# mandanasmi/lane-slam

Hardware: AMD Instinct MI355X
Metric: frames/sec (640x480) detect->descript->project->sanity->associate (higher is better)
Workload: dtype u8/f64 (FP4 e2m1 MFMA with exact f32 accumulation for association)

## Files before the change

lane_slam_amd/csrc/common.h:

```cpp
#pragma once
#include <hip/hip_runtime.h>
#include <stdint.h>
#include <stddef.h>
#include "../../include/lanefront.h"
#include "detmath.h"

namespace lf {

constexpr int kMaxKsize = 9;
constexpr int kMaxGaussTaps = 15;
constexpr float kNotDef = -1024.0f;
#ifndef LF_LABEL_ITEMS
#define LF_LABEL_ITEMS 8192
#endif
constexpr int kLabelItems = LF_LABEL_ITEMS;
#ifndef LF_LABEL_LDS
#define LF_LABEL_LDS 6144
#endif
constexpr int kLabelLds = LF_LABEL_LDS;
constexpr int kCompCap = 1024;

enum Stage {
    ST_PRE = 0, ST_CANNY, ST_HYST, ST_LSD_GRAD, ST_LSD_ORDER, ST_LSD_GROW, ST_SEGMENTS,
    ST_LBD_GRAD, ST_LBD, ST_ASSOC_PACK, ST_ASSOC, ST_MISC, ST_JPEG, ST_LSD_LABEL, ST_HOUGH, ST_DENSE, ST_COUNT
};
static_assert(ST_COUNT == LF_N_STAGES, "stage table out of sync with lanefront.h");

struct PreParams {
    int in_rows, in_cols, img_rows, img_cols, top_cutoff, Hc, W;
    int resize;
    int identity_ai;
    double ifx, ify;
    float ai_scale[3], ai_shift[3];
    int lo[4][3], hi[4][3];
    int ksize, r;
    int j1[kMaxKsize], j2[kMaxKsize];
};

struct CannyParams {
    int Hc, W, Ww;
    int low, high;
};

struct LsdParams {
    int Hc, W;
    int Hs, Ws;
    int Ww;
    int scaled;
    int ntaps, half;
    double k[kMaxGaussTaps];
    double rho;
    double prec, p;
    double log_nt, log_eps, density_th, scale;
    int min_reg_size, n_bins, refine;
    int cap_lines;
    int label_items;
    int label_items_max;
    int label_lds;
    int rec_cap;
    float* r_sd = nullptr;
    float* c_sd = nullptr;
};

struct SegParams {
    int Hc, W, img_rows, img_cols, top_cutoff, cap_lines;
    double rx, ry, cut;
    double cw, ch;
    double H[9], K[9], D[5], RR[9];
    double lanewidth, linewidth_white, linewidth_yellow, d_min, d_max, phi_min, phi_max;
    int rectified_input;
};

struct ResizeTables {
    const int* xofs;
    const float* xa;
    const int* y0;
    const int* y1;
    const float* yb;
    int xmax;
};

}

#ifdef __HIPCC__
__device__ __forceinline__ void lf_xcd_tile(int& bx, int& by, int& bz)
{
    const unsigned nx = gridDim.x, ny = gridDim.y, total = nx * ny * gridDim.z;
    unsigned b = blockIdx.x + nx * (blockIdx.y + ny * blockIdx.z);
    const unsigned group = 8u * nx;
    if (b < total / group * group) {
        const unsigned g = b / group, r = b - g * group;
        b = g * group + (r & 7u) * nx + (r >> 3);
    }
    bx = (int)(b % nx);
    const unsigned q = b / nx;
    by = (int)(q % ny);
    bz = (int)(q / ny);
}
#endif

extern "C" void lf_set_error(lf_handle* h, int code, const char* fmt, ...);

namespace lf {
void launch_pre_gray(const PreParams& p, const uint8_t* frames, int n_frames, uint8_t* gray, hipStream_t s);
void launch_pre(const PreParams& p, const uint8_t* frames, int n_frames, uint32_t* bgr, uint8_t* gray,
                uint32_t* maskbits, const int* sdiv, const int* hdiv, hipStream_t s, uint32_t* bwbits = nullptr);
void launch_canny(const CannyParams& p, const uint32_t* bgr, int n_frames, uint32_t* strong, uint32_t* weak,
                  hipStream_t s);
int launch_hysteresis(const CannyParams& p, int n_frames, uint32_t* strong, const uint32_t* weak, hipStream_t s);
void launch_bgrx_to_bgr(int n_pix, const uint32_t* bgrx, uint8_t* bgr, hipStream_t s);
void launch_edges_u8(const CannyParams& p, int n_frames, const uint32_t* bits, uint8_t* edges, hipStream_t s);
void launch_lsd_grad(const LsdParams& p, const ResizeTables& rt, int n_frames, const uint32_t* edge_bits,
                     const uint32_t* mask_bits, uint32_t* r_addr, float* r_deg, double* r_mod, double* r_cs, double* r_sn,
                     int* n_rec, unsigned long long* maxgrad, int max_nsx, int max_nsy, uint32_t* list, int* list_count,
                     uint32_t* l_addr, double* l_mod, int* n_low, int* rec_need, bool counters_zeroed, hipStream_t s);
void launch_lsd_grad_gray(const LsdParams& p, const ResizeTables& rt, int n_frames, const uint8_t* gray, uint32_t* r_addr, float* r_deg,
                          double* r_mod, double* r_cs, double* r_sn, int* n_rec, unsigned long long* maxgrad, int max_nsx, int max_nsy,
                          uint32_t* list, int* list_count, uint32_t* l_addr, double* l_mod, int* n_low, hipStream_t s);
bool lsd_seed32_supported(const LsdParams& p);
void launch_lsd_seed32(const LsdParams& p, int n_frames, int* n_rec, int* norder, int* rec_need, const unsigned long long* maxgrad, const uint32_t* c_xy,
                       const double* c_mod, const uint32_t* l_addr, double* l_mod, const int* n_low,
                       unsigned long long* sort_a, unsigned long long* sort_b, uint32_t* order_a, uint32_t* order_b, int big, hipStream_t s);
size_t std_sort_debug_words(int n);
void launch_std_sort_debug(const uint32_t* E, uint32_t* work, int n, int* count, hipStream_t s);
void launch_lsd_order(const LsdParams& p, int n_frames, const uint32_t* r_addr, const float* r_deg, const double* r_mod,
                      const double* r_cs, const double* r_sn, int* n_rec, const unsigned long long* maxgrad,
                      unsigned long long* sort_a, unsigned long long* sort_b, uint32_t* order_a, uint32_t* order_b,
                      int* norder, uint32_t* c_xy, float* c_deg, double* c_mod, double* c_cs, double* c_sn,
                      int* row_start, hipStream_t s);
void launch_lsd_dense_debug(const LsdParams& p, int n_frames, const int* norder, const uint32_t* c_xy, const float* c_deg,
                            const double* c_mod, float* ang, double* mod, hipStream_t s);
void launch_lsd_rank(int n_prob, const int* norder, int* perm, hipStream_t s);
void launch_lsd_label(const LsdParams& p, int n_frames, const int* norder, const uint32_t* c_xy, const int* row_start,
                      uint16_t* c_label, uint16_t* comp_list, int* comp_count, int* comp_key, uint32_t* scratch, hipStream_t s);
size_t lsd_grow_reg_stride(const LsdParams& p);
void launch_lsd_grow(const LsdParams& p, int n_frames, const uint32_t* order, const int* norder, const uint32_t* c_xy,
                     const float* c_deg, const double* c_mod, const double* c_cs, const double* c_sn,
                     const int* row_start, const uint16_t* c_label, const uint16_t* comp_list, const int* comp_count, int comp_cap,
                     uint32_t* reg, uint32_t* gused, float* tmp_lines, int* tmp_tags, float* lines, int* counts, const int* perm,
                     int lds_kb, bool mixed, int bitmap, hipStream_t s);
int lsd_grow_def_lds(const LsdParams& p, int lds_kb);
constexpr int kGrowLdsKb[3] = { 13, 28, 40 };
void launch_seg_offsets(int n_frames, int cap_lines, const int* counts, int* seg_offset, int* frame_offset,
                        int* overflow, const int* norder, int cap_small, int cap_medium, hipStream_t s);
void launch_dense(int Hc, int W, int Ww, int cap_lines, float thr, int n_problems, const uint32_t* strong, const uint32_t* maskbits,
                  const uint32_t* bwbits, float* slot_lines, float* rec, int* counts, hipStream_t s);
enum SegMode { SEG_FLOAT = 0, SEG_HOUGH = 1, SEG_DENSE = 2 };
void launch_segments(const SegParams& p, int n_frames, const float* slot_lines, const int* counts,
                     const int* seg_offset, const uint32_t* side, int Ww, lf_segments out, int* seg_frame,
                     double* normals64, float* centers, hipStream_t s, SegMode mode = SEG_FLOAT);
void launch_lbd_grad(int Hc, int W, int n_frames, const uint8_t* gray, uint32_t* dxy, hipStream_t s);
struct LbdPlanes { const uint32_t* base[LF_MAX_OCTAVES]; int W[LF_MAX_OCTAVES], H[LF_MAX_OCTAVES]; };
void launch_lbd_keylines(const LbdPlanes& planes, int n_cap, int n_frames, const int* n_lines, const float* in_octave4, const float* angle, const int* npx,
                         const int* octave, const int* frame, const float* gauss_g, const float* gauss_l, float* desc, uint8_t* code,
                         hipStream_t s, int wband = 7);
void launch_lbd_split_debug(size_t n, const uint32_t* dxy, int16_t* dx, int16_t* dy, hipStream_t s);
void launch_lbd(int Hc, int W, int n_seg_cap, const int* n_seg, const float* lines, const int* seg_frame,
                const uint32_t* dxy, const float* gauss_g, const float* gauss_l,
                float* desc, uint8_t* code, hipStream_t s, int wband = 7);
int lbd_max_width_of_band();
size_t assoc_rows_padded_m(int nm);
__host__ __device__ inline size_t assoc_map_offset_fp4(size_t row, int byte)
{
    return (row >> 6) * 8192 + (size_t)(byte >> 4) * 1024 + (row & 63) * 16 + (size_t)(byte & 15);
}
__host__ __device__ inline uint32_t assoc_fp4_expand(uint32_t byte)
{
    uint32_t t = (byte | (byte << 12)) & 0x000f000fu;
    t = (t | (t << 6)) & 0x03030303u;
    t = (t | (t << 3)) & 0x11111111u;
    return (t << 3) | 0x22222222u;
}
#ifdef __HIPCC__
__device__ __forceinline__ void assoc_map_write_row(int8_t* mx, int8_t* mcx, size_t pos, int b, uint32_t byte, const uint8_t* colour_byte)
{
    *reinterpret_cast<uint32_t*>(mx + assoc_map_offset_fp4(pos, 4 * b)) = assoc_fp4_expand(byte);
    if (b < 8) {
        const int colour = *colour_byte;
        uint32_t w = 0;
        if (b == 0 && colour < 3)
            for (int g = 0; g < 3; ++g) if (g != colour) w |= 0xFu << (4 * g);
        *reinterpret_cast<uint32_t*>(mcx + pos * 32 + 4 * b) = w;
    }
}
__device__ __forceinline__ void assoc_map_zero_row(int8_t* mx, int8_t* mcx, size_t pos, int b)
{
    *reinterpret_cast<uint32_t*>(mx + assoc_map_offset_fp4(pos, 4 * b)) = 0u;
    if (b < 8) *reinterpret_cast<uint32_t*>(mcx + pos * 32 + 4 * b) = 0u;
}
#endif
template <typename T>
struct DevArray {
    T* p = nullptr;
    size_t bytes = 0;
    DevArray() = default;
    DevArray(DevArray&& o) noexcept : p(o.p), bytes(o.bytes) { o.p = nullptr; o.bytes = 0; }
    DevArray& operator=(DevArray&& o) noexcept
    {
        if (this != &o) { reset(); p = o.p; bytes = o.bytes; o.p = nullptr; o.bytes = 0; }
        return *this;
    }
    ~DevArray() { reset(); }
    hipError_t alloc(size_t n_bytes)
    {
        reset();
        const hipError_t e = hipMalloc((void**)&p, n_bytes);
        if (e != hipSuccess) p = nullptr; else bytes = n_bytes;
        return e;
    }
    void reset() { if (p) (void)hipFree(p); p = nullptr; bytes = 0; }
    operator T*() const { return p; }
};
using DevBuf = DevArray<void>;

template <typename T>
struct HostArray {
    T* p = nullptr;
    size_t bytes = 0;
    HostArray() = default;
    HostArray(HostArray&& o) noexcept : p(o.p), bytes(o.bytes) { o.p = nullptr; o.bytes = 0; }
    HostArray& operator=(HostArray&& o) noexcept
    {
        if (this != &o) { reset(); p = o.p; bytes = o.bytes; o.p = nullptr; o.bytes = 0; }
        return *this;
    }
    ~HostArray() { reset(); }
    hipError_t alloc(size_t n_bytes)
    {
        reset();
        const hipError_t e = hipHostMalloc((void**)&p, n_bytes, hipHostMallocDefault);
        if (e != hipSuccess) p = nullptr; else bytes = n_bytes;
        return e;
    }
    void reset() { if (p) (void)hipHostFree(p); p = nullptr; bytes = 0; }
    operator T*() const { return p; }
};

struct AssocScratch {
    DevArray<unsigned int> part; DevArray<int> done; size_t cap_part = 0, cap_blocks = 0;
    int qblocks = 0, splits = 0, m_chunk = 0;
    DevArray<int> tie_list; size_t cap_list = 0;
    unsigned long long* tie_res = nullptr;
};
void launch_assoc_pack_map(const uint8_t* codes, int n, int n_pad, int8_t* x, hipStream_t s);
hipError_t launch_assoc_core(const uint8_t* q, const uint8_t* qcolor, int nq, const int8_t* mx, const int8_t* mcx, int nm,
                             const int* nm_dev, int gating, int max_distance, AssocScratch& w, int32_t* idx, float* dist, hipStream_t s);
hipError_t launch_assoc_ties(const uint8_t* q, const uint8_t* qcolor, int nq, const int8_t* mx, const uint8_t* mcode, const uint8_t* mcolor,
                             int nm, const int* nm_dev, int gating, AssocScratch& w, unsigned long long* res, int32_t* idx, const float* dist, hipStream_t s);
hipError_t launch_assoc(const uint8_t* q, int nq, const uint8_t* m, int nm, int8_t* mx, AssocScratch& w, int32_t* idx, float* dist, hipStream_t s);
void launch_assoc_nomatch(int nq, int32_t* idx, float* dist, hipStream_t s);
void launch_kmeans(const uint8_t* bgr, int n, int k, const double* init, int max_iter, double tol_rel, uint8_t* lab, double* out,
                   long long* counts, int* status, hipStream_t s);
void launch_draw(const void* src, bool src_bgrx, uint8_t* out, int n_frames, int Hc, int W, const int32_t* frame_offset, const float* lines,
                 const uint8_t* color, int capacity, int* bad, hipStream_t s);
void launch_ai_transform(const uint8_t* strips, long long frame_stride, int n_frames, int S, int cols, uint8_t* lab, double* fo,
                         long long* fc, int* fs, lf_ai_transform* out, hipStream_t s);
struct MapDevice {
    int capacity, policy, kept_only, merge_distance, when_full;
    uint8_t* code; uint8_t* color; double* ground; int* hits; int* last_seen; int* winner;
    int8_t* mx; int8_t* mcx;
    int* state;
    unsigned long long* totals;
};
void launch_fill_i32(int* p, size_t n, int v, hipStream_t s);
void launch_map_pack_block(int n, int n_frames, const int* frame_offset, const uint8_t* code, const uint8_t* color,
                           const uint8_t* keep, const double* ground, const int32_t* idx, const float* dist,
                           const double* pose4, int step, uint8_t* block, hipStream_t s);
void launch_map_overflow_block(int n, int n_frames, int step, uint8_t* block, hipStream_t s);
void launch_map_seed_block(int n, const uint8_t* code, const uint8_t* color, const double* ground, uint8_t* block, hipStream_t s);
void launch_map_update(const MapDevice& md, const uint8_t* blocks, int n_blocks, int block_rows, int force_append, int* act,
                       hipStream_t s);
void launch_select_queries(const uint8_t* q, const uint8_t* mask, int nq, uint8_t* out, int32_t* qidx, int* n_out, hipStream_t s);
void launch_knn(const uint8_t* q, int nq, const uint8_t* m, int nm, int k, int max_distance, int mih, int32_t* idx, float* dist, hipStream_t s);
void launch_radius(const uint8_t* q, int nq, const uint8_t* m, int nm, int max_distance, int32_t* hist, int32_t* count, int32_t* offsets,
                   int* total, int cap, int mih, int32_t* idx, float* dist, hipStream_t s);
size_t assoc_float_scratch_bytes(int nq, int nm);
hipError_t launch_assoc_float(const float* q, int nq, const float* m, int nm, float* qn, float* mn,
                              void* scratch, int32_t* idx, float* dist, hipStream_t s);
namespace jpeg { struct FrameHeader; }
struct JpegGeom { int rows, cols, Wp, Hp; int first_row = 0; };
void launch_jpeg_decode(const JpegGeom& g, int n_frames, int max_blocks, const jpeg::FrameHeader* hdrs,
                        const uint32_t* entries, const uint32_t* block_end, uint8_t* planes, uint8_t* frames,
                        hipStream_t s);

void launch_jpeg_color(const JpegGeom& g, int n_frames, const void* hdrs, size_t hdr_stride, const uint8_t* planes, uint8_t* frames, hipStream_t s);
namespace jpeg { struct DevFrame; }
void launch_jh_decode(const JpegGeom& g, int n_frames, int max_blocks, size_t max_scan_len, jpeg::DevFrame* frames, const uint8_t* bytes, uint8_t* clean,
                      uint32_t* seg_begin, void* info, uint32_t* sub, int16_t* coef, int* status, uint8_t* planes, hipStream_t s);
size_t jh_info_bytes();

void launch_msg_layout(int n_frames, int stage, const int* frame_offset, const uint8_t* keep, int* counts,
                       long long* byte_offset, hipStream_t s);
void launch_msg_write(int n_frames, int stage, const int* frame_offset, const uint8_t* color, const float* pixels_normalized,
                      const float* normals, const double* ground, const uint8_t* keep, const int* counts,
                      const long long* byte_offset, uint8_t* out, hipStream_t s);
void launch_msg_read(int n_frames, int capacity, const uint8_t* body, const long long* byte_offset, int* frame_offset,
                     int* bad, uint8_t* color, float* pixels_normalized, float* normals, double* ground, hipStream_t s);

}
```

lane_slam_amd/csrc/k_lbd.hip:

```cpp
#include "common.h"

namespace lf {

#ifndef LF_LBD_TILE_H
#define LF_LBD_TILE_H 64
#endif
constexpr int LT_W = 64, LT_H = LF_LBD_TILE_H;
static_assert(LT_H % 16 == 0, "the Sobel phase gives every lane LT_H / 16 rows of its column group");

__device__ __forceinline__ int refl101(int p, int n)
{
    if (n == 1) return 0;
    while (p < 0 || p >= n) { p = p < 0 ? -p : 2 * (n - 1) - p; }
    return p;
}

__global__ __launch_bounds__(256) void k_lbd_grad(int Hc, int W, const uint8_t* __restrict__ gray_in,
                                                  uint32_t* __restrict__ dxyo)
{
    constexpr int GW = 72, GH = LT_H + 6;
    constexpr int RW = 68, RG = RW / 4;
    constexpr int BW_ = 72, BH = LT_H + 2;
    __shared__ __attribute__((aligned(16))) uint8_t gray[GH * GW];
    __shared__ __attribute__((aligned(16))) uint32_t rowp[(GH / 2) * RW];
    __shared__ __attribute__((aligned(16))) uint8_t blur[BH * BW_];
    int tbx, tby, f;
    lf_xcd_tile(tbx, tby, f);
    const int x0 = tbx * LT_W, y0 = tby * LT_H;
    const int tid = threadIdx.y * 64 + threadIdx.x;
    const uint8_t* img = gray_in + (size_t)f * Hc * W;
    const bool interior = x0 >= 4 && x0 + 72 <= W;
    auto reflect_row = [&](int ty) {
        int gy = y0 + ty - 3;
        gy = gy < 0 ? -gy : (gy >= Hc ? 2 * (Hc - 1) - gy : gy);
        if (gy < 0 || gy >= Hc) gy = refl101(y0 + ty - 3, Hc);
        return (uint32_t)gy * (uint32_t)W;
    };
    if (interior) {
        const uint8_t* base = img + (x0 - 4);
        for (int idx = tid; idx < GH * (GW / 4); idx += 256) {
            const int ty = idx / (GW / 4), g = idx - ty * (GW / 4);
            const uint32_t* q = reinterpret_cast<const uint32_t*>(base + (reflect_row(ty) + 4u * (uint32_t)g));
            *reinterpret_cast<uint32_t*>(gray + ty * GW + 4 * g) = (q[0] >> 8) | (q[1] << 24);
        }
    } else {
        for (int idx = tid; idx < GH * (GW / 4); idx += 256) {
            const int ty = idx / (GW / 4), g = idx - ty * (GW / 4);
            const uint32_t row = reflect_row(ty);
            const int xa = x0 + 4 * g - 4;
            uint32_t packed = 0;
            if (xa >= 0 && xa + 7 < W) {
                const uint32_t* q = reinterpret_cast<const uint32_t*>(img + (row + (uint32_t)xa));
                packed = (q[0] >> 8) | (q[1] << 24);
            } else {
#pragma unroll
                for (int k = 0; k < 4; ++k) packed |= (uint32_t)img[row + (uint32_t)refl101(x0 + 4 * g + k - 3, W)] << (8 * k);
            }
            *reinterpret_cast<uint32_t*>(gray + ty * GW + 4 * g) = packed;
        }
    }
    __syncthreads();
    static_assert(GH % 2 == 0 && BH % 2 == 0, "rows are filtered in pairs");
    typedef unsigned short us2 __attribute__((ext_vector_type(2)));
    for (int idx = tid; idx < (GH / 2) * RG; idx += 256) {
        const int m = idx / RG, g = idx - m * RG;
        uint32_t o02[2], o13[2];
#pragma unroll
        for (int r = 0; r < 2; ++r) {
            const uint32_t* src = reinterpret_cast<const uint32_t*>(gray + (2 * m + r) * GW + 4 * g);
            const uint32_t lo = src[0], hi = src[1];
            const us2 E = __builtin_bit_cast(us2, lo & 0x00ff00ffu), O = __builtin_bit_cast(us2, (lo >> 8) & 0x00ff00ffu);
            const us2 E2 = __builtin_bit_cast(us2, hi & 0x00ff00ffu), O2 = __builtin_bit_cast(us2, (hi >> 8) & 0x00ff00ffu);
            const us2 P24 = { E.y, E2.x }, P35 = { O.y, O2.x };
            const us2 c14 = { 14, 14 }, c63 = { 63, 63 }, c103 = { 103, 103 };
            o02[r] = __builtin_bit_cast(uint32_t, c14 * E + c63 * O + c103 * P24 + c63 * P35 + c14 * E2);
            o13[r] = __builtin_bit_cast(uint32_t, c14 * O + c63 * P24 + c103 * P35 + c63 * E2 + c14 * O2);
        }
        const uint4 q = make_uint4(__builtin_amdgcn_perm(o02[1], o02[0], 0x05040100u), __builtin_amdgcn_perm(o13[1], o13[0], 0x05040100u),
                                   __builtin_amdgcn_perm(o02[1], o02[0], 0x07060302u), __builtin_amdgcn_perm(o13[1], o13[0], 0x07060302u));
        *reinterpret_cast<uint4*>(rowp + m * RW + 4 * g) = q;
    }
    __syncthreads();
    {
        constexpr int VPAIRS = 3, VSEG = (BH / 2 + VPAIRS - 1) / VPAIRS;
        static_assert(VSEG * RG <= 256, "one lane per (column group, segment)");
        const int g = tid % RG, seg = tid / RG;
        if (seg < VSEG) {
            const int m0 = seg * VPAIRS;
            uint4 P[3];
            auto fetch = [&](int m) { return *reinterpret_cast<const uint4*>(rowp + (m < GH / 2 ? m : GH / 2 - 1) * RW + 4 * g); };
            P[0] = fetch(m0); P[1] = fetch(m0 + 1);
#pragma unroll
            for (int i = 0; i < VPAIRS; ++i) {
                const int m = m0 + i;
                P[(i + 2) % 3] = fetch(m + 2);
                if (2 * m < BH) {
                    const uint4 A = P[i % 3], B = P[(i + 1) % 3], C = P[(i + 2) % 3];
                    const uint32_t a[4] = { A.x, A.y, A.z, A.w }, bb[4] = { B.x, B.y, B.z, B.w }, cc[4] = { C.x, C.y, C.z, C.w };
                    uint32_t even = 0, odd = 0;
#pragma unroll
                    for (int k = 0; k < 4; ++k) {
                        uint32_t e = __builtin_amdgcn_udot2(__builtin_bit_cast(us2, a[k]), us2{ 14, 63 }, 1u << 15, false);
                        e = __builtin_amdgcn_udot2(__builtin_bit_cast(us2, bb[k]), us2{ 103, 63 }, e, false);
                        e = __builtin_amdgcn_udot2(__builtin_bit_cast(us2, cc[k]), us2{ 14, 0 }, e, false);
                        uint32_t o = __builtin_amdgcn_udot2(__builtin_bit_cast(us2, a[k]), us2{ 0, 14 }, 1u << 15, false);
                        o = __builtin_amdgcn_udot2(__builtin_bit_cast(us2, bb[k]), us2{ 63, 103 }, o, false);
                        o = __builtin_amdgcn_udot2(__builtin_bit_cast(us2, cc[k]), us2{ 63, 14 }, o, false);
                        e >>= 16; o >>= 16;
                        even |= (e > 255u ? 255u : e) << (8 * k);
                        odd |= (o > 255u ? 255u : o) << (8 * k);
                    }
                    *reinterpret_cast<uint32_t*>(blur + (2 * m) * BW_ + 4 * g) = even;
                    *reinterpret_cast<uint32_t*>(blur + (2 * m + 1) * BW_ + 4 * g) = odd;
                }
            }
        }
    }
    __syncthreads();
    {
        constexpr int SROWS = LT_H / 16;
        const int g = tid & 15, seg = tid >> 4;
        const int lx = 4 * g, gx = x0 + lx, ry0 = seg * SROWS;
        typedef short s2 __attribute__((ext_vector_type(2)));
        s2 P[3][4];
        auto unpack = [&](int row, s2 (&d)[4]) {
            const uint32_t* src = reinterpret_cast<const uint32_t*>(blur + row * BW_ + lx);
            const uint32_t lo = src[0], hi = src[1];
            const s2 E = __builtin_bit_cast(s2, lo & 0x00ff00ffu), O = __builtin_bit_cast(s2, (lo >> 8) & 0x00ff00ffu);
            const s2 E2 = __builtin_bit_cast(s2, hi & 0x00ff00ffu), O2 = __builtin_bit_cast(s2, (hi >> 8) & 0x00ff00ffu);
            d[0] = E; d[1] = O; d[2] = s2{ E.y, E2.x }; d[3] = s2{ O.y, O2.x };
        };
        unpack(ry0, P[0]);
        unpack(ry0 + 1, P[1]);
        auto a_plus_2b = [](s2 a, s2 b) {
            s2 d;
            const uint32_t two = 0x00020002u;
            asm("v_pk_mad_i16 %0, %1, %2, %3" : "=v"(d) : "v"(b), "v"(two), "v"(a));
            return d;
        };
        uint32_t* orow = dxyo + ((size_t)f * Hc + (size_t)(y0 + ry0)) * W + gx;
#pragma unroll
        for (int i = 0; i < SROWS; ++i) {
            const int ry = ry0 + i, gy = y0 + ry;
            unpack(ry + 2, P[(i + 2) % 3]);
            if (gx < W && gy < Hc) {
                s2 S[4], D[4];
#pragma unroll
                for (int c = 0; c < 4; ++c) { S[c] = a_plus_2b(P[i % 3][c], P[(i + 1) % 3][c]) + P[(i + 2) % 3][c]; D[c] = P[(i + 2) % 3][c] - P[i % 3][c]; }
                const s2 vx02 = S[2] - S[0], vx13 = S[3] - S[1];
                const s2 vy02 = a_plus_2b(D[0], D[1]) + D[2], vy13 = a_plus_2b(D[1], D[2]) + D[3];
                uint32_t* op = orow + (size_t)i * W;
                const uint32_t x02 = __builtin_bit_cast(uint32_t, vx02), x13 = __builtin_bit_cast(uint32_t, vx13);
                const uint32_t y02 = __builtin_bit_cast(uint32_t, vy02), y13 = __builtin_bit_cast(uint32_t, vy13);
                const uint32_t w[4] = { __builtin_amdgcn_perm(y02, x02, 0x05040100u), __builtin_amdgcn_perm(y13, x13, 0x05040100u),
                                        __builtin_amdgcn_perm(y02, x02, 0x07060302u), __builtin_amdgcn_perm(y13, x13, 0x07060302u) };
                if (gx + 3 < W && (W & 3) == 0) {
                    *reinterpret_cast<uint4*>(op) = make_uint4(w[0], w[1], w[2], w[3]);
                } else {
                    for (int k = 0; k < 4 && gx + k < W; ++k) op[k] = w[k];
                }
            }
        }
    }
}

void launch_lbd_grad(int Hc, int W, int n_frames, const uint8_t* gray, uint32_t* dxy, hipStream_t s)
{
    dim3 grid((W + LT_W - 1) / LT_W, (Hc + LT_H - 1) / LT_H, n_frames);
    hipLaunchKernelGGL(k_lbd_grad, grid, dim3(64, 4), 0, s, Hc, W, gray, dxy);
}

__constant__ int c_comb[32][2] = {
    {0,1},{0,2},{0,3},{0,4},{0,5},{0,6},{1,2},{1,3},{1,4},{1,5},{1,6},{2,3},{2,4},{2,5},{2,6},{2,7},
    {2,8},{3,4},{3,5},{3,6},{3,7},{3,8},{4,5},{4,6},{4,7},{4,8},{5,6},{5,7},{5,8},{6,7},{6,8},{7,8} };

constexpr int NBANDS = 9, WBAND = 7, LSP_H = 63;
constexpr int LBD_STEPS = 8;

constexpr int LBD_MAXW = 21;
template <bool KL, bool ANYW = false>
__global__ __launch_bounds__(256) void k_lbd(int Hc_, int W_, const int* __restrict__ n_seg_ptr,
                                             const float* __restrict__ lines, const int* __restrict__ seg_frame,
                                             const uint32_t* __restrict__ dxyi,
                                             const float* __restrict__ gauss_g , const float* __restrict__ gauss_l ,
                                             float* __restrict__ desc, uint8_t* __restrict__ code,
                                             LbdPlanes planes, const float* __restrict__ kl_angle, const int* __restrict__ kl_npx,
                                             const int* __restrict__ kl_octave, int n_cap, int n_frames, int wband_arg = WBAND)
{
    const int WBAND = ANYW ? wband_arg : lf::WBAND;
    const int LSP_H = ANYW ? NBANDS * wband_arg : lf::LSP_H;
    __shared__ float rows[4][ANYW ? NBANDS * LBD_MAXW : lf::LSP_H][4];
    __shared__ float dsc[4][72];
    const int wave = threadIdx.x >> 6, lane = threadIdx.x & 63;
    const int n_seg = min(*n_seg_ptr, n_cap);
  for (int seg = blockIdx.x * 4 + wave; seg < n_seg; seg += gridDim.x * 4) {
    __builtin_amdgcn_wave_barrier();
    __builtin_amdgcn_fence(__ATOMIC_ACQ_REL, "wavefront");
    const int f = seg_frame[seg];
    int Hc = Hc_, W = W_;
    const uint32_t* pdxy;
    float e0 = lines[4 * (size_t)seg], e1 = lines[4 * (size_t)seg + 1], e2 = lines[4 * (size_t)seg + 2], e3 = lines[4 * (size_t)seg + 3];
    int lengthOfLSP;
    float direction;
    if (KL) {
        const int oc = kl_octave[seg];
        if (oc < 0 || oc >= LF_MAX_OCTAVES || planes.base[oc] == nullptr || f < 0 || f >= n_frames) {
            if (desc) for (int i = lane; i < 72; i += 64) desc[(size_t)seg * 72 + i] = 0.f;
            if (code && lane < 32) code[(size_t)seg * 32 + lane] = 0;
            continue;
        }
        Hc = planes.H[oc]; W = planes.W[oc];
        pdxy = planes.base[oc] + (size_t)f * Hc * W;
        lengthOfLSP = (int)(short)kl_npx[seg];
        direction = kl_angle[seg];
    } else {
    pdxy = dxyi + (size_t)f * Hc * W;
    if (e0 < 0) e0 = 0;
    if (e0 >= W) e0 = (float)W - 1.0f;
    if (e2 < 0) e2 = 0;
    if (e2 >= W) e2 = (float)W - 1.0f;
    if (e1 < 0) e1 = 0;
    if (e1 >= Hc) e1 = (float)Hc - 1.0f;
    if (e3 < 0) e3 = 0;
    if (e3 >= Hc) e3 = (float)Hc - 1.0f;
    const int ix0 = dm::round_half_even((double)e0), iy0 = dm::round_half_even((double)e1);
    const int ix1 = dm::round_half_even((double)e2), iy1 = dm::round_half_even((double)e3);
    lengthOfLSP = max(abs(ix1 - ix0), abs(iy1 - iy0)) + 1;
    const float ddy = e3 - e1, ddx = e2 - e0;
    direction = (float)dm::datan2((double)ddy, (double)ddx);
    }
    const int halfWidth = (lengthOfLSP - 1) / 2;
    const int halfHeight = (LSP_H - 1) / 2;
    const int imageWidth = W - 1, imageHeight = Hc - 1;
    const float midX = (float)(0.5 * (e0 + e2));
    const float midY = (float)(0.5 * (e1 + e3));
    double sn_, cs_;
    dm::dsincos((double)direction, sn_, cs_);
    const float dL0 = (float)cs_, dL1 = (float)sn_;
    const float dO0 = -dL1, dO1 = dL0;
    float sCorX0 = -dL0 * halfWidth + dL1 * halfHeight + midX;
    float sCorY0 = -dL1 * halfWidth - dL0 * halfHeight + midY;
    int row_done = 0;
    for (int row = lane; row < LSP_H; row += 64) {
        for (; row_done < row; ++row_done) { sCorX0 -= dL1; sCorY0 += dL0; }
        float sCorX = sCorX0, sCorY = sCorY0;
        float pgdL = 0, ngdL = 0, pgdO = 0, ngdO = 0;
        for (int w0 = 0; w0 < lengthOfLSP; w0 += LBD_STEPS) {
            uint32_t dxyv[LBD_STEPS];
#pragma unroll
            for (int u = 0; u < LBD_STEPS; ++u) {
                int tx = (int)dm::round_half_away_f(sCorX);
                int xCor = tx < 0 ? 0 : (tx > imageWidth ? imageWidth : tx);
                int ty = (int)dm::round_half_away_f(sCorY);
                int yCor = ty < 0 ? 0 : (ty > imageHeight ? imageHeight : ty);
                dxyv[u] = pdxy[yCor * W + xCor];
                sCorX += dL0;
                sCorY += dL1;
            }
#pragma unroll
            for (int u = 0; u < LBD_STEPS; ++u) {
                if (w0 + u >= lengthOfLSP) break;
                const float gx_ = (float)(int)(int16_t)(dxyv[u] & 0xffffu), gy_ = (float)((int)dxyv[u] >> 16);
                float gDL = gx_ * dL0 + gy_ * dL1;
                float gDO = gx_ * dO0 + gy_ * dO1;
                if (gDL > 0) pgdL += gDL; else ngdL -= gDL;
                if (gDO > 0) pgdO += gDO; else ngdO -= gDO;
            }
        }
        const float cg = gauss_g[row];
        rows[wave][row][0] = cg * pgdL;
        rows[wave][row][1] = cg * ngdL;
        rows[wave][row][2] = cg * pgdO;
        rows[wave][row][3] = cg * ngdO;
        if (!ANYW) break;
    }
    __builtin_amdgcn_wave_barrier();
    __builtin_amdgcn_fence(__ATOMIC_ACQ_REL, "wavefront");
    float* D = dsc[wave];
    for (int e = lane; e < 72; e += 64) {
        const int b = e >> 3, q = e & 7;
        const bool sq = q >= 4;
        const int src = q & 3;
        const int h0 = (b - 1) * WBAND;
        const float* rp = &rows[wave][0][src] + 4 * h0;
        float acc = 0;
#pragma unroll
        for (int i = 0; i < (ANYW ? 3 * LBD_MAXW : 3 * lf::WBAND); ++i) {
            if (ANYW && i >= 3 * WBAND) break;
            const int hID = h0 + i;
            if (hID >= 0 && hID < LSP_H) {
                const float coef = gauss_l[i];
                const float v = rp[4 * i];
                if (!sq) acc += coef * v;
                else acc += coef * coef * (v * v);
            }
        }
        D[e] = acc;
    }
    __builtin_amdgcn_wave_barrier();
    __builtin_amdgcn_fence(__ATOMIC_ACQ_REL, "wavefront");
    float mean[4] = {0, 0, 0, 0}, sd[4] = {0, 0, 0, 0};
    if (lane < NBANDS) {
        const float invN = (lane == 0 || lane == NBANDS - 1) ? (float)(1.0 / (WBAND * 2.0)) : (float)(1.0 / (WBAND * 3.0));
#pragma unroll
        for (int q = 0; q < 4; ++q) {
            float temp = D[lane * 8 + q] * invN;
            mean[q] = temp;
            sd[q] = (float)dm::dsqrt((double)(D[lane * 8 + 4 + q] * invN - temp * temp));
        }
    }
    __builtin_amdgcn_wave_barrier();
    __builtin_amdgcn_fence(__ATOMIC_ACQ_REL, "wavefront");
    if (lane < NBANDS) {
#pragma unroll
        for (int q = 0; q < 4; ++q) { D[lane * 8 + q] = mean[q]; D[lane * 8 + 4 + q] = sd[q]; }
    }
    __builtin_amdgcn_wave_barrier();
    __builtin_amdgcn_fence(__ATOMIC_ACQ_REL, "wavefront");
    float tempM = 0, tempS = 0;
    for (int b = 0; b < NBANDS; ++b) {
        const float* v = D + 8 * b;
        tempM += v[0] * v[0]; tempM += v[1] * v[1]; tempM += v[2] * v[2]; tempM += v[3] * v[3];
        tempS += v[4] * v[4]; tempS += v[5] * v[5]; tempS += v[6] * v[6]; tempS += v[7] * v[7];
    }
    tempM = dm::fdiv(1.f, dm::fsqrt(tempM));
    tempS = dm::fdiv(1.f, dm::fsqrt(tempS));
    __builtin_amdgcn_wave_barrier();
    for (int e = lane; e < 72; e += 64) {
        float v = D[e] * (((e & 7) < 4) ? tempM : tempS);
        if ((double)v > 0.4) v = (float)0.4;
        D[e] = v;
    }
    __builtin_amdgcn_wave_barrier();
    __builtin_amdgcn_fence(__ATOMIC_ACQ_REL, "wavefront");
    float temp = 0;
    for (int i = 0; i < 72; ++i) temp += D[i] * D[i];
    temp = dm::fdiv(1.f, dm::fsqrt(temp));
    __builtin_amdgcn_wave_barrier();
    for (int e = lane; e < 72; e += 64) {
        float v = D[e] * temp;
        D[e] = v;
        if (desc) desc[(size_t)seg * 72 + e] = v;
    }
    __builtin_amdgcn_wave_barrier();
    __builtin_amdgcn_fence(__ATOMIC_ACQ_REL, "wavefront");
    if (code && lane < 32) {
        const float* f1 = D + 8 * c_comb[lane][0];
        const float* f2 = D + 8 * c_comb[lane][1];
        unsigned r = 0;
#pragma unroll
        for (int i = 0; i < 8; ++i) if (f1[i] > f2[i]) r += 1u << i;
        code[(size_t)seg * 32 + lane] = (uint8_t)r;
    }
  }
}

void launch_lbd(int Hc, int W, int n_seg_cap, const int* n_seg, const float* lines, const int* seg_frame,
                const uint32_t* dxy, const float* gauss_g, const float* gauss_l,
                float* desc, uint8_t* code, hipStream_t s, int wband)
{
    if (n_seg_cap <= 0) return;
    int blocks = (n_seg_cap + 3) / 4;
    if (blocks > 4096) blocks = 4096;
    LbdPlanes none;
    for (int i = 0; i < LF_MAX_OCTAVES; ++i) { none.base[i] = nullptr; none.W[i] = 0; none.H[i] = 0; }
    if (wband == WBAND)
        hipLaunchKernelGGL((k_lbd<false, false>), dim3(blocks), dim3(256), 0, s, Hc, W, n_seg, lines, seg_frame, dxy,
                           gauss_g, gauss_l, desc, code, none, nullptr, nullptr, nullptr, n_seg_cap, 0, WBAND);
    else
        hipLaunchKernelGGL((k_lbd<false, true>), dim3(blocks), dim3(256), 0, s, Hc, W, n_seg, lines, seg_frame, dxy,
                           gauss_g, gauss_l, desc, code, none, nullptr, nullptr, nullptr, n_seg_cap, 0, wband);
}
int lbd_max_width_of_band() { return LBD_MAXW; }

void launch_lbd_keylines(const LbdPlanes& planes, int n_cap, int n_frames, const int* n_lines, const float* in_octave4, const float* angle, const int* npx,
                         const int* octave, const int* frame, const float* gauss_g, const float* gauss_l, float* desc, uint8_t* code,
                         hipStream_t s, int wband)
{
    if (n_cap <= 0) return;
    int blocks = (n_cap + 3) / 4;
    if (blocks > 4096) blocks = 4096;
    if (wband == WBAND)
        hipLaunchKernelGGL((k_lbd<true, false>), dim3(blocks), dim3(256), 0, s, 0, 0, n_lines, in_octave4, frame, nullptr, gauss_g, gauss_l, desc, code,
                           planes, angle, npx, octave, n_cap, n_frames, WBAND);
    else
        hipLaunchKernelGGL((k_lbd<true, true>), dim3(blocks), dim3(256), 0, s, 0, 0, n_lines, in_octave4, frame, nullptr, gauss_g, gauss_l, desc, code,
                           planes, angle, npx, octave, n_cap, n_frames, wband);
}

__global__ void k_lbd_split_debug(size_t n, const uint32_t* __restrict__ dxy, int16_t* __restrict__ dx, int16_t* __restrict__ dy)
{
    const size_t i = blockIdx.x * (size_t)blockDim.x + threadIdx.x;
    if (i >= n) return;
    const uint32_t v = dxy[i];
    dx[i] = (int16_t)(v & 0xffffu);
    dy[i] = (int16_t)(v >> 16);
}

void launch_lbd_split_debug(size_t n, const uint32_t* dxy, int16_t* dx, int16_t* dy, hipStream_t s)
{
    hipLaunchKernelGGL(k_lbd_split_debug, dim3((unsigned)((n + 255) / 256)), dim3(256), 0, s, n, dxy, dx, dy);
}

}
```

lane_slam_amd/csrc/k_segments.hip:

```cpp
#include "common.h"
#include "lane_vote.h"

namespace lf {

__global__ void k_seg_offsets(int n_frames, int cap_lines, const int* __restrict__ counts, int* __restrict__ seg_offset,
                              int* __restrict__ frame_offset, int* __restrict__ overflow, const int* __restrict__ norder, int cap_small, int cap_medium)
{
    __shared__ int carry;
    __shared__ int wsum[16];
    const int n = n_frames * 3;
    const int t = threadIdx.x, lane = t & 63, wave = t >> 6;
    if (t == 0) carry = 0;
    __syncthreads();
    int ovf = 0;
    for (int base = 0; base < n; base += blockDim.x) {
        int i = base + t;
        int v = 0;
        if (i < n) {
            v = counts[i]; if (v > cap_lines) { v = cap_lines; ovf = 1; }
            if (norder) { const int nd = norder[i]; if (nd > cap_small) atomicAdd(overflow + 1, 1); if (nd > cap_medium) atomicAdd(overflow + 2, 1); atomicMax(overflow + 3, nd); }
        }
        int inc = v;
#pragma unroll
        for (int d = 1; d < 64; d <<= 1) { int o = __shfl_up(inc, d); if (lane >= d) inc += o; }
        if (lane == 63) wsum[wave] = inc;
        __syncthreads();
        int off = carry;
        for (int w = 0; w < wave; ++w) off += wsum[w];
        if (i < n) {
            int ex = off + inc - v;
            seg_offset[i] = ex;
            if (i % 3 == 0) frame_offset[i / 3] = ex;
        }
        __syncthreads();
        if (t == blockDim.x - 1) carry = off + inc;
        __syncthreads();
    }
    if (t == 0) { seg_offset[n] = carry; frame_offset[n_frames] = carry; overflow[7] = carry; }
    if (ovf) atomicOr(overflow, 1);
}

void launch_seg_offsets(int n_frames, int cap_lines, const int* counts, int* seg_offset, int* frame_offset,
                        int* overflow, const int* norder, int cap_small, int cap_medium, hipStream_t s)
{
    hipLaunchKernelGGL(k_seg_offsets, dim3(1), dim3(256), 0, s, n_frames, cap_lines, counts, seg_offset,
                       frame_offset, overflow, norder, cap_small, cap_medium);
}

__device__ __forceinline__ int check_bounds(int v, int bound) { return v < 0 ? 0 : (v >= bound ? bound - 1 : v); }

__device__ void ground_point(const SegParams& p, double vx, double vy, double& gx, double& gy)
{
    double u = p.cw * vx, v = p.ch * vy;
    if (u < 0) u = 0;
    if (u > p.cw - 1) u = p.cw - 1;
    if (v < 0) v = 0;
    if (v > p.ch - 1) v = 0;
    double ur = u, vr = v;
    if (!p.rectified_input) {
    const double fx = p.K[0], fy = p.K[4], cx = p.K[2], cy = p.K[5];
    const double ifx = 1. / fx, ify = 1. / fy;
    const double* k = p.D;
    double x = (u - cx) * ifx, y = (v - cy) * ify;
    const double x0 = x, y0 = y;
    for (int j = 0; j < 5; ++j) {
        double r2 = x * x + y * y;
        double icdist = 1 / (1 + ((k[4] * r2 + k[1]) * r2 + k[0]) * r2);
        double deltaX = 2 * k[2] * x * y + k[3] * (r2 + 2 * x * x);
        double deltaY = k[2] * (r2 + 2 * y * y) + 2 * k[3] * x * y;
        x = (x0 - deltaX) * icdist;
        y = (y0 - deltaY) * icdist;
    }
    const double* RR = p.RR;
    double xx = RR[0] * x + RR[1] * y + RR[2];
    double yy = RR[3] * x + RR[4] * y + RR[5];
    double ww = 1. / (RR[6] * x + RR[7] * y + RR[8]);
    ur = xx * ww; vr = yy * ww;
    }
    const double* H = p.H;
    double g0 = H[0] * ur + H[1] * vr + H[2] * 1.0;
    double g1 = H[3] * ur + H[4] * vr + H[5] * 1.0;
    double g2 = H[6] * ur + H[7] * vr + H[8] * 1.0;
    gx = g0 / g2;
    gy = g1 / g2;
}

template <int kMode>
__global__ void k_segments(SegParams p, int n_frames, const float* __restrict__ slot_lines,
                           const int* __restrict__ counts, const int* __restrict__ seg_offset,
                           const uint32_t* __restrict__ maskbits, int Ww, lf_segments out, int* __restrict__ seg_frame,
                           double* __restrict__ normals64, float* __restrict__ centers)
{
    const int slot = blockIdx.x * blockDim.x + threadIdx.x;
    const int pc = slot / p.cap_lines, i = slot - pc * p.cap_lines;
    if (pc >= n_frames * 3) return;
    int cnt = counts[pc];
    if (cnt > p.cap_lines) cnt = p.cap_lines;
    if (i >= cnt) return;
    const int idx = seg_offset[pc] + i;
    if (idx >= out.capacity) return;
    const int f = pc / 3, col = pc - 3 * f;
    const float* L = slot_lines + ((size_t)pc * p.cap_lines + i) * 4;
    float x1 = L[0], y1 = L[1], x2 = L[2], y2 = L[3];
    if constexpr (kMode == SEG_DENSE) {
        const float4 r = reinterpret_cast<const float4*>(maskbits)[(size_t)pc * p.cap_lines + i];
        if (out.lines) { float* o = out.lines + 4 * (size_t)idx; o[0] = x1; o[1] = y1; o[2] = x2; o[3] = y2; }
        if (out.normals) { out.normals[2 * (size_t)idx] = r.x; out.normals[2 * (size_t)idx + 1] = r.y; }
        if (out.color) out.color[idx] = (uint8_t)col;
        if (normals64) { normals64[2 * (size_t)idx] = (double)r.x; normals64[2 * (size_t)idx + 1] = (double)r.y; }
        if (centers) { centers[2 * (size_t)idx] = r.z; centers[2 * (size_t)idx + 1] = r.w; }
    } else if constexpr (kMode == SEG_HOUGH) {
        int ix1 = (int)x1, iy1 = (int)y1, ix2 = (int)x2, iy2 = (int)y2;
        const int ex = ix1 - ix2, ey = iy1 - iy2;
        const double len = dm::dsqrt((double)(ex * ex + ey * ey));
        const double dx = (double)(iy2 - iy1) / len;
        const double dy = (double)(ix1 - ix2) / len;
        const int cx = (ix1 + ix2) >> 1, cy = (iy1 + iy2) >> 1;
        int x3 = (int)((double)cx - 3. * dx), y3 = (int)((double)cy - 3. * dy);
        int x4 = (int)((double)cx + 3. * dx), y4 = (int)((double)cy + 3. * dy);
        x3 = check_bounds(x3, p.W); y3 = check_bounds(y3, p.Hc);
        x4 = check_bounds(x4, p.W); y4 = check_bounds(y4, p.Hc);
        const uint32_t* bw = maskbits + (size_t)pc * p.Hc * Ww;
        const bool on3 = (bw[(size_t)y3 * Ww + (x3 >> 5)] >> (x3 & 31)) & 1u;
        const bool on4 = (bw[(size_t)y4 * Ww + (x4 >> 5)] >> (x4 & 31)) & 1u;
        const int sign = (on3 && !on4) ? 1 : -1;
        const double nx = dx * sign, ny = dy * sign;
        const double flag = (double)(ix2 - ix1) * ny - (double)(iy2 - iy1) * nx;
        if (flag > 0) { int tx = ix1, ty = iy1; ix1 = ix2; iy1 = iy2; ix2 = tx; iy2 = ty; }
        x1 = (float)ix1; y1 = (float)iy1; x2 = (float)ix2; y2 = (float)iy2;
        if (out.lines) { float* o = out.lines + 4 * (size_t)idx; o[0] = x1; o[1] = y1; o[2] = x2; o[3] = y2; }
        if (out.normals) { out.normals[2 * (size_t)idx] = (float)nx; out.normals[2 * (size_t)idx + 1] = (float)ny; }
        if (out.color) out.color[idx] = (uint8_t)col;
        if (normals64) { normals64[2 * (size_t)idx] = nx; normals64[2 * (size_t)idx + 1] = ny; }
        if (centers) { centers[2 * (size_t)idx] = (float)cx; centers[2 * (size_t)idx + 1] = (float)cy; }
    } else {
    const float ex = x1 - x2, ey = y1 - y2;
    const float len = dm::fsqrt(ex * ex + ey * ey);
    const float dx = dm::fdiv(y2 - y1, len);
    const float dy = dm::fdiv(x1 - x2, len);
    const float cx = (x1 + x2) / 2, cy = (y1 + y2) / 2;
    int x3 = (int)(cx - 3.f * dx), y3 = (int)(cy - 3.f * dy);
    int x4 = (int)(cx + 3.f * dx), y4 = (int)(cy + 3.f * dy);
    x3 = check_bounds(x3, p.W); y3 = check_bounds(y3, p.Hc);
    x4 = check_bounds(x4, p.W); y4 = check_bounds(y4, p.Hc);
    const uint32_t* bw = maskbits + (size_t)pc * p.Hc * Ww;
    const bool on3 = (bw[(size_t)y3 * Ww + (x3 >> 5)] >> (x3 & 31)) & 1u;
    const bool on4 = (bw[(size_t)y4 * Ww + (x4 >> 5)] >> (x4 & 31)) & 1u;
    const int sign = (on3 && !on4) ? 1 : -1;
    const double nx = (double)dx * sign, ny = (double)dy * sign;
    const double flag = (double)(x2 - x1) * ny - (double)(y2 - y1) * nx;
    if (flag > 0) { float tx = x1, ty = y1; x1 = x2; y1 = y2; x2 = tx; y2 = ty; }
    if (out.lines) { float* o = out.lines + 4 * (size_t)idx; o[0] = x1; o[1] = y1; o[2] = x2; o[3] = y2; }
    if (out.normals) { out.normals[2 * (size_t)idx] = (float)nx; out.normals[2 * (size_t)idx + 1] = (float)ny; }
    if (out.color) out.color[idx] = (uint8_t)col;
    if (normals64) { normals64[2 * (size_t)idx] = nx; normals64[2 * (size_t)idx + 1] = ny; }
    if (centers) { centers[2 * (size_t)idx] = cx; centers[2 * (size_t)idx + 1] = cy; }
    }
    if (seg_frame) seg_frame[idx] = f;
    const float pn0 = (float)(((double)x1 + 0.0) * p.rx);
    const float pn1 = (float)(((double)y1 + p.cut) * p.ry);
    const float pn2 = (float)(((double)x2 + 0.0) * p.rx);
    const float pn3 = (float)(((double)y2 + p.cut) * p.ry);
    if (out.pixels_normalized) {
        float* o = out.pixels_normalized + 4 * (size_t)idx;
        o[0] = pn0; o[1] = pn1; o[2] = pn2; o[3] = pn3;
    }
    double p1x, p1y, p2x, p2y;
    ground_point(p, (double)pn0, (double)pn1, p1x, p1y);
    ground_point(p, (double)pn2, (double)pn3, p2x, p2y);
    if (out.ground) { double* o = out.ground + 4 * (size_t)idx; o[0] = p1x; o[1] = p1y; o[2] = p2x; o[3] = p2y; }
    if (out.keep) {
        double d_i, phi_i;
        const int state = lane_vote(col, p1x, p1y, p2x, p2y, p.lanewidth, p.linewidth_white, p.linewidth_yellow, d_i, phi_i);
        int k = 1;
        if (p1x < 0 || p2x < 0) k = 0;
        else if (col != LF_WHITE && col != LF_YELLOW) k = 0;
        else if (state == 0) k = 0;
        else if (d_i > p.d_max || d_i < p.d_min || phi_i < p.phi_min || phi_i > p.phi_max) k = 0;
        out.keep[idx] = (uint8_t)k;
    }
}

void launch_segments(const SegParams& p, int n_frames, const float* slot_lines, const int* counts,
                     const int* seg_offset, const uint32_t* side, int Ww, lf_segments out, int* seg_frame,
                     double* normals64, float* centers, hipStream_t s, SegMode mode)
{
    const int total = n_frames * 3 * p.cap_lines;
    if (mode == SEG_DENSE)
        hipLaunchKernelGGL(k_segments<SEG_DENSE>, dim3((total + 255) / 256), dim3(256), 0, s, p, n_frames, slot_lines, counts,
                           seg_offset, side, Ww, out, seg_frame, normals64, centers);
    else if (mode == SEG_HOUGH)
        hipLaunchKernelGGL(k_segments<SEG_HOUGH>, dim3((total + 255) / 256), dim3(256), 0, s, p, n_frames, slot_lines, counts,
                           seg_offset, side, Ww, out, seg_frame, normals64, centers);
    else
        hipLaunchKernelGGL(k_segments<SEG_FLOAT>, dim3((total + 255) / 256), dim3(256), 0, s, p, n_frames, slot_lines, counts,
                           seg_offset, side, Ww, out, seg_frame, normals64, centers);
}

}
```

lane_slam_amd/csrc/lanefront_api.hip:

```cpp
#include <stdarg.h>
#include <stdio.h>
#include <string.h>
#include <math.h>
#include <vector>
#include <new>
#include <atomic>
#include <chrono>
#include <cstdlib>
#include <functional>
#include "lanefront_handle.h"

using namespace lf;

static const char* kStageNames[LF_N_STAGES] = {
    "pre(resize+correct+hsv+masks+dilate)", "canny_nms", "canny_hysteresis", "lsd_blur_resample_grad",
    "lsd_order", "lsd_grow", "segments(normal+project+sanity)", "lbd_gray_blur_sobel", "lbd_descriptor",
    "assoc_pack", "assoc_mfma", "misc", "jpeg(idct+upsample+color)", "lsd_label(components+launch order)",
    "hough(probabilistic lines)", "dense(sobel-vote lines)" };




extern "C" void lf_set_error(lf_handle* h, int code, const char* fmt, ...)
{
    va_list ap;
    va_start(ap, fmt);
    vset_error(h, code, fmt, ap);
    va_end(ap);
}

static char g_create_err[512] = "no error";



static int cv_round_host(double v) { return dm::round_half_even(v); }


static int build_params(lf_handle* h)
{
    const lf_config& c = h->cfg;
    h->Hc = c.img_rows - c.top_cutoff;
    h->W = c.img_cols;
    if (h->Hc <= 0 || h->W <= 0 || c.in_rows <= 0 || c.in_cols <= 0 || c.top_cutoff < 0) {
        lf_set_error(h, LF_ERR_BAD_ARG, "bad geometry: in %dx%d img %dx%d cutoff %d", c.in_rows, c.in_cols, c.img_rows,
                     c.img_cols, c.top_cutoff);
        return LF_ERR_BAD_ARG;
    }
    if (h->W % 32 != 0) { lf_set_error(h, LF_ERR_UNSUPPORTED, "img_cols must be a multiple of 32 (got %d)", h->W); return LF_ERR_UNSUPPORTED; }
    h->P = (size_t)h->Hc * h->W;
    h->Ww = (h->W + 31) / 32;
    PreParams& p = h->pre;
    memset(&p, 0, sizeof(p));
    p.in_rows = c.in_rows; p.in_cols = c.in_cols; p.img_rows = c.img_rows; p.img_cols = c.img_cols;
    p.top_cutoff = c.top_cutoff; p.Hc = h->Hc; p.W = h->W;
    p.resize = (c.img_rows != c.in_rows) || (c.img_cols != c.in_cols);
    const double fx = (double)c.img_cols / (double)c.in_cols, fy = (double)c.img_rows / (double)c.in_rows;
    p.ifx = 1.0 / fx; p.ify = 1.0 / fy;
    p.identity_ai = 1;
    for (int i = 0; i < 3; ++i) { p.ai_scale[i] = c.ai_scale[i]; p.ai_shift[i] = c.ai_shift[i]; if (c.ai_scale[i] != 1.f || c.ai_shift[i] != 0.f) p.identity_ai = 0; }
    for (int k = 0; k < 4; ++k) for (int ch = 0; ch < 3; ++ch) { p.lo[k][ch] = c.hsv_lo[k][ch]; p.hi[k][ch] = c.hsv_hi[k][ch]; }
    p.ksize = c.dilation_kernel_size;
    if (p.ksize < 1 || p.ksize > kMaxKsize) { lf_set_error(h, LF_ERR_UNSUPPORTED, "dilation_kernel_size %d not in [1,%d]", p.ksize, kMaxKsize); return LF_ERR_UNSUPPORTED; }
    p.r = p.ksize / 2;
    {
        int r = p.ksize / 2, cc = p.ksize / 2;
        double inv_r2 = r ? 1.0 / ((double)r * r) : 0.0;
        for (int i = 0; i < p.ksize; ++i) {
            int dy = i - r;
            p.j1[i] = 0; p.j2[i] = 0;
            if (abs(dy) <= r) {
                int dx = cv_round_host(cc * sqrt((r * r - dy * dy) * inv_r2));
                p.j1[i] = cc - dx > 0 ? cc - dx : 0;
                p.j2[i] = cc + dx + 1 < p.ksize ? cc + dx + 1 : p.ksize;
            }
        }
        if (p.ksize % 2 == 0) { lf_set_error(h, LF_ERR_UNSUPPORTED, "even dilation kernels are not supported"); return LF_ERR_UNSUPPORTED; }
    }
    h->canny.Hc = h->Hc; h->canny.W = h->W; h->canny.Ww = h->Ww;
    double lo = c.canny_lo, hi = c.canny_hi;
    if (lo > hi) { double t = lo; lo = hi; hi = t; }
    h->canny.low = dm::ifloor(lo); h->canny.high = dm::ifloor(hi);
    if ((size_t)h->Hc * h->Ww > 8 * 1024 && (8192 / h->Ww < 1 || (int)((60 * 1024 / 4) / (2 * (size_t)h->Ww)) - 1 < 1)) { lf_set_error(h, LF_ERR_UNSUPPORTED, "img_cols %d: one row of the edge bit planes exceeds the hysteresis strip budget", h->W); return LF_ERR_UNSUPPORTED; }
    SegParams& S = h->seg;
    memset(&S, 0, sizeof(S));
    S.Hc = h->Hc; S.W = h->W; S.img_rows = c.img_rows; S.img_cols = c.img_cols; S.top_cutoff = c.top_cutoff;
    S.cap_lines = h->cap_lines;
    S.rx = 1.0 / (double)c.img_cols; S.ry = 1.0 / (double)c.img_rows; S.cut = (double)c.top_cutoff;
    memcpy(S.H, c.H, sizeof(S.H));
    seg_camera(h);
    S.lanewidth = c.lanewidth; S.linewidth_white = c.linewidth_white; S.linewidth_yellow = c.linewidth_yellow;
    S.d_min = c.d_min; S.d_max = c.d_max; S.phi_min = c.phi_min; S.phi_max = c.phi_max;
    return LF_OK;
}

static int lbd_weights(lf_handle* h, int w)
{
    std::vector<float> gg(9 * (size_t)w), gl(3 * (size_t)w);
    double u = (w * 3 - 1) / 2;
    double sigma = (w * 2 + 1) / 2;
    double inv = -1 / (2 * sigma * sigma);
    for (int i = 0; i < 3 * w; ++i) { double d = i - u; gl[i] = (float)dm::dexp(d * d * inv); }
    u = (9 * w - 1) / 2;
    sigma = u;
    inv = -1 / (2 * sigma * sigma);
    for (int i = 0; i < 9 * w; ++i) { double d = i - u; gg[i] = (float)dm::dexp(d * d * inv); }
    LF_HIP_CHECK(h, hipMemcpy(h->d_gauss_g, gg.data(), gg.size() * sizeof(float), hipMemcpyHostToDevice));
    LF_HIP_CHECK(h, hipMemcpy(h->d_gauss_l, gl.data(), gl.size() * sizeof(float), hipMemcpyHostToDevice));
    return LF_OK;
}

static int upload_tables(lf_handle* h)
{
    std::vector<int> sdiv(256), hdiv(256);
    sdiv[0] = hdiv[0] = 0;
    for (int i = 1; i < 256; ++i) {
        sdiv[i] = cv_round_host((255 << 12) / (1.0 * i));
        hdiv[i] = cv_round_host((180 << 12) / (6.0 * i));
    }
    if (dalloc(h, &h->d_sdiv, 256) || dalloc(h, &h->d_hdiv, 256)) return LF_ERR_HIP;
    LF_HIP_CHECK(h, hipMemcpy(h->d_sdiv, sdiv.data(), 256 * sizeof(int), hipMemcpyHostToDevice));
    LF_HIP_CHECK(h, hipMemcpy(h->d_hdiv, hdiv.data(), 256 * sizeof(int), hipMemcpyHostToDevice));
    const int mw = lbd_max_width_of_band();
    if (dalloc(h, &h->d_gauss_g, 9 * (size_t)mw) || dalloc(h, &h->d_gauss_l, 3 * (size_t)mw)) return LF_ERR_HIP;
    return lbd_weights(h, h->desc_params.width_of_band);
}

extern "C" void lf_descriptor_default_params(lf_descriptor_params* p)
{
    if (!p) return;
    p->num_of_octave = 1; p->width_of_band = 7; p->reduction_ratio = 2; p->ksize = 5;
}

extern "C" int lf_get_descriptor_params(lf_handle* h, lf_descriptor_params* p)
{
    if (!h) return LF_ERR_NOT_INITIALISED;
    if (!p) { lf_set_error(h, LF_ERR_BAD_ARG, "lf_get_descriptor_params: null argument"); return LF_ERR_BAD_ARG; }
    *p = h->desc_params;
    return LF_OK;
}

extern "C" int lf_set_descriptor_params(lf_handle* h, const lf_descriptor_params* p)
{
    if (!h) return LF_ERR_NOT_INITIALISED;
    if (!p) { lf_set_error(h, LF_ERR_BAD_ARG, "lf_set_descriptor_params: null argument"); return LF_ERR_BAD_ARG; }
    if (h->pending) { lf_set_error(h, LF_ERR_BAD_ARG, "a batch is in flight on this handle: call lf_wait first"); return LF_ERR_BAD_ARG; }
    if (p->width_of_band < 1 || p->width_of_band > lbd_max_width_of_band()) {
        lf_set_error(h, LF_ERR_UNSUPPORTED, "widthOfBand %d outside 1..%d", p->width_of_band, lbd_max_width_of_band());
        return LF_ERR_UNSUPPORTED;
    }
    if (p->ksize < 1 || p->ksize > 31 || !(p->ksize & 1)) { lf_set_error(h, LF_ERR_BAD_ARG, "ksize %d: an odd size in 1..31 (cv::GaussianBlur asserts the oddness)", p->ksize); return LF_ERR_BAD_ARG; }
    if (p->num_of_octave < 1 || p->num_of_octave > LF_MAX_OCTAVES || p->reduction_ratio < 1) {
        lf_set_error(h, LF_ERR_BAD_ARG, "lf_set_descriptor_params: numOfOctave_ outside 1..%d or reductionRatio < 1", LF_MAX_OCTAVES);
        return LF_ERR_BAD_ARG;
    }
    LF_HIP_CHECK(h, hipSetDevice(h->device));
    LF_HIP_CHECK(h, hipStreamSynchronize(h->stream));
    if (p->width_of_band != h->desc_params.width_of_band) { const int rc = lbd_weights(h, p->width_of_band); if (rc != LF_OK) return rc; }
    h->desc_params = *p;
    return LF_OK;
}

static int init_lsd(lf_handle* h)
{
    const lf_config& c = h->cfg;
    lf_lsd_options o;
    o.refine = c.lsd_refine; o.n_bins = c.lsd_n_bins; o.scale = c.lsd_scale; o.sigma_scale = c.lsd_sigma_scale; o.quant = c.lsd_quant;
    o.ang_th = c.lsd_ang_th; o.log_eps = c.lsd_log_eps; o.density_th = c.lsd_density_th; o.min_length = 0.0;
    const int rc = h->lsd.init(h, h->Hc, h->W, o, c.lsd_seed_order, h->max_frames, h->cap_lines);
    if (rc != LF_OK) return rc;
    const size_t Ps = h->lsd.Ps;
    size_t cap = Ps;
    if (h->max_frames > 16) cap = (Ps / 8 + 4095) / 4096 * 4096;
    const char* e = getenv("LF_LSD_RECORDS");
    if (e && *e) { if (!strcmp(e, "full")) cap = Ps; else if (atol(e) > 0) cap = (size_t)atol(e); }
    else if (cap < 8192) cap = 8192;
    if (cap < 1024) cap = 1024;
    if (cap > Ps) cap = Ps;
    return h->lsd.alloc_lists(h, (int)cap);
}

static int alloc_buffers(lf_handle* h)
{
    const size_t B = (size_t)h->max_frames, P = h->P;
    const size_t in_px = (size_t)h->cfg.in_rows * h->cfg.in_cols;
    const size_t nprob = B * 3;
    const size_t cap = nprob * (size_t)h->cap_lines;
    h->frames_bytes = B * in_px * 3 > P * 3 ? B * in_px * 3 : P * 3;
    if (dalloc(h, &h->d_frames, h->frames_bytes) || dalloc(h, &h->d_bgr, B * P) || dalloc(h, &h->d_gray, B * P) || 
        dalloc(h, &h->d_edges_u8, B * P) || dalloc(h, &h->d_strong, B * h->Hc * h->Ww) || dalloc(h, &h->d_weak, B * h->Hc * h->Ww) || dalloc(h, &h->d_maskbits, nprob * h->Hc * h->Ww) ||
        dalloc(h, &h->d_counts, nprob) || dalloc(h, &h->d_seg_offset, nprob + 1) || dalloc(h, &h->d_frame_offset, B + 1) ||
        dalloc(h, &h->d_slot_lines, cap * 4) || dalloc(h, &h->d_seg_frame, cap) ||
        dalloc(h, &h->d_dxy, B * P) || dalloc(h, &h->d_normals64, cap * 2) ||
        dalloc(h, &h->d_centers, cap * 2))
        return LF_ERR_HIP;
    h->out_capacity = (int)cap;
    lf_segments& o = h->d_out;
    memset(&o, 0, sizeof(o));
    o.capacity = (int)cap;
    if (dalloc(h, &h->out_lines, cap * 4) || dalloc(h, &h->out_normals, cap * 2) || dalloc(h, &h->out_color, cap) ||
        dalloc(h, &h->out_pixels_normalized, cap * 4) || dalloc(h, &h->out_ground, cap * 4) || dalloc(h, &h->out_keep, cap) ||
        dalloc(h, &h->out_desc, cap * 72) || dalloc(h, &h->out_code, cap * 32))
        return LF_ERR_HIP;
    o.lines = h->out_lines; o.normals = h->out_normals; o.color = h->out_color; o.pixels_normalized = h->out_pixels_normalized;
    o.ground = h->out_ground; o.keep = h->out_keep; o.desc = h->out_desc; o.code = h->out_code;
    o.frame_offset = h->d_frame_offset;
    LF_HIP_CHECK(h, h->h_pinned.alloc(16 * sizeof(int)));
    return LF_OK;
}

extern "C" int lf_abi_version(void) { return LF_ABI_VERSION; }

extern "C" int lf_get_stream(lf_handle* h, void** hip_stream)
{
    if (!h) return LF_ERR_NOT_INITIALISED;
    if (!hip_stream) { lf_set_error(h, LF_ERR_BAD_ARG, "lf_get_stream: null argument"); return LF_ERR_BAD_ARG; }
    *hip_stream = static_cast<void*>(h->stream);
    return LF_OK;
}

extern "C" const char* lf_last_error(const lf_handle* h) { return h ? h->err : g_create_err; }

extern "C" const char* lf_stage_name(int stage) { return (stage >= 0 && stage < LF_N_STAGES) ? kStageNames[stage] : "?"; }

extern "C" void lf_destroy(lf_handle* h)
{
    if (!h) return;
    (void)hipSetDevice(h->device);
    if (h->stream) (void)hipStreamSynchronize(h->stream);
    if (h->stream) (void)hipStreamDestroy(h->stream);
    delete h;
}

extern "C" int lf_create(const lf_config* cfg, int device_id, int max_frames, int max_lines_per_color, lf_handle** out)
{
    if (!cfg || !out || max_frames < 1 || max_lines_per_color < 1) {
        snprintf(g_create_err, sizeof(g_create_err), "lf_create: bad argument");
        return LF_ERR_BAD_ARG;
    }
    *out = nullptr;
    if (const int rc = check_device(device_id, "lf_create", g_create_err, sizeof(g_create_err))) return rc;
    lf_handle* h = new (std::nothrow) lf_handle();
    if (!h) return LF_ERR_HIP;
    h->cfg = *cfg; h->device = device_id; h->max_frames = max_frames; h->cap_lines = max_lines_per_color;
    if (const char* ev = getenv("LF_KL_LDS_LINES")) { const int v = atoi(ev); h->env_kl_lds_lines = v < 1 ? 1 : (v > 4096 ? 4096 : v); }
    int rc = LF_OK;
    do {
        if (hipSetDevice(device_id) != hipSuccess) { lf_set_error(h, LF_ERR_HIP, "hipSetDevice(%d) failed", device_id); rc = LF_ERR_HIP; break; }
        if ((rc = build_params(h)) != LF_OK) break;
        if ((rc = init_lsd(h)) != LF_OK) break;
        if (hipStreamCreateWithFlags(&h->stream, hipStreamNonBlocking) != hipSuccess) { lf_set_error(h, LF_ERR_HIP, "hipStreamCreate failed"); rc = LF_ERR_HIP; break; }
        if ((rc = upload_tables(h)) != LF_OK) break;
        if ((rc = alloc_buffers(h)) != LF_OK) break;
    } while (0);
    if (rc != LF_OK) {
        snprintf(g_create_err, sizeof(g_create_err), "%s", h->err);
        lf_destroy(h);
        return rc;
    }
    *out = h;
    return LF_OK;
}

extern "C" int lf_synchronize(lf_handle* h)
{
    if (!h) return LF_ERR_NOT_INITIALISED;
    LF_HIP_CHECK(h, hipSetDevice(h->device));
    LF_HIP_CHECK(h, hipStreamSynchronize(h->stream));
    return LF_OK;
}

static const char* detector_name(int detector)
{
    return detector == LF_DETECTOR_HOUGH ? "HoughLinesP" : (detector == LF_DETECTOR_DENSE ? "LineDetector2Dense" : "LSD");
}

int lf::run_detect(lf_handle* h, const uint8_t* d_frames, int n, bool from_working_image)
{
    hipStream_t s = h->stream;
    if (h->lsd.lists_lost) { lf_set_error(h, LF_ERR_HIP, "the handle lost its LSD lists to an out-of-memory growth (lf_wait / lf_set_image reported it)"); return LF_ERR_HIP; }
    h->overflow_zeroed = false;
    h->draw_frames = 0;
    PreParams pp = h->pre;
    if (from_working_image) {
        pp.in_rows = h->Hc; pp.in_cols = h->W; pp.img_rows = h->Hc; pp.img_cols = h->W; pp.top_cutoff = 0;
        pp.resize = 0;
        for (int i = 0; i < 3; ++i) { pp.ai_scale[i] = 1.f; pp.ai_shift[i] = 0.f; }
        pp.identity_ai = 1;
    }
    const bool dense = h->detector == LF_DETECTOR_DENSE;
    if (dense) {
        int rc = dense_prepare(h);
        if (rc != LF_OK) return rc;
    }
    { StageClock::Scope t(h, h->clock, ST_PRE); launch_pre(pp, d_frames, n, h->d_bgr, h->d_gray, h->d_maskbits, h->d_sdiv, h->d_hdiv, s, dense ? h->d_bwbits.p : nullptr); }
    { StageClock::Scope t(h, h->clock, ST_CANNY); launch_canny(h->canny, h->d_bgr, n, h->d_strong, h->d_weak, s); }
    {
        StageClock::Scope t(h, h->clock, ST_HYST);
        if (launch_hysteresis(h->canny, n, h->d_strong, h->d_weak, s) != 0) {
            lf_set_error(h, LF_ERR_UNSUPPORTED, "canny hysteresis: a %dx%d working image does not fit the LDS-resident strips", h->Hc, h->W);
            return LF_ERR_UNSUPPORTED;
        }
    }
    if (h->detector == LF_DETECTOR_HOUGH) {
        int rc = hough_prepare(h);
        if (rc != LF_OK) return rc;
        StageClock::Scope t(h, h->clock, ST_HOUGH);
        LF_HIP_CHECK(h, hipMemsetAsync(h->lsd.d_zero, 0, h->lsd.zero_bytes, s));
        HoughParams hp = h->hough_p;
        hp.threshold = h->hough_params.threshold; hp.line_length = h->hough_params.min_line_length; hp.line_gap = h->hough_params.max_line_gap;
        launch_hough(hp, n * 3, h->hough_slots < n * 3 ? h->hough_slots : n * 3, h->d_strong, h->d_maskbits, h->d_hough_tab, h->d_hough_acc,
                     h->d_hough_nz, h->d_slot_lines, h->d_counts, s);
        LF_HIP_CHECK(h, hipGetLastError());
        h->slot_mode = SEG_HOUGH;
        h->last_frames = n;
        h->overflow_zeroed = true;
        return LF_OK;
    }
    if (dense) {
        StageClock::Scope t(h, h->clock, ST_DENSE);
        LF_HIP_CHECK(h, hipMemsetAsync(h->lsd.d_zero, 0, h->lsd.zero_bytes, s));
        launch_dense(h->Hc, h->W, h->Ww, h->cap_lines, (float)h->dense_params.sobel_threshold, n * 3, h->d_strong, h->d_maskbits,
                     h->d_bwbits, h->d_slot_lines, h->d_dense_rec, h->d_counts, s);
        LF_HIP_CHECK(h, hipGetLastError());
        h->slot_mode = SEG_DENSE;
        h->last_frames = n;
        h->overflow_zeroed = true;
        return LF_OK;
    }
    h->slot_mode = SEG_FLOAT;
    {
        StageClock::Scope t(h, h->clock, ST_LSD_GRAD);
        LF_HIP_CHECK(h, hipMemsetAsync(h->lsd.d_zero, 0, h->lsd.zero_bytes, s));
        h->lsd.grad(n, h->d_strong, h->d_maskbits, true, s);
    }
    { StageClock::Scope t(h, h->clock, ST_LSD_ORDER); h->lsd.order(n, 0, s); }
    {
        StageClock::Scope t(h, h->clock, ST_LSD_LABEL);
        h->lsd.label(n, true, s);
    }
    static const char* diag_skip = getenv("LF_DIAG_SKIP");
    if (diag_skip && strstr(diag_skip, "grow")) LF_HIP_CHECK(h, hipMemsetAsync(h->d_counts, 0, (size_t)n * 3 * sizeof(int), s));
    else {
        StageClock::Scope t(h, h->clock, ST_LSD_GROW);
        const LsdState& L = h->lsd;
        h->lsd.grow(n, h->d_slot_lines, h->d_counts, kGrowLdsKb[L.env_lds_level >= 0 ? L.env_lds_level : L.grow_lds_level],
                    L.env_mixed >= 0 ? L.env_mixed != 0 : L.grow_mixed, true, s);
    }
    LF_HIP_CHECK(h, hipGetLastError());
    h->last_frames = n;
    h->overflow_zeroed = true;
    return LF_OK;
}


int lf::run_segments(lf_handle* h, int n, lf_segments dev_out, bool describe)
{
    hipStream_t s = h->stream;
    {
        StageClock::Scope t(h, h->clock, ST_SEGMENTS);
        if (!h->overflow_zeroed) LF_HIP_CHECK(h, hipMemsetAsync(h->lsd.d_overflow, 0, 4 * sizeof(int), s));
        h->overflow_zeroed = false;
        launch_seg_offsets(n, h->cap_lines, h->d_counts, h->d_seg_offset, dev_out.frame_offset ? dev_out.frame_offset : h->d_frame_offset,
                           h->lsd.d_overflow, h->slot_mode != SEG_FLOAT ? nullptr : h->lsd.d_norder, lsd_grow_def_lds(h->lsd.params, kGrowLdsKb[0]),
                           lsd_grow_def_lds(h->lsd.params, kGrowLdsKb[1]), s);
        launch_segments(h->seg, n, h->d_slot_lines, h->d_counts, h->d_seg_offset,
                        h->slot_mode == SEG_DENSE ? reinterpret_cast<const uint32_t*>(h->d_dense_rec.p) : h->d_maskbits.p, h->Ww, dev_out,
                        h->d_seg_frame, h->d_normals64, h->d_centers, s, h->slot_mode);
    }
    if (describe) {
        { StageClock::Scope t(h, h->clock, ST_LBD_GRAD); launch_lbd_grad(h->Hc, h->W, n, h->d_gray, h->d_dxy, s); }
        {
            StageClock::Scope t(h, h->clock, ST_LBD);
            int cap = dev_out.capacity < n * 3 * h->cap_lines ? dev_out.capacity : n * 3 * h->cap_lines;
            launch_lbd(h->Hc, h->W, cap, h->d_seg_offset + n * 3, dev_out.lines, h->d_seg_frame, h->d_dxy,
                       h->d_gauss_g, h->d_gauss_l, dev_out.desc, dev_out.code, s, h->desc_params.width_of_band);
        }
    }
    LF_HIP_CHECK(h, hipGetLastError());
    return LF_OK;
}

extern "C" int lf_process_batch_async(lf_handle* h, const uint8_t* frames, int n_frames, int frames_on_device,
                                      lf_segments* out_dev, int describe)
{
    if (!h) return LF_ERR_NOT_INITIALISED;
    if (!frames || !out_dev || n_frames < 1) { lf_set_error(h, LF_ERR_BAD_ARG, "lf_process_batch: null argument or n_frames < 1"); return LF_ERR_BAD_ARG; }
    if (n_frames > h->max_frames) { lf_set_error(h, LF_ERR_CAPACITY, "n_frames %d exceeds max_frames %d", n_frames, h->max_frames); return LF_ERR_CAPACITY; }
    if (describe && (!out_dev->lines)) { lf_set_error(h, LF_ERR_BAD_ARG, "describe needs out->lines"); return LF_ERR_BAD_ARG; }
    if (h->pending) { lf_set_error(h, LF_ERR_BAD_ARG, "a batch is already in flight on this handle: call lf_wait first"); return LF_ERR_BAD_ARG; }
    LF_HIP_CHECK(h, hipSetDevice(h->device));
    hipStream_t s = h->stream;
    const size_t frame_bytes = (size_t)h->cfg.in_rows * h->cfg.in_cols * 3;
    const uint8_t* d_in = frames;
    if (!frames_on_device) {
        int r0 = h->cfg.top_cutoff;
        if (h->pre.resize) r0 = dm::ifloor(h->cfg.top_cutoff * h->pre.ify) - 1;
        r0 = r0 < 0 ? 0 : (r0 > h->cfg.in_rows - 1 ? h->cfg.in_rows - 1 : r0);
        const size_t skip = (size_t)r0 * h->cfg.in_cols * 3;
        LF_HIP_CHECK(h, hipMemcpy2DAsync(h->d_frames + skip, frame_bytes, frames + skip, frame_bytes, frame_bytes - skip, (size_t)n_frames,
                                         hipMemcpyHostToDevice, s));
        d_in = h->d_frames;
    }
    h->plugin_ready = false;
    int rc = h->detector == LF_DETECTOR_EDLINES ? run_detect_edlines(h, d_in, n_frames) : run_detect(h, d_in, n_frames, false);
    if (rc != LF_OK) return rc;
    rc = run_segments(h, n_frames, *out_dev, describe != 0);
    if (rc != LF_OK) return rc;
    LF_HIP_CHECK(h, hipMemcpyAsync(&h->h_pinned[1], h->lsd.d_overflow, 8 * sizeof(int), hipMemcpyDeviceToHost, s));
    h->pending = true;
    h->pending_keylines = false;
    h->pending_problems = n_frames * 3;
    h->pending_capacity = out_dev->capacity;
    h->pend_in = d_in; h->pend_n = n_frames; h->pend_out = *out_dev; h->pend_describe = describe != 0;
    return LF_OK;
}

extern "C" int lf_wait(lf_handle* h, int* n_segments)
{
    if (!h) return LF_ERR_NOT_INITIALISED;
    LF_HIP_CHECK(h, hipSetDevice(h->device));
    LF_HIP_CHECK(h, hipStreamSynchronize(h->stream));
    if (!h->pending) { if (n_segments) *n_segments = 0; return LF_OK; }
    h->pending = false;
    if (h->pending_keylines) {
        h->pending_keylines = false;
        int total_kl = 0, overflow = 0;
        keylines_pending_result(h, &total_kl, &overflow);
        if (n_segments) *n_segments = total_kl;
        if (overflow) { lf_set_error(h, LF_ERR_CAPACITY, "%d KeyLines exceed the output capacity %d", total_kl, h->pending_capacity); return LF_ERR_CAPACITY; }
        return LF_OK;
    }
    for (int attempt = 0; h->detector == LF_DETECTOR_LSD && h->h_pinned[6] > h->lsd.params.rec_cap; ++attempt) {
        if (attempt == 4) { lf_set_error(h, LF_ERR_CAPACITY, "the LSD lists keep overflowing (%d entries needed)", h->h_pinned[6]); return LF_ERR_CAPACITY; }
        int rc = h->lsd.grow_lists(h, h->h_pinned[6]);
        if (rc == LF_OK) rc = run_detect(h, h->pend_in, h->pend_n, false);
        if (rc == LF_OK) rc = run_segments(h, h->pend_n, h->pend_out, h->pend_describe);
        if (rc != LF_OK) return rc;
        LF_HIP_CHECK(h, hipMemcpyAsync(&h->h_pinned[1], h->lsd.d_overflow, 8 * sizeof(int), hipMemcpyDeviceToHost, h->stream));
        LF_HIP_CHECK(h, hipStreamSynchronize(h->stream));
    }
    h->detector_failures = h->detector == LF_DETECTOR_EDLINES ? h->h_pinned[5] : 0;
    h->draw_frames = 0;
    const int total = h->h_pinned[8];
    if (n_segments) *n_segments = total;
    if (h->pending_problems > 0) h->lsd.adapt_slice(h->h_pinned[2], h->h_pinned[3], h->pending_problems);
    if (h->h_pinned[1]) { lf_set_error(h, LF_ERR_CAPACITY, "%s %s run produced more than max_lines_per_color=%d lines", h->detector == LF_DETECTOR_DENSE ? "a" : "an", detector_name(h->detector), h->cap_lines); return LF_ERR_CAPACITY; }
    if (total > h->pending_capacity) { lf_set_error(h, LF_ERR_CAPACITY, "%d segments exceed the output capacity %d", total, h->pending_capacity); return LF_ERR_CAPACITY; }
    h->draw_frames = h->pend_n;
    return LF_OK;
}

extern "C" int lf_process_batch(lf_handle* h, const uint8_t* frames, int n_frames, int frames_on_device,
                                lf_segments* out, int out_on_device, int describe, int* n_segments)
{
    if (!h) return LF_ERR_NOT_INITIALISED;
    if (!out) { lf_set_error(h, LF_ERR_BAD_ARG, "lf_process_batch: null out"); return LF_ERR_BAD_ARG; }
    lf_segments dev = out_on_device ? *out : h->d_out;
    if (!out_on_device) {
        dev.capacity = out->capacity < h->out_capacity ? out->capacity : h->out_capacity;
        if (!out->normals) dev.normals = nullptr;
        if (!out->color) dev.color = nullptr;
        if (!out->pixels_normalized) dev.pixels_normalized = nullptr;
        if (!out->ground) dev.ground = nullptr;
        if (!out->keep) dev.keep = nullptr;
        if (!out->desc) dev.desc = nullptr;
        if (!out->code) dev.code = nullptr;
        dev.frame_offset = h->d_frame_offset;
        if (describe && !out->lines) { lf_set_error(h, LF_ERR_BAD_ARG, "describe needs out->lines"); return LF_ERR_BAD_ARG; }
    }
    int rc = lf_process_batch_async(h, frames, n_frames, frames_on_device, &dev, describe);
    if (rc != LF_OK) return rc;
    int total = 0;
    rc = lf_wait(h, &total);
    if (n_segments) *n_segments = total;
    if (rc != LF_OK) return rc;
    hipStream_t s = h->stream;
    if (!out_on_device) {
        const size_t n = (size_t)total;
        if (out->frame_offset) LF_HIP_CHECK(h, hipMemcpyAsync(out->frame_offset, h->d_frame_offset, (n_frames + 1) * sizeof(int), hipMemcpyDeviceToHost, s));
        if (out->lines) LF_HIP_CHECK(h, hipMemcpyAsync(out->lines, dev.lines, n * 4 * sizeof(float), hipMemcpyDeviceToHost, s));
        if (out->normals) LF_HIP_CHECK(h, hipMemcpyAsync(out->normals, dev.normals, n * 2 * sizeof(float), hipMemcpyDeviceToHost, s));
        if (out->color) LF_HIP_CHECK(h, hipMemcpyAsync(out->color, dev.color, n, hipMemcpyDeviceToHost, s));
        if (out->pixels_normalized) LF_HIP_CHECK(h, hipMemcpyAsync(out->pixels_normalized, dev.pixels_normalized, n * 4 * sizeof(float), hipMemcpyDeviceToHost, s));
        if (out->ground) LF_HIP_CHECK(h, hipMemcpyAsync(out->ground, dev.ground, n * 4 * sizeof(double), hipMemcpyDeviceToHost, s));
        if (out->keep) LF_HIP_CHECK(h, hipMemcpyAsync(out->keep, dev.keep, n, hipMemcpyDeviceToHost, s));
        if (describe && out->desc) LF_HIP_CHECK(h, hipMemcpyAsync(out->desc, dev.desc, n * 72 * sizeof(float), hipMemcpyDeviceToHost, s));
        if (describe && out->code) LF_HIP_CHECK(h, hipMemcpyAsync(out->code, dev.code, n * 32, hipMemcpyDeviceToHost, s));
        LF_HIP_CHECK(h, hipStreamSynchronize(s));
    }
    return LF_OK;
}

constexpr int kPlugEager = 1024;

int lf::plugin_stage_image(lf_handle* h, const uint8_t* bgr, int rows, int cols, int row_stride_bytes)
{
    const size_t need = (size_t)rows * cols * 3;
    if (h->plug_in.bytes < need) LF_HIP_CHECK(h, h->plug_in.alloc(need));
    LF_HIP_CHECK(h, hipStreamSynchronize(h->stream));
    for (int y = 0; y < rows; ++y) memcpy(h->plug_in + (size_t)y * cols * 3, bgr + (size_t)y * row_stride_bytes, (size_t)cols * 3);
    LF_HIP_CHECK(h, hipMemcpyAsync(h->d_frames, h->plug_in, need, hipMemcpyHostToDevice, h->stream));
    return LF_OK;
}

int lf::plugin_fetch_results(lf_handle* h)
{
    hipStream_t s = h->stream;
    const int eager = kPlugEager < 3 * h->cap_lines ? kPlugEager : 3 * h->cap_lines;
    const size_t need = (size_t)eager * 40 + 3 * h->P;
    if (h->plug_host.bytes < need) LF_HIP_CHECK(h, h->plug_host.alloc(need));
    h->plug_eager = eager;
    uint8_t* p = h->plug_host;
    LF_HIP_CHECK(h, hipMemcpyAsync(p, h->d_out.lines, (size_t)eager * 16, hipMemcpyDeviceToHost, s));
    LF_HIP_CHECK(h, hipMemcpyAsync(p + (size_t)eager * 16, h->d_normals64, (size_t)eager * 16, hipMemcpyDeviceToHost, s));
    LF_HIP_CHECK(h, hipMemcpyAsync(p + (size_t)eager * 32, h->d_centers, (size_t)eager * 8, hipMemcpyDeviceToHost, s));
    LF_HIP_CHECK(h, hipMemcpyAsync(p + (size_t)eager * 40, h->dbg_masks.p, 3 * h->P, hipMemcpyDeviceToHost, s));
    return LF_OK;
}

extern "C" int lf_set_image(lf_handle* h, const uint8_t* bgr, int rows, int cols, int row_stride_bytes)
{
    if (!h) return LF_ERR_NOT_INITIALISED;
    if (!bgr) { lf_set_error(h, LF_ERR_BAD_ARG, "lf_set_image: null image"); return LF_ERR_BAD_ARG; }
    if (rows != h->Hc || cols != h->W) { lf_set_error(h, LF_ERR_BAD_ARG, "lf_set_image: image is %dx%d, handle expects %dx%d", rows, cols, h->Hc, h->W); return LF_ERR_BAD_ARG; }
    if (row_stride_bytes < cols * 3) { lf_set_error(h, LF_ERR_BAD_ARG, "lf_set_image: row stride %d < %d", row_stride_bytes, cols * 3); return LF_ERR_BAD_ARG; }
    LF_HIP_CHECK(h, hipSetDevice(h->device));
    hipStream_t s = h->stream;
    h->plugin_ready = false;
    int rc = plugin_stage_image(h, bgr, rows, cols, row_stride_bytes);
    if (rc != LF_OK) return rc;
    for (int attempt = 0;; ++attempt) {
    rc = run_detect(h, h->d_frames, 1, true);
    if (rc != LF_OK) return rc;
    lf_segments dev = h->d_out;
    dev.desc = nullptr; dev.code = nullptr;
    rc = run_segments(h, 1, dev, false);
    if (rc != LF_OK) return rc;
    if ((rc = scratch(h, h->dbg_masks, 3 * h->P)) != LF_OK) return rc;
    launch_edges_u8(h->canny, 3, h->detector == LF_DETECTOR_DENSE ? h->d_bwbits.p : h->d_maskbits.p, (uint8_t*)h->dbg_masks.p, s);
    h->h_counts.resize(3); h->h_seg_offset.resize(4);
    if ((rc = plugin_fetch_results(h)) != LF_OK) return rc;
    LF_HIP_CHECK(h, hipMemcpyAsync(h->h_counts.data(), h->d_counts, 3 * sizeof(int), hipMemcpyDeviceToHost, s));
    LF_HIP_CHECK(h, hipMemcpyAsync(h->h_seg_offset.data(), h->d_seg_offset, 4 * sizeof(int), hipMemcpyDeviceToHost, s));
    LF_HIP_CHECK(h, hipMemcpyAsync(&h->h_pinned[6], h->lsd.d_overflow + 5, sizeof(int), hipMemcpyDeviceToHost, s));
    LF_HIP_CHECK(h, hipStreamSynchronize(s));
    if (h->h_pinned[6] <= h->lsd.params.rec_cap) break;
    if (attempt == 4) { lf_set_error(h, LF_ERR_CAPACITY, "the LSD lists keep overflowing (%d entries needed)", h->h_pinned[6]); return LF_ERR_CAPACITY; }
    if ((rc = h->lsd.grow_lists(h, h->h_pinned[6])) != LF_OK) return rc;
    }
    h->plugin_ready = true;
    return LF_OK;
}

extern "C" int lf_detect_lines(lf_handle* h, int color, float* lines4, double* normals2, float* centers2,
                               uint8_t* area_or_null, int cap, int* n_out)
{
    if (!h) return LF_ERR_NOT_INITIALISED;
    if (color < 0 || color > 2) { lf_set_error(h, LF_ERR_BAD_ARG, "Error: Undefined color strings..."); return LF_ERR_BAD_ARG; }
    if (!h->plugin_ready) { lf_set_error(h, LF_ERR_NOT_INITIALISED, "lf_detect_lines before lf_set_image"); return LF_ERR_NOT_INITIALISED; }
    if (!n_out) { lf_set_error(h, LF_ERR_BAD_ARG, "lf_detect_lines: n_out is null"); return LF_ERR_BAD_ARG; }
    LF_HIP_CHECK(h, hipSetDevice(h->device));
    hipStream_t s = h->stream;
    int n = h->h_counts[color];
    if (n > h->cap_lines) { lf_set_error(h, LF_ERR_CAPACITY, "%s found %d lines, max_lines_per_color is %d", detector_name(h->detector), n, h->cap_lines); return LF_ERR_CAPACITY; }
    if (n > cap) { lf_set_error(h, LF_ERR_CAPACITY, "%d lines exceed caller capacity %d", n, cap); return LF_ERR_CAPACITY; }
    const size_t off = (size_t)h->h_seg_offset[color];
    if (h->plug_host && off + (size_t)n <= (size_t)h->plug_eager) {
        const uint8_t* p = h->plug_host;
        const size_t e = (size_t)h->plug_eager;
        if (n > 0) {
            if (lines4) memcpy(lines4, p + off * 16, (size_t)n * 16);
            if (normals2) memcpy(normals2, p + e * 16 + off * 16, (size_t)n * 16);
            if (centers2) memcpy(centers2, p + e * 32 + off * 8, (size_t)n * 8);
        }
        if (area_or_null) memcpy(area_or_null, p + e * 40 + (size_t)color * h->P, h->P);
        *n_out = n;
        return LF_OK;
    }
    if (n > 0) {
        if (lines4) LF_HIP_CHECK(h, hipMemcpyAsync(lines4, h->d_out.lines + off * 4, (size_t)n * 4 * sizeof(float), hipMemcpyDeviceToHost, s));
        if (normals2) LF_HIP_CHECK(h, hipMemcpyAsync(normals2, h->d_normals64 + off * 2, (size_t)n * 2 * sizeof(double), hipMemcpyDeviceToHost, s));
        if (centers2) LF_HIP_CHECK(h, hipMemcpyAsync(centers2, h->d_centers + off * 2, (size_t)n * 2 * sizeof(float), hipMemcpyDeviceToHost, s));
    }
    if (area_or_null) LF_HIP_CHECK(h, hipMemcpyAsync(area_or_null, static_cast<uint8_t*>(h->dbg_masks.p) + (size_t)color * h->P, h->P, hipMemcpyDeviceToHost, s));
    LF_HIP_CHECK(h, hipStreamSynchronize(s));
    *n_out = n;
    return LF_OK;
}

extern "C" int lf_associate(lf_handle* h, const uint8_t* query32, int nq, const uint8_t* map32, int nm,
                            int32_t* idx, float* dist, int on_device)
{
    if (!h) return LF_ERR_NOT_INITIALISED;
    if (nq < 0 || nm < 0 || (nq > 0 && (!query32 || !idx || !dist)) || (nm > 0 && !map32)) { lf_set_error(h, LF_ERR_BAD_ARG, "lf_associate: bad argument"); return LF_ERR_BAD_ARG; }
    if (nm > (1 << 21)) { lf_set_error(h, LF_ERR_UNSUPPORTED, "map larger than 2^21 entries"); return LF_ERR_UNSUPPORTED; }
    if (nq == 0) return LF_OK;
    LF_HIP_CHECK(h, hipSetDevice(h->device));
    hipStream_t s = h->stream;
    if (nm == 0) {
        std::vector<int32_t> hi(nq, -1); std::vector<float> hd(nq, -1.f);
        if (on_device) {
            LF_HIP_CHECK(h, hipMemcpyAsync(idx, hi.data(), nq * sizeof(int32_t), hipMemcpyHostToDevice, s));
            LF_HIP_CHECK(h, hipMemcpyAsync(dist, hd.data(), nq * sizeof(float), hipMemcpyHostToDevice, s));
            LF_HIP_CHECK(h, hipStreamSynchronize(s));
        } else { memcpy(idx, hi.data(), nq * sizeof(int32_t)); memcpy(dist, hd.data(), nq * sizeof(float)); }
        return LF_OK;
    }
    const size_t nm_pad = assoc_rows_padded_m(nm);
    int rc;
    if ((rc = scratch(h, h->a_mx, nm_pad * 256)) != LF_OK) return rc;
    const bool ties = h->tie_rule == LF_TIE_MIHASHER;
    if (ties && (rc = scratch(h, h->a_best, (size_t)nq * 8)) != LF_OK) return rc;
    const uint8_t *dq = query32, *dmp = map32;
    int32_t* didx = idx; float* ddist = dist;
    if (!on_device) {
        if ((rc = scratch(h, h->a_q, (size_t)nq * 32)) || (rc = scratch(h, h->a_m, (size_t)nm * 32)) ||
            (rc = scratch(h, h->a_idx, (size_t)nq * 4)) || (rc = scratch(h, h->a_dist, (size_t)nq * 4))) return rc;
        LF_HIP_CHECK(h, hipMemcpyAsync(h->a_q.p, query32, (size_t)nq * 32, hipMemcpyHostToDevice, s));
        LF_HIP_CHECK(h, hipMemcpyAsync(h->a_m.p, map32, (size_t)nm * 32, hipMemcpyHostToDevice, s));
        dq = (const uint8_t*)h->a_q.p; dmp = (const uint8_t*)h->a_m.p; didx = (int32_t*)h->a_idx.p; ddist = (float*)h->a_dist.p;
    }
    {
        StageClock::Scope t(h, h->clock, ST_ASSOC);
        h->a_ws.tie_res = ties ? static_cast<unsigned long long*>(h->a_best.p) : nullptr;
        LF_HIP_CHECK(h, launch_assoc(dq, nq, dmp, nm, (int8_t*)h->a_mx.p, h->a_ws, didx, ddist, s));
        if (ties)
            LF_HIP_CHECK(h, launch_assoc_ties(dq, nullptr, nq, (const int8_t*)h->a_mx.p, dmp, nullptr, nm, nullptr, 0, h->a_ws,
                                              static_cast<unsigned long long*>(h->a_best.p), didx, ddist, s));
    }
    LF_HIP_CHECK(h, hipGetLastError());
    if (!on_device) {
        LF_HIP_CHECK(h, hipMemcpyAsync(idx, didx, (size_t)nq * 4, hipMemcpyDeviceToHost, s));
        LF_HIP_CHECK(h, hipMemcpyAsync(dist, ddist, (size_t)nq * 4, hipMemcpyDeviceToHost, s));
        LF_HIP_CHECK(h, hipStreamSynchronize(s));
    }
    return LF_OK;
}

extern "C" int lf_set_tie_rule(lf_handle* h, int tie_rule)
{
    if (!h) return LF_ERR_NOT_INITIALISED;
    if (tie_rule != LF_TIE_LOWEST && tie_rule != LF_TIE_MIHASHER) { lf_set_error(h, LF_ERR_BAD_ARG, "lf_set_tie_rule: unknown rule %d", tie_rule); return LF_ERR_BAD_ARG; }
    h->tie_rule = tie_rule;
    return LF_OK;
}

extern "C" int lf_associate_float(lf_handle* h, const float* query72, int nq, const float* map72, int nm,
                                  int32_t* idx, float* dist, int on_device)
{
    if (!h) return LF_ERR_NOT_INITIALISED;
    if (nq <= 0 || nm <= 0 || !query72 || !map72 || !idx || !dist) { lf_set_error(h, LF_ERR_BAD_ARG, "lf_associate_float: bad argument"); return LF_ERR_BAD_ARG; }
    LF_HIP_CHECK(h, hipSetDevice(h->device));
    hipStream_t s = h->stream;
    int rc;
    if ((rc = scratch(h, h->a_best, assoc_float_scratch_bytes(nq, nm))) || (rc = scratch(h, h->a_qn, (size_t)nq * 4)) || (rc = scratch(h, h->a_mn, (size_t)nm * 4))) return rc;
    const float *dq = query72, *dmp = map72;
    int32_t* didx = idx; float* ddist = dist;
    if (!on_device) {
        if ((rc = scratch(h, h->a_q, (size_t)nq * 288)) || (rc = scratch(h, h->a_m, (size_t)nm * 288)) ||
            (rc = scratch(h, h->a_idx, (size_t)nq * 4)) || (rc = scratch(h, h->a_dist, (size_t)nq * 4))) return rc;
        LF_HIP_CHECK(h, hipMemcpyAsync(h->a_q.p, query72, (size_t)nq * 288, hipMemcpyHostToDevice, s));
        LF_HIP_CHECK(h, hipMemcpyAsync(h->a_m.p, map72, (size_t)nm * 288, hipMemcpyHostToDevice, s));
        dq = (const float*)h->a_q.p; dmp = (const float*)h->a_m.p; didx = (int32_t*)h->a_idx.p; ddist = (float*)h->a_dist.p;
    }
    {
        StageClock::Scope t(h, h->clock, ST_ASSOC);
        LF_HIP_CHECK(h, launch_assoc_float(dq, nq, dmp, nm, (float*)h->a_qn.p, (float*)h->a_mn.p, h->a_best.p, didx, ddist, s));
    }
    LF_HIP_CHECK(h, hipGetLastError());
    if (!on_device) {
        LF_HIP_CHECK(h, hipMemcpyAsync(idx, didx, (size_t)nq * 4, hipMemcpyDeviceToHost, s));
        LF_HIP_CHECK(h, hipMemcpyAsync(dist, ddist, (size_t)nq * 4, hipMemcpyDeviceToHost, s));
        LF_HIP_CHECK(h, hipStreamSynchronize(s));
    }
    return LF_OK;
}

extern "C" int lf_select_queries(lf_handle* h, const uint8_t* query32, int nq, const uint8_t* mask, uint8_t* selected32, int32_t* query_idx,
                                 int* n_selected, int on_device)
{
    if (!h) return LF_ERR_NOT_INITIALISED;
    if (nq < 0 || !n_selected || (nq > 0 && (!query32 || !mask || !selected32 || !query_idx))) { lf_set_error(h, LF_ERR_BAD_ARG, "lf_select_queries: bad argument"); return LF_ERR_BAD_ARG; }
    *n_selected = 0;
    if (nq == 0) return LF_OK;
    LF_HIP_CHECK(h, hipSetDevice(h->device));
    hipStream_t s = h->stream;
    int rc;
    if ((rc = scratch(h, h->kn_total, 4 * sizeof(int))) != LF_OK) return rc;
    const uint8_t *dq = query32, *dmask = mask;
    uint8_t* dsel = selected32; int32_t* dqi = query_idx;
    if (!on_device) {
        if ((rc = scratch(h, h->a_q, (size_t)nq * 32)) || (rc = scratch(h, h->a_m, (size_t)nq * 33)) || (rc = scratch(h, h->a_idx, (size_t)nq * 4))) return rc;
        LF_HIP_CHECK(h, hipMemcpyAsync(h->a_q.p, query32, (size_t)nq * 32, hipMemcpyHostToDevice, s));
        uint8_t* m8 = static_cast<uint8_t*>(h->a_m.p) + (size_t)nq * 32;
        LF_HIP_CHECK(h, hipMemcpyAsync(m8, mask, (size_t)nq, hipMemcpyHostToDevice, s));
        dq = static_cast<const uint8_t*>(h->a_q.p); dmask = m8; dsel = static_cast<uint8_t*>(h->a_m.p); dqi = static_cast<int32_t*>(h->a_idx.p);
    }
    launch_select_queries(dq, dmask, nq, dsel, dqi, static_cast<int*>(h->kn_total.p), s);
    LF_HIP_CHECK(h, hipGetLastError());
    int n = 0;
    LF_HIP_CHECK(h, hipMemcpyAsync(&n, h->kn_total.p, sizeof(int), hipMemcpyDeviceToHost, s));
    LF_HIP_CHECK(h, hipStreamSynchronize(s));
    *n_selected = n;
    if (!on_device && n > 0) {
        LF_HIP_CHECK(h, hipMemcpyAsync(selected32, dsel, (size_t)n * 32, hipMemcpyDeviceToHost, s));
        LF_HIP_CHECK(h, hipMemcpyAsync(query_idx, dqi, (size_t)n * 4, hipMemcpyDeviceToHost, s));
        LF_HIP_CHECK(h, hipStreamSynchronize(s));
    }
    return LF_OK;
}

extern "C" int lf_knn_match(lf_handle* h, const uint8_t* query32, int nq, const uint8_t* map32, int nm, int k, int32_t* idx, float* dist,
                            int on_device)
{
    if (!h) return LF_ERR_NOT_INITIALISED;
    if (nq < 0 || nm < 0 || k < 1 || k > 16 || (nq > 0 && (!query32 || !idx || !dist)) || (nm > 0 && !map32)) {
        lf_set_error(h, LF_ERR_BAD_ARG, "lf_knn_match: bad argument (k must be 1..16)");
        return LF_ERR_BAD_ARG;
    }
    if (nm > (1 << 24)) { lf_set_error(h, LF_ERR_UNSUPPORTED, "lf_knn_match: map larger than 2^24 entries"); return LF_ERR_UNSUPPORTED; }
    if (nq == 0) return LF_OK;
    LF_HIP_CHECK(h, hipSetDevice(h->device));
    hipStream_t s = h->stream;
    int rc;
    const uint8_t *dq = query32, *dm_ = map32;
    int32_t* didx = idx; float* ddist = dist;
    const size_t out = (size_t)nq * k;
    if (!on_device) {
        if ((rc = scratch(h, h->a_q, (size_t)nq * 32)) || (rc = scratch(h, h->a_m, (size_t)(nm > 0 ? nm : 1) * 32)) ||
            (rc = scratch(h, h->a_idx, out * 4)) || (rc = scratch(h, h->a_dist, out * 4))) return rc;
        LF_HIP_CHECK(h, hipMemcpyAsync(h->a_q.p, query32, (size_t)nq * 32, hipMemcpyHostToDevice, s));
        if (nm > 0) LF_HIP_CHECK(h, hipMemcpyAsync(h->a_m.p, map32, (size_t)nm * 32, hipMemcpyHostToDevice, s));
        dq = (const uint8_t*)h->a_q.p; dm_ = (const uint8_t*)h->a_m.p; didx = (int32_t*)h->a_idx.p; ddist = (float*)h->a_dist.p;
    }
    { StageClock::Scope t(h, h->clock, ST_ASSOC); launch_knn(dq, nq, dm_, nm, k, 128, h->tie_rule == LF_TIE_MIHASHER, didx, ddist, s); }
    LF_HIP_CHECK(h, hipGetLastError());
    if (!on_device) {
        LF_HIP_CHECK(h, hipMemcpyAsync(idx, didx, out * 4, hipMemcpyDeviceToHost, s));
        LF_HIP_CHECK(h, hipMemcpyAsync(dist, ddist, out * 4, hipMemcpyDeviceToHost, s));
        LF_HIP_CHECK(h, hipStreamSynchronize(s));
    }
    return LF_OK;
}

extern "C" int lf_radius_match(lf_handle* h, const uint8_t* query32, int nq, const uint8_t* map32, int nm, float max_distance,
                               int32_t* offsets, int32_t* idx, float* dist, int cap, int* total_out, int on_device)
{
    if (!h) return LF_ERR_NOT_INITIALISED;
    if (nq < 0 || nm < 0 || cap < 0 || !offsets || (cap > 0 && (!idx || !dist)) || (nq > 0 && !query32) || (nm > 0 && !map32) || !(max_distance >= 0)) {
        lf_set_error(h, LF_ERR_BAD_ARG, "lf_radius_match: bad argument");
        return LF_ERR_BAD_ARG;
    }
    if (nm > (1 << 24)) { lf_set_error(h, LF_ERR_UNSUPPORTED, "lf_radius_match: map larger than 2^24 entries"); return LF_ERR_UNSUPPORTED; }
    int md = max_distance >= 128.f ? 128 : (int)max_distance;
    LF_HIP_CHECK(h, hipSetDevice(h->device));
    hipStream_t s = h->stream;
    if (nq == 0) { if (on_device) LF_HIP_CHECK(h, hipMemsetAsync(offsets, 0, sizeof(int32_t), s)); else offsets[0] = 0; if (total_out) *total_out = 0; return LF_OK; }
    int rc;
    if ((rc = scratch(h, h->kn_hist, (size_t)nq * 129 * 4)) || (rc = scratch(h, h->kn_count, (size_t)nq * 4)) || (rc = scratch(h, h->kn_off, (size_t)(nq + 1) * 4)) ||
        (rc = scratch(h, h->kn_total, 16))) return rc;
    const uint8_t *dq = query32, *dm_ = map32;
    int32_t *doff = offsets, *didx = idx; float* ddist = dist;
    if (!on_device) {
        if ((rc = scratch(h, h->a_q, (size_t)nq * 32)) || (rc = scratch(h, h->a_m, (size_t)(nm > 0 ? nm : 1) * 32)) ||
            (rc = scratch(h, h->a_idx, (size_t)(cap > 0 ? cap : 1) * 4)) || (rc = scratch(h, h->a_dist, (size_t)(cap > 0 ? cap : 1) * 4))) return rc;
        LF_HIP_CHECK(h, hipMemcpyAsync(h->a_q.p, query32, (size_t)nq * 32, hipMemcpyHostToDevice, s));
        if (nm > 0) LF_HIP_CHECK(h, hipMemcpyAsync(h->a_m.p, map32, (size_t)nm * 32, hipMemcpyHostToDevice, s));
        dq = (const uint8_t*)h->a_q.p; dm_ = (const uint8_t*)h->a_m.p; doff = (int32_t*)h->kn_off.p; didx = (int32_t*)h->a_idx.p; ddist = (float*)h->a_dist.p;
    }
    {
        StageClock::Scope t(h, h->clock, ST_ASSOC);
        launch_radius(dq, nq, dm_, nm, md, (int32_t*)h->kn_hist.p, (int32_t*)h->kn_count.p, doff, (int*)h->kn_total.p, cap, h->tie_rule == LF_TIE_MIHASHER, didx, ddist, s);
    }
    LF_HIP_CHECK(h, hipGetLastError());
    int total = 0;
    LF_HIP_CHECK(h, hipMemcpyAsync(&total, h->kn_total.p, sizeof(int), hipMemcpyDeviceToHost, s));
    if (!on_device) LF_HIP_CHECK(h, hipMemcpyAsync(offsets, doff, (size_t)(nq + 1) * 4, hipMemcpyDeviceToHost, s));
    LF_HIP_CHECK(h, hipStreamSynchronize(s));
    if (total_out) *total_out = total;
    if (total > cap) { lf_set_error(h, LF_ERR_CAPACITY, "lf_radius_match: %d matches exceed the capacity %d (offsets are complete: size the arrays from them)", total, cap); return LF_ERR_CAPACITY; }
    if (!on_device && total > 0) {
        LF_HIP_CHECK(h, hipMemcpyAsync(idx, didx, (size_t)total * 4, hipMemcpyDeviceToHost, s));
        LF_HIP_CHECK(h, hipMemcpyAsync(dist, ddist, (size_t)total * 4, hipMemcpyDeviceToHost, s));
        LF_HIP_CHECK(h, hipStreamSynchronize(s));
    }
    return LF_OK;
}

extern "C" int lf_kmeans(lf_handle* h, const uint8_t* bgr_points, int n, int on_device, int k, const double* init_centers, int max_iter,
                         double tol, double* centers_out, long long* counts_out, double* inertia_out, int* n_iter_out)
{
    if (!h) return LF_ERR_NOT_INITIALISED;
    if (!bgr_points || !init_centers || !centers_out || !counts_out || n < 1 || k < 1 || k > 16 || max_iter < 1) {
        lf_set_error(h, LF_ERR_BAD_ARG, "lf_kmeans: null argument, n < 1, max_iter < 1 or k outside 1..16");
        return LF_ERR_BAD_ARG;
    }
    if (n > (1 << 24)) {
        lf_set_error(h, LF_ERR_UNSUPPORTED, "lf_kmeans: more than 2^24 points (%d) are not supported", n);
        return LF_ERR_UNSUPPORTED;
    }
    LF_HIP_CHECK(h, hipSetDevice(h->device));
    hipStream_t s = h->stream;
    int rc;
    if ((rc = scratch(h, h->km_lab, (size_t)n)) || (rc = scratch(h, h->km_f64, 128 * sizeof(double))) || (rc = scratch(h, h->km_cnt, 32 * sizeof(long long)))) return rc;
    const uint8_t* dp = bgr_points;
    if (!on_device) {
        if ((rc = scratch(h, h->km_pts, (size_t)n * 3)) != LF_OK) return rc;
        LF_HIP_CHECK(h, hipMemcpyAsync(h->km_pts.p, bgr_points, (size_t)n * 3, hipMemcpyHostToDevice, s));
        dp = static_cast<const uint8_t*>(h->km_pts.p);
    }
    double* f64 = static_cast<double*>(h->km_f64.p);
    long long* cnt = static_cast<long long*>(h->km_cnt.p);
    int* status = reinterpret_cast<int*>(cnt + 16);
    LF_HIP_CHECK(h, hipMemcpyAsync(f64, init_centers, (size_t)k * 3 * sizeof(double), hipMemcpyHostToDevice, s));
    launch_kmeans(dp, n, k, f64, max_iter, tol, static_cast<uint8_t*>(h->km_lab.p), f64 + 64, cnt, status, s);
    LF_HIP_CHECK(h, hipGetLastError());
    double res[49];
    long long hc[17];
    LF_HIP_CHECK(h, hipMemcpyAsync(res, f64 + 64, (size_t)(3 * k + 1) * sizeof(double), hipMemcpyDeviceToHost, s));
    LF_HIP_CHECK(h, hipMemcpyAsync(hc, cnt, 17 * sizeof(long long), hipMemcpyDeviceToHost, s));
    LF_HIP_CHECK(h, hipStreamSynchronize(s));
    const int iters = *reinterpret_cast<int*>(&hc[16]);
    if (iters < 0) { lf_set_error(h, LF_ERR_BAD_ARG, "lf_kmeans: a cluster stayed empty (fewer distinct samples than clusters)"); return LF_ERR_BAD_ARG; }
    for (int j = 0; j < 3 * k; ++j) centers_out[j] = res[j];
    for (int j = 0; j < k; ++j) counts_out[j] = hc[j];
    if (inertia_out) *inertia_out = res[3 * k];
    if (n_iter_out) *n_iter_out = iters;
    return LF_OK;
}

extern "C" int lf_lsd_list_capacity(const lf_handle* h, int* entries, int* grown)
{
    if (!h) return LF_ERR_NOT_INITIALISED;
    if (entries) *entries = h->lsd.params.rec_cap;
    if (grown) *grown = h->lsd.lists_grown;
    return LF_OK;
}

extern "C" int lf_lsd_scratch_stride(const lf_handle* h)
{
    if (!h) return LF_ERR_NOT_INITIALISED;
    return (int)lsd_grow_reg_stride(h->lsd.params);
}

extern "C" int lf_suggested_depth(const lf_handle* h)
{
    if (!h) return LF_ERR_NOT_INITIALISED;
    return h->lsd.grow_lds_level == 0 && !h->lsd.grow_mixed ? 8 : 18;
}

extern "C" int lf_debug_std_sort(lf_handle* h, const int32_t* keys, int n, int32_t* order)
{
    if (!h) return LF_ERR_NOT_INITIALISED;
    if (!keys || !order || n < 1 || n >= (1 << 20)) { lf_set_error(h, LF_ERR_BAD_ARG, "lf_debug_std_sort: bad argument (1 <= n < 2^20)"); return LF_ERR_BAD_ARG; }
    LF_HIP_CHECK(h, hipSetDevice(h->device));
    hipStream_t s = h->stream;
    std::vector<uint32_t> e((size_t)n);
    for (int i = 0; i < n; ++i) {
        if (keys[i] < 0 || keys[i] > 1023) { lf_set_error(h, LF_ERR_BAD_ARG, "lf_debug_std_sort: keys must be in [0, 1023]"); return LF_ERR_BAD_ARG; }
        e[i] = ((uint32_t)keys[i] << 20) | (uint32_t)(i + 1);
    }
    int rc;
    const size_t words = std_sort_debug_words(n);
    if ((rc = scratch(h, h->a_q, (size_t)n * 4)) || (rc = scratch(h, h->a_m, words * 4)) || (rc = scratch(h, h->a_best, 64))) return rc;
    LF_HIP_CHECK(h, hipMemcpyAsync(h->a_q.p, e.data(), (size_t)n * 4, hipMemcpyHostToDevice, s));
    launch_std_sort_debug(static_cast<const uint32_t*>(h->a_q.p), static_cast<uint32_t*>(h->a_m.p), n, static_cast<int*>(h->a_best.p), s);
    LF_HIP_CHECK(h, hipGetLastError());
    int cnt = 0;
    LF_HIP_CHECK(h, hipMemcpyAsync(&cnt, h->a_best.p, sizeof(int), hipMemcpyDeviceToHost, s));
    LF_HIP_CHECK(h, hipStreamSynchronize(s));
    const size_t cap = words / 12;
    if (cnt > 0) LF_HIP_CHECK(h, hipMemcpy(e.data(), static_cast<uint32_t*>(h->a_m.p) + 4 * cap, (size_t)cnt * 4, hipMemcpyDeviceToHost));
    for (int i = 0; i < cnt; ++i) order[i] = (int32_t)(e[i] & 0xfffffu);
    {
        int k = cnt;
        for (int i = 0; i < n; ++i) if (keys[i] == 0) order[k++] = i;
    }
    return LF_OK;
}

extern "C" int lf_debug_lsd_binary(lf_handle* h, const uint8_t* img, int rows, int cols, float* lines4, int cap, int* n_out)
{
    if (!h) return LF_ERR_NOT_INITIALISED;
    if (!img || !lines4 || !n_out || rows != h->Hc || cols != h->W) { lf_set_error(h, LF_ERR_BAD_ARG, "lf_debug_lsd_binary: bad argument (image must be %dx%d)", h->Hc, h->W); return LF_ERR_BAD_ARG; }
    LF_HIP_CHECK(h, hipSetDevice(h->device));
    hipStream_t s = h->stream;
    if ((size_t)h->lsd.params.rec_cap < h->lsd.Ps) {
        LF_HIP_CHECK(h, hipStreamSynchronize(s));
        const int rc = h->lsd.grow_lists(h, (int)h->lsd.Ps);
        if (rc != LF_OK) return rc;
    }
    const size_t nw = (size_t)h->Hc * h->Ww;
    std::vector<uint32_t> bits(nw, 0u), ones(nw * 3, 0xffffffffu);
    for (int y = 0; y < rows; ++y)
        for (int x = 0; x < cols; ++x)
            if (img[(size_t)y * cols + x]) bits[(size_t)y * h->Ww + (x >> 5)] |= 1u << (x & 31);
    LF_HIP_CHECK(h, hipMemcpyAsync(h->d_strong, bits.data(), nw * 4, hipMemcpyHostToDevice, s));
    LF_HIP_CHECK(h, hipMemcpyAsync(h->d_maskbits, ones.data(), nw * 12, hipMemcpyHostToDevice, s));
    LF_HIP_CHECK(h, hipMemsetAsync(h->lsd.d_maxgrad, 0, 3 * sizeof(unsigned long long), s));
    h->lsd.grad(1, h->d_strong, h->d_maskbits, false, s);
    h->lsd.order(1, 0, s);
    h->lsd.label(1, false, s);
    h->lsd.grow(1, h->d_slot_lines, h->d_counts, kGrowLdsKb[h->lsd.grow_lds_level], true, false, s);
    LF_HIP_CHECK(h, hipGetLastError());
    int n = 0;
    LF_HIP_CHECK(h, hipMemcpyAsync(&n, h->d_counts, sizeof(int), hipMemcpyDeviceToHost, s));
    LF_HIP_CHECK(h, hipStreamSynchronize(s));
    h->last_frames = 1;
    h->plugin_ready = false;
    *n_out = n;
    if (n > h->cap_lines) { lf_set_error(h, LF_ERR_CAPACITY, "LSD found %d lines, max_lines_per_color is %d", n, h->cap_lines); return LF_ERR_CAPACITY; }
    if (n > cap) { lf_set_error(h, LF_ERR_CAPACITY, "%d lines exceed caller capacity %d", n, cap); return LF_ERR_CAPACITY; }
    if (n > 0) LF_HIP_CHECK(h, hipMemcpy(lines4, h->d_slot_lines, (size_t)n * 4 * sizeof(float), hipMemcpyDeviceToHost));
    return LF_OK;
}

extern "C" int lf_lsd_size(const lf_handle* h, int* rows, int* cols)
{
    if (!h || !rows || !cols) return LF_ERR_BAD_ARG;
    *rows = h->lsd.params.Hs; *cols = h->lsd.params.Ws;
    return LF_OK;
}

extern "C" int lf_debug_fetch(lf_handle* h, int buffer_id, void* dst, size_t bytes)
{
    if (!h) return LF_ERR_NOT_INITIALISED;
    if (!dst) { lf_set_error(h, LF_ERR_BAD_ARG, "lf_debug_fetch: null dst"); return LF_ERR_BAD_ARG; }
    LF_HIP_CHECK(h, hipSetDevice(h->device));
    hipStream_t s = h->stream;
    const size_t n = (size_t)h->last_frames;
    const void* src = nullptr;
    size_t avail = 0;
    switch (buffer_id) {
    case LF_BUF_BGR: {
        int rc = scratch(h, h->dbg_bgr, n * h->P * 3);
        if (rc != LF_OK) return rc;
        launch_bgrx_to_bgr((int)(n * h->P), h->d_bgr, (uint8_t*)h->dbg_bgr.p, s);
        src = h->dbg_bgr.p; avail = n * h->P * 3; break;
    }
    case LF_BUF_MASKS: {
        int rc = scratch(h, h->dbg_masks, n * 3 * h->P);
        if (rc != LF_OK) return rc;
        launch_edges_u8(h->canny, (int)(n * 3), h->d_maskbits, (uint8_t*)h->dbg_masks.p, s);
        src = h->dbg_masks.p; avail = n * 3 * h->P; break;
    }
    case LF_BUF_EDGES:
        launch_edges_u8(h->canny, (int)n, h->d_strong, h->d_edges_u8, s);
        src = h->d_edges_u8; avail = n * h->P; break;
    case LF_BUF_LSD_ANGLE:
    case LF_BUF_LSD_MODGRAD: {
        const LsdState& L = h->lsd;
        int rc = scratch(h, h->dbg_ang, n * 3 * L.Ps * sizeof(float));
        if (rc == LF_OK) rc = scratch(h, h->dbg_mod, n * 3 * L.Ps * sizeof(double));
        if (rc != LF_OK) return rc;
        launch_lsd_dense_debug(L.params, (int)n, L.d_norder, L.d_cxy, L.d_cdeg, L.d_cmod, (float*)h->dbg_ang.p, (double*)h->dbg_mod.p, s);
        if (buffer_id == LF_BUF_LSD_ANGLE) { src = h->dbg_ang.p; avail = n * 3 * L.Ps * sizeof(float); }
        else { src = h->dbg_mod.p; avail = n * 3 * L.Ps * sizeof(double); }
        break;
    }
    case LF_BUF_LSD_ORDER: {
        const size_t row = h->lsd.Ps * sizeof(uint32_t), have = (size_t)h->lsd.params.rec_cap * sizeof(uint32_t);
        if (bytes > n * 3 * row) { lf_set_error(h, LF_ERR_CAPACITY, "buffer %d holds %zu bytes, %zu requested", buffer_id, n * 3 * row, bytes); return LF_ERR_CAPACITY; }
        LF_HIP_CHECK(h, hipMemcpy2DAsync(dst, row, h->lsd.d_order_a, have, have, bytes / row, hipMemcpyDeviceToHost, s));
        LF_HIP_CHECK(h, hipStreamSynchronize(s));
        return LF_OK;
    }
    case LF_BUF_LSD_NORDER: src = h->lsd.d_norder; avail = n * 3 * sizeof(int); break;
    case LF_BUF_LBD_DX:
    case LF_BUF_LBD_DY: {
        int rc = scratch(h, h->dbg_dx, n * h->P * sizeof(int16_t));
        if (rc == LF_OK) rc = scratch(h, h->dbg_dy, n * h->P * sizeof(int16_t));
        if (rc != LF_OK) return rc;
        launch_lbd_split_debug(n * h->P, h->d_dxy, (int16_t*)h->dbg_dx.p, (int16_t*)h->dbg_dy.p, s);
        src = buffer_id == LF_BUF_LBD_DX ? h->dbg_dx.p : h->dbg_dy.p;
        avail = n * h->P * sizeof(int16_t);
        break;
    }
    case LF_BUF_LSD_COUNTS: src = h->d_counts; avail = n * 3 * sizeof(int); break;
    case LF_BUF_LSD_NLOW:
        if (!h->lsd.d_nlow) { memset(dst, 0, bytes < n * 3 * sizeof(int) ? bytes : n * 3 * sizeof(int)); return LF_OK; }
        src = h->lsd.d_nlow; avail = n * 3 * sizeof(int); break;
    case LF_BUF_LSD_SCRATCH: src = h->lsd.d_reg; avail = n * 3 * lsd_grow_reg_stride(h->lsd.params) * sizeof(uint32_t); break;
    default: lf_set_error(h, LF_ERR_BAD_ARG, "unknown buffer id %d", buffer_id); return LF_ERR_BAD_ARG;
    }
    if (bytes > avail) { lf_set_error(h, LF_ERR_CAPACITY, "buffer %d holds %zu bytes, %zu requested", buffer_id, avail, bytes); return LF_ERR_CAPACITY; }
    LF_HIP_CHECK(h, hipMemcpyAsync(dst, src, bytes, hipMemcpyDeviceToHost, s));
    LF_HIP_CHECK(h, hipStreamSynchronize(s));
    return LF_OK;
}

extern "C" int lf_set_profiling(lf_handle* h, int enabled)
{
    if (!h) return LF_ERR_NOT_INITIALISED;
    h->profiling = enabled != 0;
    if (h->profiling) {
        (void)hipSetDevice(h->device);
        h->clock.prefill(1024);
    }
    return LF_OK;
}

extern "C" int lf_reset_timing(lf_handle* h)
{
    if (!h) return LF_ERR_NOT_INITIALISED;
    h->clock.take(nullptr, nullptr, 0);
    return LF_OK;
}

extern "C" int lf_get_timing(lf_handle* h, double* ms_per_stage, int32_t* launches_per_stage, int n)
{
    if (!h) return LF_ERR_NOT_INITIALISED;
    h->clock.resolve();
    for (int i = 0; i < n && i < LF_N_STAGES; ++i) {
        if (ms_per_stage) ms_per_stage[i] = h->clock.ms[i];
        if (launches_per_stage) launches_per_stage[i] = h->clock.launches[i];
    }
    return LF_OK;
}

extern "C" int lf_jpeg_info(const uint8_t* jpeg, size_t jpeg_size, int* rows, int* cols, int* components, int* hmax, int* vmax)
{
    if (!jpeg) return LF_ERR_BAD_ARG;
    return lf::jpeg::peek(jpeg, jpeg_size, rows, cols, components, hmax, vmax);
}

extern "C" int lf_frames_buffer(lf_handle* h, uint8_t** device_ptr, size_t* bytes)
{
    if (!h) return LF_ERR_NOT_INITIALISED;
    if (device_ptr) *device_ptr = h->d_frames;
    if (bytes) *bytes = h->frames_bytes;
    return LF_OK;
}

extern "C" int lf_jpeg_decode_batch(lf_handle* h, const uint8_t* const* jpeg, const size_t* jpeg_size, int n_frames,
                                    int rows, int cols, uint8_t* frames, int frames_on_device, int n_threads,
                                    int* frame_status)
{
    if (!h) return LF_ERR_NOT_INITIALISED;
    if (!jpeg || !jpeg_size || !frames || n_frames < 1 || rows < 1 || cols < 1 || rows > 65535 || cols > 65535) {
        lf_set_error(h, LF_ERR_BAD_ARG, "lf_jpeg_decode_batch: null argument, n_frames < 1 or bad size %dx%d", rows, cols);
        return LF_ERR_BAD_ARG;
    }
    if (n_frames > 65535) { lf_set_error(h, LF_ERR_CAPACITY, "lf_jpeg_decode_batch: at most 65535 frames per call"); return LF_ERR_CAPACITY; }
    if (frames_on_device && frames == h->d_frames &&
        (size_t)n_frames * rows * cols * 3 > h->frames_bytes) {
        lf_set_error(h, LF_ERR_CAPACITY, "lf_jpeg_decode_batch: %d frames of %dx%d do not fit the handle's frame buffer (%d of %dx%d)",
                     n_frames, rows, cols, h->max_frames, h->cfg.in_rows, h->cfg.in_cols);
        return LF_ERR_CAPACITY;
    }
    LF_HIP_CHECK(h, hipSetDevice(h->device));
    if (!h->jpeg) {
        h->jpeg.reset(new (std::nothrow) JpegState());
        if (!h->jpeg) { lf_set_error(h, LF_ERR_HIP, "out of host memory"); return LF_ERR_HIP; }
        LF_HIP_CHECK(h, hipEventCreateWithFlags(&h->jpeg->staged, hipEventDisableTiming));
    }
    JpegState& J = *h->jpeg;
    hipStream_t s = h->stream;
    static const bool trace = getenv("LF_JPEG_TRACE") != nullptr;
    auto now = [] { return std::chrono::steady_clock::now(); };
    auto ms_since = [](std::chrono::steady_clock::time_point a) { return std::chrono::duration<double, std::milli>(std::chrono::steady_clock::now() - a).count(); };
    const auto t_begin = now();
    double t_decode = 0, t_wait = 0, t_pack = 0;
    if ((int)J.frames.size() < n_frames) J.frames.resize((size_t)n_frames);

    int nt = n_threads > 0 ? n_threads : (n_frames < 64 ? n_frames : 64);
    if (nt > n_frames) nt = n_frames;
    {
        std::atomic<int> next(0);
        J.pool.run(nt, [&](int) {
            for (;;) {
                const int i = next.fetch_add(1);
                if (i >= n_frames) break;
                lf::jpeg::FrameCoefs& fc = J.frames[(size_t)i];
                if (!jpeg[i]) { fc.status = LF_ERR_BAD_ARG; fc.hdr.valid = 0; fc.hdr.nblocks = 0; fc.n_entries = 0; continue; }
                (void)lf::jpeg::decode_coefficients(jpeg[i], jpeg_size[i], fc, rows, cols);
                if (fc.status != LF_OK) { fc.hdr.valid = 0; fc.hdr.nblocks = 0; fc.n_entries = 0; }
            }
        });
    }
    t_decode = ms_since(t_begin);
    size_t total_entries = 0, total_blocks = 0;
    int max_blocks = 0, n_failed = 0, first_error = LF_OK;
    for (int i = 0; i < n_frames; ++i) {
        lf::jpeg::FrameCoefs& fc = J.frames[(size_t)i];
        if (frame_status) frame_status[i] = fc.status;
        if (fc.status != LF_OK) { ++n_failed; if (first_error == LF_OK) first_error = fc.status; }
        fc.hdr.entry_base = (uint32_t)total_entries;
        fc.hdr.block_base = (uint32_t)total_blocks;
        total_entries += fc.n_entries;
        total_blocks += (size_t)fc.hdr.nblocks;
        if (fc.hdr.nblocks > max_blocks) max_blocks = fc.hdr.nblocks;
    }
    if (total_entries >= (1ull << 32) || total_blocks >= (1ull << 32)) { lf_set_error(h, LF_ERR_CAPACITY, "batch too large"); return LF_ERR_CAPACITY; }
    const size_t hdr_bytes = (size_t)n_frames * sizeof(lf::jpeg::FrameHeader);
    const size_t blk_bytes = (total_blocks + 1) * sizeof(uint32_t);
    const size_t ent_bytes = (total_entries + 1) * sizeof(uint32_t);
    const size_t off_blk = (hdr_bytes + 255) & ~(size_t)255, off_ent = (off_blk + blk_bytes + 255) & ~(size_t)255;
    const size_t stage_bytes = off_ent + ent_bytes;
    const auto t_w = now();
    if (J.staged_pending) { LF_HIP_CHECK(h, hipEventSynchronize(J.staged)); J.staged_pending = false; }
    t_wait = ms_since(t_w);
    if (J.h_stage.bytes < stage_bytes) LF_HIP_CHECK(h, J.h_stage.alloc(stage_bytes + stage_bytes / 4 + 4096));
    const auto t_p = now();
    {
        uint8_t* st = static_cast<uint8_t*>(J.h_stage.p);
        std::atomic<int> next(0);
        J.pool.run(nt, [&](int) {
            for (;;) {
                const int i = next.fetch_add(1);
                if (i >= n_frames) break;
                const lf::jpeg::FrameCoefs& fc = J.frames[(size_t)i];
                memcpy(st + (size_t)i * sizeof(lf::jpeg::FrameHeader), &fc.hdr, sizeof(lf::jpeg::FrameHeader));
                if (fc.hdr.nblocks) memcpy(st + off_blk + (size_t)fc.hdr.block_base * 4, fc.block_end.data(), (size_t)fc.hdr.nblocks * 4);
                if (fc.n_entries) memcpy(st + off_ent + (size_t)fc.hdr.entry_base * 4, fc.entries.data(), fc.n_entries * 4);
            }
        });
    }
    t_pack = ms_since(t_p);
    JpegGeom g;
    g.rows = rows; g.cols = cols;
    g.Wp = (cols + 15) / 16 * 16;
    g.Hp = (rows + 15) / 16 * 16;
    int rc;
    if ((rc = scratch(h, J.planes, (size_t)n_frames * 3 * g.Wp * g.Hp)) != LF_OK) return rc;
    if ((rc = scratch(h, J.hdrs, stage_bytes)) != LF_OK) return rc;
    uint8_t* d_stage = static_cast<uint8_t*>(J.hdrs.p);
    LF_HIP_CHECK(h, hipMemcpyAsync(d_stage, J.h_stage, stage_bytes, hipMemcpyHostToDevice, s));
    LF_HIP_CHECK(h, hipEventRecord(J.staged, s));
    J.staged_pending = true;
    uint8_t* d_out = frames;
    const size_t out_bytes = (size_t)n_frames * rows * cols * 3;
    if (!frames_on_device) {
        if ((rc = scratch(h, J.out, out_bytes)) != LF_OK) return rc;
        d_out = static_cast<uint8_t*>(J.out.p);
    }
    {
        StageClock::Scope t(h, h->clock, ST_JPEG);
        launch_jpeg_decode(g, n_frames, max_blocks, reinterpret_cast<const lf::jpeg::FrameHeader*>(d_stage),
                           reinterpret_cast<const uint32_t*>(d_stage + off_ent), reinterpret_cast<const uint32_t*>(d_stage + off_blk),
                           static_cast<uint8_t*>(J.planes.p), d_out, s);
    }
    LF_HIP_CHECK(h, hipGetLastError());
    if (!frames_on_device) {
        LF_HIP_CHECK(h, hipMemcpyAsync(frames, d_out, out_bytes, hipMemcpyDeviceToHost, s));
        LF_HIP_CHECK(h, hipStreamSynchronize(s));
        J.staged_pending = false;
    }
    if (trace)
        fprintf(stderr, "lf_jpeg_decode_batch: %d frames, %d threads: decode %.2f ms, wait %.2f, pack %.2f (%.1f MB), total host %.2f ms\n",
                n_frames, nt, t_decode, t_wait, t_pack, stage_bytes / 1e6, ms_since(t_begin));
    if (n_failed && !frame_status) {
        lf_set_error(h, first_error, "%d of %d JPEG streams could not be decoded (first status %d)", n_failed, n_frames, first_error);
        return LF_ERR_DECODE;
    }
    return LF_OK;
}

extern "C" int lf_serialize_segments(lf_handle* h, const lf_segments* segs, int segs_on_device, int n_frames, int stage,
                                     uint8_t* out, size_t out_capacity, int out_on_device, int64_t* frame_byte_offset)
{
    if (!h) return LF_ERR_NOT_INITIALISED;
    if (!segs || !out || !frame_byte_offset || n_frames < 1 || stage < LF_MSG_DETECTOR || stage > LF_MSG_FILTERED || !segs->frame_offset || !segs->color) {
        lf_set_error(h, LF_ERR_BAD_ARG, "lf_serialize_segments: null argument, n_frames < 1 or unknown stage");
        return LF_ERR_BAD_ARG;
    }
    if (stage == LF_MSG_DETECTOR ? (!segs->pixels_normalized || !segs->normals) : (!segs->ground || (stage == LF_MSG_FILTERED && !segs->keep))) {
        lf_set_error(h, LF_ERR_BAD_ARG, "lf_serialize_segments: the arrays of stage %d are missing", stage);
        return LF_ERR_BAD_ARG;
    }
    LF_HIP_CHECK(h, hipSetDevice(h->device));
    hipStream_t s = h->stream;
    const int* d_fo = segs->frame_offset;
    const uint8_t* d_color = segs->color;
    const float* d_pn = segs->pixels_normalized;
    const float* d_nm = segs->normals;
    const double* d_gr = segs->ground;
    const uint8_t* d_keep = segs->keep;
    int rc;
    if (!segs_on_device) {
        const int total = segs->frame_offset[n_frames];
        if (total < 0) { lf_set_error(h, LF_ERR_BAD_ARG, "negative segment count"); return LF_ERR_BAD_ARG; }
        const size_t n = (size_t)total;
        if ((rc = scratch(h, h->m_fo, (size_t)(n_frames + 1) * sizeof(int))) != LF_OK) return rc;
        if ((rc = scratch(h, h->m_color, n + 1)) != LF_OK) return rc;
        LF_HIP_CHECK(h, hipMemcpyAsync(h->m_fo.p, segs->frame_offset, (size_t)(n_frames + 1) * sizeof(int), hipMemcpyHostToDevice, s));
        LF_HIP_CHECK(h, hipMemcpyAsync(h->m_color.p, segs->color, n, hipMemcpyHostToDevice, s));
        d_fo = static_cast<const int*>(h->m_fo.p);
        d_color = static_cast<const uint8_t*>(h->m_color.p);
        if (stage == LF_MSG_DETECTOR) {
            if ((rc = scratch(h, h->m_pn, n * 16 + 16)) != LF_OK) return rc;
            if ((rc = scratch(h, h->m_nm, n * 8 + 8)) != LF_OK) return rc;
            LF_HIP_CHECK(h, hipMemcpyAsync(h->m_pn.p, segs->pixels_normalized, n * 16, hipMemcpyHostToDevice, s));
            LF_HIP_CHECK(h, hipMemcpyAsync(h->m_nm.p, segs->normals, n * 8, hipMemcpyHostToDevice, s));
            d_pn = static_cast<const float*>(h->m_pn.p);
            d_nm = static_cast<const float*>(h->m_nm.p);
        } else {
            if ((rc = scratch(h, h->m_gr, n * 32 + 32)) != LF_OK) return rc;
            LF_HIP_CHECK(h, hipMemcpyAsync(h->m_gr.p, segs->ground, n * 32, hipMemcpyHostToDevice, s));
            d_gr = static_cast<const double*>(h->m_gr.p);
            if (stage == LF_MSG_FILTERED) {
                if ((rc = scratch(h, h->m_keep, n + 1)) != LF_OK) return rc;
                LF_HIP_CHECK(h, hipMemcpyAsync(h->m_keep.p, segs->keep, n, hipMemcpyHostToDevice, s));
                d_keep = static_cast<const uint8_t*>(h->m_keep.p);
            }
        }
    }
    if ((rc = scratch(h, h->m_counts, (size_t)n_frames * sizeof(int))) != LF_OK) return rc;
    if ((rc = scratch(h, h->m_boff, (size_t)(n_frames + 1) * sizeof(long long))) != LF_OK) return rc;
    launch_msg_layout(n_frames, stage, d_fo, d_keep, static_cast<int*>(h->m_counts.p), static_cast<long long*>(h->m_boff.p), s);
    static_assert(sizeof(long long) == sizeof(int64_t), "byte offsets are int64");
    LF_HIP_CHECK(h, hipMemcpyAsync(frame_byte_offset, h->m_boff.p, (size_t)(n_frames + 1) * sizeof(long long), hipMemcpyDeviceToHost, s));
    LF_HIP_CHECK(h, hipStreamSynchronize(s));
    const size_t need = (size_t)frame_byte_offset[n_frames];
    if (need > out_capacity) {
        lf_set_error(h, LF_ERR_CAPACITY, "lf_serialize_segments: %zu bytes needed, %zu available", need, out_capacity);
        return LF_ERR_CAPACITY;
    }
    uint8_t* d_out = out;
    if (!out_on_device) {
        if ((rc = scratch(h, h->m_body, need + 16)) != LF_OK) return rc;
        d_out = static_cast<uint8_t*>(h->m_body.p);
    }
    launch_msg_write(n_frames, stage, d_fo, d_color, d_pn, d_nm, d_gr, d_keep, static_cast<const int*>(h->m_counts.p),
                     static_cast<const long long*>(h->m_boff.p), d_out, s);
    LF_HIP_CHECK(h, hipGetLastError());
    if (!out_on_device) {
        LF_HIP_CHECK(h, hipMemcpyAsync(out, d_out, need, hipMemcpyDeviceToHost, s));
        LF_HIP_CHECK(h, hipStreamSynchronize(s));
    }
    return LF_OK;
}

extern "C" int lf_deserialize_segments(lf_handle* h, const uint8_t* bodies, int bodies_on_device, const int64_t* frame_byte_offset,
                                       int n_frames, lf_segments* out, int out_on_device, int* n_segments)
{
    if (!h) return LF_ERR_NOT_INITIALISED;
    if (!bodies || !frame_byte_offset || !out || n_frames < 1 || !out->frame_offset) {
        lf_set_error(h, LF_ERR_BAD_ARG, "lf_deserialize_segments: null argument or n_frames < 1");
        return LF_ERR_BAD_ARG;
    }
    for (int f = 0; f < n_frames; ++f)
        if (frame_byte_offset[f + 1] < frame_byte_offset[f] + 4) { lf_set_error(h, LF_ERR_DECODE, "body %d is shorter than its count field", f); return LF_ERR_DECODE; }
    LF_HIP_CHECK(h, hipSetDevice(h->device));
    hipStream_t s = h->stream;
    const size_t bytes = (size_t)frame_byte_offset[n_frames];
    const size_t max_segs = bytes / 73 + 1;
    int rc;
    const uint8_t* d_body = bodies;
    if (!bodies_on_device) {
        if ((rc = scratch(h, h->m_body, bytes + 16)) != LF_OK) return rc;
        LF_HIP_CHECK(h, hipMemcpyAsync(h->m_body.p, bodies, bytes, hipMemcpyHostToDevice, s));
        d_body = static_cast<const uint8_t*>(h->m_body.p);
    }
    if ((rc = scratch(h, h->m_boff, (size_t)(n_frames + 1) * sizeof(long long))) != LF_OK) return rc;
    if ((rc = scratch(h, h->m_bad, sizeof(int))) != LF_OK) return rc;
    LF_HIP_CHECK(h, hipMemcpyAsync(h->m_boff.p, frame_byte_offset, (size_t)(n_frames + 1) * sizeof(long long), hipMemcpyHostToDevice, s));
    LF_HIP_CHECK(h, hipMemsetAsync(h->m_bad.p, 0, sizeof(int), s));
    lf_segments dev = *out;
    if (!out_on_device) {
        if ((rc = scratch(h, h->m_fo, (size_t)(n_frames + 1) * sizeof(int))) != LF_OK) return rc;
        dev.frame_offset = static_cast<int32_t*>(h->m_fo.p);
        dev.color = nullptr; dev.pixels_normalized = nullptr; dev.normals = nullptr; dev.ground = nullptr;
        if (out->color) { if ((rc = scratch(h, h->m_color, max_segs)) != LF_OK) return rc; dev.color = static_cast<uint8_t*>(h->m_color.p); }
        if (out->pixels_normalized) { if ((rc = scratch(h, h->m_pn, max_segs * 16)) != LF_OK) return rc; dev.pixels_normalized = static_cast<float*>(h->m_pn.p); }
        if (out->normals) { if ((rc = scratch(h, h->m_nm, max_segs * 8)) != LF_OK) return rc; dev.normals = static_cast<float*>(h->m_nm.p); }
        if (out->ground) { if ((rc = scratch(h, h->m_gr, max_segs * 32)) != LF_OK) return rc; dev.ground = static_cast<double*>(h->m_gr.p); }
    }
    const int cap = out->capacity;
    launch_msg_read(n_frames, cap, d_body, static_cast<const long long*>(h->m_boff.p), dev.frame_offset, static_cast<int*>(h->m_bad.p),
                    dev.color, dev.pixels_normalized, dev.normals, dev.ground, s);
    LF_HIP_CHECK(h, hipGetLastError());
    int bad = 0, total = 0;
    LF_HIP_CHECK(h, hipMemcpyAsync(&bad, h->m_bad.p, sizeof(int), hipMemcpyDeviceToHost, s));
    LF_HIP_CHECK(h, hipMemcpyAsync(&total, dev.frame_offset + n_frames, sizeof(int), hipMemcpyDeviceToHost, s));
    LF_HIP_CHECK(h, hipStreamSynchronize(s));
    if (n_segments) *n_segments = total;
    if (bad) { lf_set_error(h, LF_ERR_DECODE, "a SegmentList body's count does not match its length"); return LF_ERR_DECODE; }
    if (total > cap) { lf_set_error(h, LF_ERR_CAPACITY, "%d segments exceed the output capacity %d", total, cap); return LF_ERR_CAPACITY; }
    if (!out_on_device) {
        const size_t n = (size_t)total;
        LF_HIP_CHECK(h, hipMemcpyAsync(out->frame_offset, dev.frame_offset, (size_t)(n_frames + 1) * sizeof(int), hipMemcpyDeviceToHost, s));
        if (out->color && n) LF_HIP_CHECK(h, hipMemcpyAsync(out->color, dev.color, n, hipMemcpyDeviceToHost, s));
        if (out->pixels_normalized && n) LF_HIP_CHECK(h, hipMemcpyAsync(out->pixels_normalized, dev.pixels_normalized, n * 16, hipMemcpyDeviceToHost, s));
        if (out->normals && n) LF_HIP_CHECK(h, hipMemcpyAsync(out->normals, dev.normals, n * 8, hipMemcpyDeviceToHost, s));
        if (out->ground && n) LF_HIP_CHECK(h, hipMemcpyAsync(out->ground, dev.ground, n * 32, hipMemcpyDeviceToHost, s));
        LF_HIP_CHECK(h, hipStreamSynchronize(s));
    }
    return LF_OK;
}
```

lane_slam_amd/csrc/lanefront_handle.h:

```cpp
#pragma once
#include <stdio.h>
#include <stdlib.h>
#include <string.h>
#include <memory>
#include <utility>
#include <vector>
#include "lanefront_core.h"
#include "jpeg_entropy.h"
#include "k_edlines_types.h"
#include "k_hough.h"
#include "k_jenc.h"
#include "k_rectify.h"

namespace lf {

struct JpegState {
    lf::jpeg::WorkerPool pool;
    std::vector<lf::jpeg::FrameCoefs> frames;
    int rows = 0, cols = 0, max_frames = 0;
    DevBuf planes, entries, block_end, hdrs, out;
    DevBuf gh_clean, gh_sub, gh_seg, gh_info, gh_coef;
    std::vector<int> h_status;
    HostArray<void> h_stage;
    hipEvent_t staged = nullptr;
    bool staged_pending = false;
    HostArray<int> h_status_pinned;
    int status_frames = 0;
    hipEvent_t status_done = nullptr;
    ~JpegState()
    {
        if (staged) (void)hipEventDestroy(staged);
        if (status_done) (void)hipEventDestroy(status_done);
    }
};

struct JencState {
    DevBuf tab, in, coef, bits, dcdiff, total, bitbuf, ff, out, sizes;
    HostArray<jenc::Tables> h_tab;
    HostArray<uint32_t> h_sizes;
    int rows = 0, cols = 0, quality = 0;
    CallClock clock{jenc::kStages};
};

struct RectState {
    DevBuf xy, frac, tab;
    DevBuf in, out;
    int w = 0, h = 0;
    bool map_ready = false;
    int maps_built = 0;
    CallClock clock{rect::kStages};
};

struct KlArrays {
    DevBuf start_end, in_octave, angle, num_pixels, line_length, octave, class_id, response, size, pt, salience, desc, code, frame;
    int stage(lf_handle* h, const lf_keylines& out, bool describe, lf_keylines* dev);
    int all(lf_handle* h, int capacity, KlOut* ko);
    static int copy_back(lf_handle* h, const lf_keylines& dev, const lf_keylines& out, int n, int n_frames);
};

struct KlBatch {
    DevBuf frame_count, frame_offset, totals, line_frame;
    DevBuf gray, masks;
    KlArrays staged;
    HostArray<int> h_pinned;
    int alloc(lf_handle* h);
    int images(lf_handle* h, const uint8_t* images, int n, int input_kind, int on_device, const uint8_t** d);
    int upload(lf_handle* h, DevBuf& buf, const uint8_t* planes, int n, const uint8_t** d);
    int keylines(lf_handle* h, const char* who, const lf_keylines& out, int on_device, int describe, lf_keylines* dev);
};

int kl_batch_check(lf_handle* h, const char* who, const uint8_t* images, const lf_keylines* out, int n_frames, int n_octaves, int input_kind);
KlOut kl_out(const lf_keylines& k, int32_t* frame);

struct KlOctave {
    int W = 0, H = 0, cap = 0, max_edges = 0, max_lines = 0;
    bool marks_in_lds = false;
    bool aflags_on = false;
    DevBuf src, blur, dxy, g, anchors, part, chain, sid, gmarks, counts, l_ep, l_c, l_dir, l_npx, l_sal, tl, rs_tab, ework;
    DevBuf aflags;
};

struct KlState {
    int n_octaves = 0;
    KlOctave oct[LF_MAX_OCTAVES];
    KlBatch batch;
    DevBuf status, big;
    DevBuf m_fo, m_totals, m_erased, m_kept;
    KlArrays unmasked;
    DevBuf any_tmp, any_blur;
    DevBuf d_frame, d_io, d_angle, d_npx, d_oct, d_desc, d_code, d_n;
    size_t lds_bytes = 0;
    int last_octaves = 0, last_frames = 0;
};

struct LsdState {
    LsdParams params;
    ResizeTables rt{};
    int seed_order = LF_LSD_SEED_OPENCV30, max_frames = 0;
    size_t Ps = 0;
    int max_nsx = 0, max_nsy = 0;
    int label_items_full = 0;
    DevArray<int> d_xofs, d_y0, d_y1;
    DevArray<float> d_xa, d_yb;
    DevArray<uint32_t> d_raddr, d_order_a, d_order_b, d_cxy, d_reg, d_laddr;
    DevArray<float> d_rdeg, d_cdeg, d_rsd, d_csd;
    DevArray<double> d_rmod, d_rcs, d_rsn, d_cmod, d_ccs, d_lmod;
    DevArray<unsigned long long> d_sort_a, d_sort_b;
    DevArray<uint16_t> d_clabel, d_comp_list;
    double* d_csn = nullptr;
    DevArray<uint32_t> d_tile_list, d_gused;
    DevArray<int> d_row_start, d_norder, d_comp_count, d_comp_key, d_perm;
    DevArray<float> d_tmp_lines;
    DevArray<int> d_tmp_tags;
    DevArray<uint8_t> d_zero; size_t zero_bytes = 0;
    unsigned long long* d_maxgrad = nullptr;
    int *d_nrec = nullptr, *d_nlow = nullptr, *d_tile_count = nullptr, *d_overflow = nullptr;
    int lists_grown = 0;
    bool lists_lost = false;
    bool grow_mixed = false;
    int grow_lds_level = 0;
    int env_lds_level = -1;
    int env_mixed = -1;
    int env_bitmap = 1;

    int init(lf_handle* h, int Hc, int W, const lf_lsd_options& o, int seed_order, int max_frames, int cap_lines);
    int alloc_lists(lf_handle* h, int rec_cap);
    void free_lists();
    int grow_lists(lf_handle* h, int need);
    void adapt_slice(int over_small, int over_medium, int problems);
    void grad(int n, const uint32_t* edge_bits, const uint32_t* mask_bits, bool counters_zeroed, hipStream_t s);
    void grad_gray(int n, const uint8_t* gray, hipStream_t s);
    void order(int n, int big, hipStream_t s);
    void label(int n, bool rank, hipStream_t s);
    void grow(int n, float* lines, int* counts, int lds_kb, bool mixed, bool use_perm, hipStream_t s);
};

struct LsdKlLevel {
    LsdState lsd;
    DevArray<float> lines;
    DevArray<int> counts;
    lf_lsd_options opts{};
    bool ready = false;
};

struct LsdKlState {
    LsdKlLevel level[LF_MAX_OCTAVES];
    DevBuf pyr[LF_MAX_OCTAVES];
    KlBatch batch;
};

struct MatcherState {
    DevBuf codes;
    std::vector<std::pair<int, int> > index_map;
    int num_images = 0;
    int total = 0;
    DevBuf q, idx, dist, off;
};

}

struct lf_handle : lf::Core {
    lf_config cfg;
    int max_frames = 0, cap_lines = 0;
    int Hc = 0, W = 0, Ww = 0;
    size_t P = 0;
    lf_descriptor_params desc_params = { 1, 7, 2, 5 };
    lf::PreParams pre;
    lf::CannyParams canny;
    lf::LsdState lsd;
    lf::SegParams seg;
    lf::DevArray<uint8_t> d_frames, d_edges_u8;
    lf::DevBuf dbg_masks;
    size_t frames_bytes = 0;
    lf::DevArray<uint32_t> d_bgr;
    lf::DevArray<uint8_t> d_gray;
    lf::DevBuf dbg_bgr;
    lf::DevArray<uint32_t> d_strong, d_weak, d_maskbits;
    lf::DevArray<int> d_sdiv, d_hdiv;
    bool overflow_zeroed = false;
    lf::DevBuf dbg_ang, dbg_mod;
    lf::DevArray<int> d_counts, d_seg_offset, d_frame_offset;
    lf::DevArray<float> d_slot_lines;
    lf::DevArray<int> d_seg_frame;
    lf::DevArray<uint32_t> d_dxy;
    lf::DevBuf dbg_dx, dbg_dy;
    lf::DevArray<float> d_gauss_g, d_gauss_l;
    lf_segments d_out;
    lf::DevArray<float> out_lines, out_normals, out_pixels_normalized;
    lf::DevArray<uint8_t> out_color, out_keep, out_code;
    lf::DevArray<double> out_ground;
    lf::DevArray<float> out_desc;
    lf::DevArray<double> d_normals64;
    lf::DevArray<float> d_centers;
    int out_capacity = 0;
    lf::DevBuf a_q, a_m, a_mx, a_best, a_idx, a_dist, a_qn, a_mn;
    lf::DevBuf km_pts, km_lab, km_f64, km_cnt;
    lf::DevBuf ai_strip, ai_lab, ai_fit, ai_out;
    lf::DevBuf dr_img, dr_fo, dr_lines, dr_color, dr_bad;
    int draw_frames = 0;
    lf::DevBuf kn_hist, kn_count, kn_off, kn_total;
    lf::AssocScratch a_ws;
    std::unique_ptr<lf::MatcherState> matcher;
    lf::HostArray<int> h_pinned;
    const uint8_t* pend_in = nullptr; int pend_n = 0; lf_segments pend_out; bool pend_describe = false;
    int last_frames = 0;
    bool plugin_ready = false;
    bool pending = false;
    lf::HostArray<uint8_t> plug_host, plug_in;
    int plug_eager = 0;
    bool pending_keylines = false;
    int detector = LF_DETECTOR_LSD;
    lf_edlines_params ed_params;
    int detector_failures = 0;
    lf_hough_params hough_params = { 2, 3, 1, 1.0, 3.14159265358979323846 / 180 };
    lf::DevArray<lf::HoughTables> d_hough_tab;
    lf::DevArray<int> d_hough_acc;
    lf::DevArray<uint32_t> d_hough_nz;
    lf::HoughParams hough_p{};
    int hough_slots = 0;
    lf_dense_params dense_params = { 40.0 };
    lf::DevArray<uint32_t> d_bwbits;
    lf::DevArray<float> d_dense_rec;
    lf::SegMode slot_mode = lf::SEG_FLOAT;
    int tie_rule = LF_TIE_MIHASHER;
    int env_kl_lds_lines = 0;
    int pending_problems = 0;
    int pending_capacity = 0;
    std::vector<int> h_counts, h_seg_offset;
    std::unique_ptr<lf::JpegState> jpeg;
    std::unique_ptr<lf::JencState> jenc;
    std::unique_ptr<lf::RectState> rect;
    std::unique_ptr<lf::KlState> kl;
    std::unique_ptr<lf::LsdKlState> lsdkl;
    lf::DevBuf m_fo, m_color, m_pn, m_nm, m_gr, m_keep, m_counts, m_boff, m_body, m_bad;
    lf::StageClock clock{LF_N_STAGES, 8192, true};
};

namespace lf {

inline bool alloc_trace() { static const bool on = [] { const char* e = getenv("LF_ALLOC_TRACE"); return e && *e && *e != '0'; }(); return on; }
template <typename T>
inline int dalloc_(lf_handle* h, DevArray<T>* p, size_t count, const char* what)
{
    const size_t bytes = count ? count * sizeof(T) : sizeof(T);
    LF_HIP_CHECK(h, p->alloc(bytes));
    if (alloc_trace()) fprintf(stderr, "lanefront alloc %-28s %12zu B\n", what, bytes);
    return LF_OK;
}
#define dalloc(h, p, count) dalloc_(h, p, count, #p)

inline void seg_camera(lf_handle* h)
{
    const lf_config& c = h->cfg;
    SegParams& S = h->seg;
    S.cw = (double)c.cam_w; S.ch = (double)c.cam_h;
    memcpy(S.K, c.K, sizeof(S.K)); memcpy(S.D, c.D, sizeof(S.D));
    for (int i = 0; i < 3; ++i)
        for (int j = 0; j < 3; ++j) {
            double s = 0;
            for (int t = 0; t < 3; ++t) s += c.P[4 * i + t] * c.R[3 * t + j];
            S.RR[3 * i + j] = s;
        }
}

int run_detect(lf_handle* h, const uint8_t* d_frames, int n, bool from_working_image);
int run_segments(lf_handle* h, int n, lf_segments dev_out, bool describe);
int plugin_stage_image(lf_handle* h, const uint8_t* bgr, int rows, int cols, int row_stride_bytes);
int plugin_fetch_results(lf_handle* h);
int hough_prepare(lf_handle* h);
int dense_prepare(lf_handle* h);
int run_detect_edlines(lf_handle* h, const uint8_t* d_frames, int n);
void keylines_pending_result(lf_handle* h, int* total, int* overflow);

}
```

lane_slam_amd/csrc/lanefront_lsd.hip:

```cpp
#include <string.h>
#include <math.h>
#include <vector>
#include "lanefront_handle.h"
#include "lsd_bitplane.h"

namespace lf {

int LsdState::init(lf_handle* h, int Hc, int W, const lf_lsd_options& o, int seed_order_, int max_frames_, int cap_lines)
{
    seed_order = seed_order_;
    max_frames = max_frames_;
    LsdParams& L = params;
    memset(&L, 0, sizeof(L));
    L.Hc = Hc; L.W = W; L.Ww = (W + 31) / 32;
    L.scaled = o.scale != 1.0;
    L.scale = o.scale;
    if (o.scale <= 0 || o.scale > 1.0) { lf_set_error(h, LF_ERR_UNSUPPORTED, "lsd_scale must be in (0,1]"); return LF_ERR_UNSUPPORTED; }
    if (L.scaled) { L.Ws = dm::round_half_even(W * o.scale); L.Hs = dm::round_half_even(Hc * o.scale); }
    else { L.Ws = W; L.Hs = Hc; }
    const int Hs = L.Hs, Ws = L.Ws;
    Ps = (size_t)Hs * Ws;
    if (Ps >= (1u << 20) || L.Ws > 65535 || L.Hs > 65535) { lf_set_error(h, LF_ERR_UNSUPPORTED, "scaled LSD image too large"); return LF_ERR_UNSUPPORTED; }
    if ((size_t)((L.Hs + 2) & ~1) * 4 + 512 * 4 + 1024 > 64 * 1024) { lf_set_error(h, LF_ERR_UNSUPPORTED, "scaled LSD image has %d rows: the row table exceeds the LDS of one problem", L.Hs); return LF_ERR_UNSUPPORTED; }
    if (o.n_bins < 2 || o.n_bins > 4096) { lf_set_error(h, LF_ERR_UNSUPPORTED, "lsd_n_bins must be in [2,4096] (a seed is its bin above a 20-bit pixel index in one word)"); return LF_ERR_UNSUPPORTED; }
    if (L.scaled) {
        const double sigma = (o.scale < 1) ? (o.sigma_scale / o.scale) : o.sigma_scale;
        const double sprec = 3;
        const unsigned hh = (unsigned)ceil(sigma * sqrt(2 * sprec * dm::dlog(10.0)));
        const int n = 1 + 2 * (int)hh;
        if (n > kMaxGaussTaps) { lf_set_error(h, LF_ERR_UNSUPPORTED, "LSD Gaussian needs %d taps (max %d)", n, kMaxGaussTaps); return LF_ERR_UNSUPPORTED; }
        const double scale2X = -0.5 / (sigma * sigma);
        double sum = 0;
        for (int i = 0; i < n; ++i) { double x = i - (n - 1) * 0.5; double t = dm::dexp(scale2X * x * x); L.k[i] = t; sum += t; }
        sum = 1.0 / sum;
        for (int i = 0; i < n; ++i) L.k[i] *= sum;
        L.ntaps = n; L.half = n / 2;
    } else { L.ntaps = 1; L.half = 0; L.k[0] = 1.0; }
    L.prec = 3.14159265358979323846 * o.ang_th / 180;
    L.p = o.ang_th / 180;
    L.rho = o.quant / dm::dsin(L.prec);
    L.log_nt = 5 * (dm::dlog10((double)L.Ws) + dm::dlog10((double)L.Hs)) / 2 + dm::dlog10(11.0);
    L.min_reg_size = (int)(-L.log_nt / dm::dlog10(L.p));
    L.log_eps = o.log_eps; L.density_th = o.density_th;
    L.n_bins = o.n_bins; L.refine = o.refine; L.cap_lines = cap_lines;
    if (seed_order != LF_LSD_SEED_OPENCV30 && seed_order != LF_LSD_SEED_OPENCV32) { lf_set_error(h, LF_ERR_BAD_ARG, "lsd_seed_order %d: LF_LSD_SEED_OPENCV30 or LF_LSD_SEED_OPENCV32", seed_order); return LF_ERR_BAD_ARG; }
    if (seed_order == LF_LSD_SEED_OPENCV32 && !lsd_seed32_supported(L)) { lf_set_error(h, LF_ERR_UNSUPPORTED, "lsd_seed_order OPENCV32: the %dx%d LSD image exceeds the row tables of the sort emulation, or (n_bins - 1) * quant / sin(ang_th) < 361 (k_lsd_seed32.hip)", L.Ws, L.Hs); return LF_ERR_UNSUPPORTED; }
    L.label_lds = kLabelLds;
    {
        const size_t plane = bitplane_lds_words(Ps) * 4;
        if (plane <= 150 * 1024 && plane / 4 > (size_t)L.label_lds) L.label_lds = (int)((plane / 4 < 65534 ? plane / 4 : 65534) & ~(size_t)1);
    }
    L.label_items = (int)(Ps / 3 / 1024) * 1024;
    if (L.label_items > 64512) L.label_items = 64512;
    if (L.label_items < kLabelItems) L.label_items = kLabelItems;
    L.label_items_max = L.label_items;
    label_items_full = L.label_items;
    L.rec_cap = (int)Ps;
    std::vector<int> xofs(Ws), y0(Hs), y1(Hs);
    std::vector<float> xa(2 * (size_t)Ws), yb(2 * (size_t)Hs);
    int xmax = Ws;
    const double scale_x = 1.0 / L.scale, scale_y = 1.0 / L.scale;
    for (int dx = 0; dx < Ws; ++dx) {
        float fx; int sx;
        if (L.scaled) {
            fx = (float)((dx + 0.5) * scale_x - 0.5);
            sx = dm::ifloor((double)fx);
            fx -= sx;
        } else { fx = 0.f; sx = dx; }
        if (sx < 0) { fx = 0; sx = 0; }
        if (sx + 1 >= W) {
            if (dx < xmax) xmax = dx;
            if (sx >= W - 1) { fx = 0; sx = W - 1; }
        }
        xofs[dx] = sx; xa[2 * dx] = 1.f - fx; xa[2 * dx + 1] = fx;
    }
    for (int dy = 0; dy < Hs; ++dy) {
        float fy; int sy;
        if (L.scaled) {
            fy = (float)((dy + 0.5) * scale_y - 0.5);
            sy = dm::ifloor((double)fy);
            fy -= sy;
        } else { fy = 0.f; sy = dy; }
        yb[2 * dy] = 1.f - fy; yb[2 * dy + 1] = fy;
        y0[dy] = sy < 0 ? 0 : (sy > Hc - 1 ? Hc - 1 : sy);
        y1[dy] = sy + 1 < 0 ? 0 : (sy + 1 > Hc - 1 ? Hc - 1 : sy + 1);
    }
    const int GT = 32;
    int mx = 0, my = 0;
    for (int X0 = 0; X0 < Ws; X0 += GT) {
        int X1 = X0 + GT < Ws - 1 ? X0 + GT : Ws - 1;
        int lo = xofs[X0], hi = xofs[X1] + 1 < W - 1 ? xofs[X1] + 1 : W - 1;
        if (hi - lo + 1 > mx) mx = hi - lo + 1;
    }
    for (int Y0 = 0; Y0 < Hs; Y0 += GT) {
        int Y1 = Y0 + GT < Hs - 1 ? Y0 + GT : Hs - 1;
        int lo = y0[Y0], hi = y1[Y1];
        if (hi - lo + 1 > my) my = hi - lo + 1;
    }
    max_nsx = mx; max_nsy = my;
    {
        const int hh = L.half;
        const size_t szF = (size_t)(my + 2 * hh) * mx, szBl = (size_t)my * mx;
        const size_t szHb = (size_t)my * (GT + 1), szSc = (size_t)(GT + 1) * (GT + 1);
        size_t regA = szF > szHb ? szF : szHb;
        if (regA < (size_t)2 * GT * GT) regA = (size_t)2 * GT * GT;
        const size_t regB = szBl > szSc ? szBl : szSc;
        size_t lds = sizeof(double) * (regA + regB);
        if (lds > 64 * 1024) { lf_set_error(h, LF_ERR_UNSUPPORTED, "lsd_scale %.3f needs %zu B of LDS per tile (max 65536)", L.scale, lds); return LF_ERR_UNSUPPORTED; }
    }
    if (dalloc(h, &d_xofs, Ws) || dalloc(h, &d_y0, Hs) || dalloc(h, &d_y1, Hs) || dalloc(h, &d_xa, 2 * (size_t)Ws) || dalloc(h, &d_yb, 2 * (size_t)Hs))
        return LF_ERR_HIP;
    LF_HIP_CHECK(h, hipMemcpy(d_xofs, xofs.data(), Ws * sizeof(int), hipMemcpyHostToDevice));
    LF_HIP_CHECK(h, hipMemcpy(d_y0, y0.data(), Hs * sizeof(int), hipMemcpyHostToDevice));
    LF_HIP_CHECK(h, hipMemcpy(d_y1, y1.data(), Hs * sizeof(int), hipMemcpyHostToDevice));
    LF_HIP_CHECK(h, hipMemcpy(d_xa, xa.data(), 2 * (size_t)Ws * sizeof(float), hipMemcpyHostToDevice));
    LF_HIP_CHECK(h, hipMemcpy(d_yb, yb.data(), 2 * (size_t)Hs * sizeof(float), hipMemcpyHostToDevice));
    rt.xofs = d_xofs; rt.xa = d_xa; rt.y0 = d_y0; rt.y1 = d_y1; rt.yb = d_yb; rt.xmax = xmax;
    const size_t nprob = (size_t)max_frames * 3, cap = nprob * (size_t)cap_lines;
    if (dalloc(h, &d_tile_list, nprob * (size_t)(((Ws + 31) / 32) * ((Hs + 31) / 32))) ||
        dalloc(h, &d_gused, nprob * ((Ps + 31) / 32)) || dalloc(h, &d_row_start, nprob * (size_t)(Hs + 1)) ||
        dalloc(h, &d_comp_list, nprob * (size_t)kCompCap) || dalloc(h, &d_comp_count, nprob) || dalloc(h, &d_perm, nprob) || dalloc(h, &d_comp_key, nprob) ||
        dalloc(h, &d_tmp_lines, cap * 4) || dalloc(h, &d_tmp_tags, cap) || dalloc(h, &d_norder, nprob))
        return LF_ERR_HIP;
    zero_bytes = nprob * 8 + nprob * 4 + nprob * 4 + 16 + 32;
    if (dalloc(h, &d_zero, zero_bytes)) return LF_ERR_HIP;
    d_maxgrad = reinterpret_cast<unsigned long long*>(d_zero.p);
    d_nrec = reinterpret_cast<int*>(d_zero + nprob * 8);
    int* nlow = d_nrec + nprob;
    if (seed_order == LF_LSD_SEED_OPENCV32) d_nlow = nlow;
    d_tile_count = nlow + nprob;
    d_overflow = d_tile_count + 4;
    LF_HIP_CHECK(h, hipMemset(d_zero, 0, zero_bytes));
    if (const char* ev = getenv("LF_GROW_LDS_LEVEL")) { const int v = atoi(ev); env_lds_level = v < 0 ? 0 : (v > 2 ? 2 : v); }
    if (const char* ev = getenv("LF_GROW_MIXED")) env_mixed = atoi(ev) != 0 ? 1 : 0;
    if (const char* ev = getenv("LF_GROW_BITMAP")) { const int v = atoi(ev); env_bitmap = v < 0 ? 0 : v; }
    return LF_OK;
}

void LsdState::free_lists()
{
    for (auto* b : { &d_raddr, &d_order_a, &d_order_b, &d_cxy, &d_reg, &d_laddr }) b->reset();
    for (auto* b : { &d_rdeg, &d_cdeg, &d_rsd, &d_csd }) b->reset();
    for (auto* b : { &d_rmod, &d_rcs, &d_rsn, &d_cmod, &d_ccs, &d_lmod }) b->reset();
    d_sort_a.reset(); d_sort_b.reset(); d_clabel.reset();
    params.r_sd = nullptr; params.c_sd = nullptr; d_csn = nullptr;
}

int LsdState::alloc_lists(lf_handle* h, int rec_cap)
{
    const size_t nprob = (size_t)max_frames * 3, S = (size_t)rec_cap;
    LsdParams& L = params;
    L.rec_cap = rec_cap;
    const int li = rec_cap > kLabelItems ? rec_cap : kLabelItems;
    L.label_items = label_items_full < li ? label_items_full : li;
    L.label_items_max = L.label_items;
    if (dalloc(h, &d_raddr, nprob * S) || dalloc(h, &d_rdeg, nprob * S) || dalloc(h, &d_rmod, nprob * S) ||
        dalloc(h, &d_rcs, nprob * S) || dalloc(h, &d_rsn, nprob * S) || dalloc(h, &d_sort_a, nprob * S) || dalloc(h, &d_sort_b, nprob * S) ||
        dalloc(h, &d_order_a, nprob * S) || dalloc(h, &d_order_b, nprob * S) || dalloc(h, &d_cxy, nprob * S) || dalloc(h, &d_cdeg, nprob * S) ||
        dalloc(h, &d_cmod, nprob * S) || dalloc(h, &d_ccs, nprob * S * 2) || dalloc(h, &d_reg, nprob * lsd_grow_reg_stride(L)) ||
        dalloc(h, &d_clabel, nprob * S))
        return LF_ERR_HIP;
    d_csn = d_ccs + 1;
    if (dalloc(h, &d_rsd, nprob * S * 2) || dalloc(h, &d_csd, nprob * S * 2)) return LF_ERR_HIP;
    L.r_sd = d_rsd; L.c_sd = d_csd;
    if (seed_order == LF_LSD_SEED_OPENCV32 && (dalloc(h, &d_laddr, nprob * S) || dalloc(h, &d_lmod, nprob * S)))
        return LF_ERR_HIP;
    return LF_OK;
}

int LsdState::grow_lists(lf_handle* h, int need)
{
    size_t cap = ((size_t)need + (size_t)need / 4 + 4095) / 4096 * 4096;
    if (cap > Ps) cap = Ps;
    if (alloc_trace()) fprintf(stderr, "lanefront: a problem needs %d list entries, the handle holds %d: growing to %zu\n", need, params.rec_cap, cap);
    const int old_cap = params.rec_cap;
    free_lists();
    int rc = alloc_lists(h, (int)cap);
    if (rc == LF_OK) { ++lists_grown; lists_lost = false; return LF_OK; }
    free_lists();
    if (alloc_lists(h, old_cap) != LF_OK) { free_lists(); params.rec_cap = old_cap; lists_lost = true; }
    lf_set_error(h, LF_ERR_HIP, "out of device memory growing the LSD lists from %d to %zu entries per problem%s", old_cap, cap,
                 lists_lost ? "; the lists are gone: the handle refuses detection" : "; the handle keeps its old lists");
    return LF_ERR_HIP;
}

void LsdState::adapt_slice(int over_small, int over_medium, int problems)
{
    grow_lds_level = over_medium * 4 > problems ? 2 : (over_small * 20 > problems ? 1 : 0);
    grow_mixed = (grow_lds_level == 0 ? over_small : over_medium) * 100 > problems;
}

void LsdState::grad(int n, const uint32_t* edge_bits, const uint32_t* mask_bits, bool counters_zeroed, hipStream_t s)
{
    launch_lsd_grad(params, rt, n, edge_bits, mask_bits, d_raddr, d_rdeg, d_rmod, d_rcs, d_rsn, d_nrec, d_maxgrad, max_nsx, max_nsy,
                    d_tile_list, d_tile_count, d_laddr, d_lmod, d_nlow, d_overflow + 5, counters_zeroed, s);
}

void LsdState::grad_gray(int n, const uint8_t* gray, hipStream_t s)
{
    launch_lsd_grad_gray(params, rt, n, gray, d_raddr, d_rdeg, d_rmod, d_rcs, d_rsn, d_nrec, d_maxgrad, max_nsx, max_nsy,
                         d_tile_list, d_tile_count, d_laddr, d_lmod, d_nlow, s);
}

void LsdState::order(int n, int big, hipStream_t s)
{
    launch_lsd_order(params, n, d_raddr, d_rdeg, d_rmod, d_rcs, d_rsn, d_nrec, d_maxgrad, d_sort_a, d_sort_b, d_order_a, d_order_b,
                     d_norder, d_cxy, d_cdeg, d_cmod, d_ccs, d_csn, d_row_start, s);
    if (seed_order == LF_LSD_SEED_OPENCV32)
        launch_lsd_seed32(params, n, d_nrec, d_norder, d_overflow + 5, d_maxgrad, d_cxy, d_cmod, d_laddr, d_lmod, d_nlow, d_sort_a, d_sort_b,
                          d_order_a, d_order_b, big, s);
}

void LsdState::label(int n, bool rank, hipStream_t s)
{
    launch_lsd_label(params, n, d_norder, d_cxy, d_row_start, d_clabel, d_comp_list, d_comp_count, d_comp_key, d_reg, s);
    if (rank) launch_lsd_rank(n * 3, d_comp_key, d_perm, s);
}

void LsdState::grow(int n, float* lines, int* counts, int lds_kb, bool mixed, bool use_perm, hipStream_t s)
{
    launch_lsd_grow(params, n, d_order_a, d_norder, d_cxy, d_cdeg, d_cmod, d_ccs, d_csn, d_row_start, d_clabel, d_comp_list, d_comp_count,
                    kCompCap, d_reg, d_gused, d_tmp_lines, d_tmp_tags, lines, counts, use_perm ? d_perm : nullptr, lds_kb, mixed,
                    env_bitmap, s);
}

}
```

Baseline: 114,400.

## Compute LBD gradients only for tiles touched by segments, precompute segment headers

The segments kernel now also emits a per-segment LBD header (length, frame, direction vector, start corner) and marks, in a per-frame bitmask, which 64x64 gradient tiles each segment's support region touches. The LBD gradient kernel then exits early for unmarked tiles, so Sobel work is skipped over empty parts of the image. The descriptor kernel reads the precomputed header instead of redoing atan2/sincos per segment, and the band-normalisation stage for four segments is handled by one wave after a block barrier. The changes add mask bookkeeping and a __syncthreads in the descriptor loop, and they rely on the tile margin being large enough to cover every gradient sample read.

```diff
diff --git a/lane_slam_amd/csrc/common.h b/lane_slam_amd/csrc/common.h
--- a/lane_slam_amd/csrc/common.h
+++ b/lane_slam_amd/csrc/common.h
@@ -4,6 +4,7 @@
 #include <stddef.h>
 #include "../../include/lanefront.h"
 #include "detmath.h"
+#include "lbd_setup.h"
 
 namespace lf {
 
@@ -148,14 +149,15 @@
 enum SegMode { SEG_FLOAT = 0, SEG_HOUGH = 1, SEG_DENSE = 2 };
 void launch_segments(const SegParams& p, int n_frames, const float* slot_lines, const int* counts,
                      const int* seg_offset, const uint32_t* side, int Ww, lf_segments out, int* seg_frame,
-                     double* normals64, float* centers, hipStream_t s, SegMode mode = SEG_FLOAT);
-void launch_lbd_grad(int Hc, int W, int n_frames, const uint8_t* gray, uint32_t* dxy, hipStream_t s);
+                     double* normals64, float* centers, hipStream_t s, SegMode mode = SEG_FLOAT,
+                     LbdSegHeader* lbd_hdr = nullptr, uint32_t* lbd_mask = nullptr, int lbd_rows = 63);
+void launch_lbd_grad(int Hc, int W, int n_frames, const uint8_t* gray, uint32_t* dxy, hipStream_t s, const uint32_t* tile_mask = nullptr);
 struct LbdPlanes { const uint32_t* base[LF_MAX_OCTAVES]; int W[LF_MAX_OCTAVES], H[LF_MAX_OCTAVES]; };
 void launch_lbd_keylines(const LbdPlanes& planes, int n_cap, int n_frames, const int* n_lines, const float* in_octave4, const float* angle, const int* npx,
                          const int* octave, const int* frame, const float* gauss_g, const float* gauss_l, float* desc, uint8_t* code,
                          hipStream_t s, int wband = 7);
 void launch_lbd_split_debug(size_t n, const uint32_t* dxy, int16_t* dx, int16_t* dy, hipStream_t s);
-void launch_lbd(int Hc, int W, int n_seg_cap, const int* n_seg, const float* lines, const int* seg_frame,
+void launch_lbd(int Hc, int W, int n_seg_cap, const int* n_seg, const LbdSegHeader* hdr,
                 const uint32_t* dxy, const float* gauss_g, const float* gauss_l,
                 float* desc, uint8_t* code, hipStream_t s, int wband = 7);
 int lbd_max_width_of_band();
diff --git a/lane_slam_amd/csrc/k_lbd.hip b/lane_slam_amd/csrc/k_lbd.hip
--- a/lane_slam_amd/csrc/k_lbd.hip
+++ b/lane_slam_amd/csrc/k_lbd.hip
@@ -2,10 +2,7 @@
 
 namespace lf {
 
-#ifndef LF_LBD_TILE_H
-#define LF_LBD_TILE_H 64
-#endif
-constexpr int LT_W = 64, LT_H = LF_LBD_TILE_H;
+constexpr int LT_W = LBD_TILE_W, LT_H = LBD_TILE_H;
 static_assert(LT_H % 16 == 0, "the Sobel phase gives every lane LT_H / 16 rows of its column group");
 
 __device__ __forceinline__ int refl101(int p, int n)
@@ -16,7 +13,7 @@
 }
 
 __global__ __launch_bounds__(256) void k_lbd_grad(int Hc, int W, const uint8_t* __restrict__ gray_in,
-                                                  uint32_t* __restrict__ dxyo)
+                                                  uint32_t* __restrict__ dxyo, const uint32_t* __restrict__ tile_mask)
 {
     constexpr int GW = 72, GH = LT_H + 6;
     constexpr int RW = 68, RG = RW / 4;
@@ -26,6 +23,10 @@
     __shared__ __attribute__((aligned(16))) uint8_t blur[BH * BW_];
     int tbx, tby, f;
     lf_xcd_tile(tbx, tby, f);
+    if (tile_mask) {
+        const int t = tby * (int)gridDim.x + tbx;
+        if (!((tile_mask[(size_t)f * lbd_mask_words(W, Hc) + (t >> 5)] >> (t & 31)) & 1u)) return;
+    }
     const int x0 = tbx * LT_W, y0 = tby * LT_H;
     const int tid = threadIdx.y * 64 + threadIdx.x;
     const uint8_t* img = gray_in + (size_t)f * Hc * W;
@@ -164,10 +165,10 @@
     }
 }
 
-void launch_lbd_grad(int Hc, int W, int n_frames, const uint8_t* gray, uint32_t* dxy, hipStream_t s)
-{
-    dim3 grid((W + LT_W - 1) / LT_W, (Hc + LT_H - 1) / LT_H, n_frames);
-    hipLaunchKernelGGL(k_lbd_grad, grid, dim3(64, 4), 0, s, Hc, W, gray, dxy);
+void launch_lbd_grad(int Hc, int W, int n_frames, const uint8_t* gray, uint32_t* dxy, hipStream_t s, const uint32_t* tile_mask)
+{
+    dim3 grid(lbd_tiles_x(W), lbd_tiles_y(Hc), n_frames);
+    hipLaunchKernelGGL(k_lbd_grad, grid, dim3(64, 4), 0, s, Hc, W, gray, dxy, tile_mask);
 }
 
 __constant__ int c_comb[32][2] = {
@@ -181,7 +182,7 @@
 template <bool KL, bool ANYW = false>
 __global__ __launch_bounds__(256) void k_lbd(int Hc_, int W_, const int* __restrict__ n_seg_ptr,
                                              const float* __restrict__ lines, const int* __restrict__ seg_frame,
-                                             const uint32_t* __restrict__ dxyi,
+                                             const LbdSegHeader* __restrict__ hdr, const uint32_t* __restrict__ dxyi,
                                              const float* __restrict__ gauss_g , const float* __restrict__ gauss_l ,
                                              float* __restrict__ desc, uint8_t* __restrict__ code,
                                              LbdPlanes planes, const float* __restrict__ kl_angle, const int* __restrict__ kl_npx,
@@ -193,53 +194,51 @@
     __shared__ float dsc[4][72];
     const int wave = threadIdx.x >> 6, lane = threadIdx.x & 63;
     const int n_seg = min(*n_seg_ptr, n_cap);
-  for (int seg = blockIdx.x * 4 + wave; seg < n_seg; seg += gridDim.x * 4) {
-    __builtin_amdgcn_wave_barrier();
-    __builtin_amdgcn_fence(__ATOMIC_ACQ_REL, "wavefront");
-    const int f = seg_frame[seg];
+    auto described = [&](int sg) {
+        if (!KL) return true;
+        const int oc = kl_octave[sg], f = seg_frame[sg];
+        return !(oc < 0 || oc >= LF_MAX_OCTAVES || planes.base[oc] == nullptr || f < 0 || f >= n_frames);
+    };
+  for (int base = blockIdx.x * 4; base < n_seg; base += gridDim.x * 4) {
+    const int seg = base + wave;
+    bool sample = seg < n_seg;
     int Hc = Hc_, W = W_;
-    const uint32_t* pdxy;
-    float e0 = lines[4 * (size_t)seg], e1 = lines[4 * (size_t)seg + 1], e2 = lines[4 * (size_t)seg + 2], e3 = lines[4 * (size_t)seg + 3];
-    int lengthOfLSP;
-    float direction;
-    if (KL) {
-        const int oc = kl_octave[seg];
-        if (oc < 0 || oc >= LF_MAX_OCTAVES || planes.base[oc] == nullptr || f < 0 || f >= n_frames) {
+    const uint32_t* pdxy = nullptr;
+    int lengthOfLSP = 0;
+    float dL0 = 0, dL1 = 0, sCorX0 = 0, sCorY0 = 0;
+    if (sample && KL) {
+        if (!described(seg)) {
             if (desc) for (int i = lane; i < 72; i += 64) desc[(size_t)seg * 72 + i] = 0.f;
             if (code && lane < 32) code[(size_t)seg * 32 + lane] = 0;
-            continue;
-        }
-        Hc = planes.H[oc]; W = planes.W[oc];
-        pdxy = planes.base[oc] + (size_t)f * Hc * W;
-        lengthOfLSP = (int)(short)kl_npx[seg];
-        direction = kl_angle[seg];
-    } else {
-    pdxy = dxyi + (size_t)f * Hc * W;
-    if (e0 < 0) e0 = 0;
-    if (e0 >= W) e0 = (float)W - 1.0f;
-    if (e2 < 0) e2 = 0;
-    if (e2 >= W) e2 = (float)W - 1.0f;
-    if (e1 < 0) e1 = 0;
-    if (e1 >= Hc) e1 = (float)Hc - 1.0f;
-    if (e3 < 0) e3 = 0;
-    if (e3 >= Hc) e3 = (float)Hc - 1.0f;
-    const int ix0 = dm::round_half_even((double)e0), iy0 = dm::round_half_even((double)e1);
-    const int ix1 = dm::round_half_even((double)e2), iy1 = dm::round_half_even((double)e3);
-    lengthOfLSP = max(abs(ix1 - ix0), abs(iy1 - iy0)) + 1;
-    const float ddy = e3 - e1, ddx = e2 - e0;
-    direction = (float)dm::datan2((double)ddy, (double)ddx);
-    }
-    const int halfWidth = (lengthOfLSP - 1) / 2;
-    const int halfHeight = (LSP_H - 1) / 2;
+            sample = false;
+        } else {
+            const int f = seg_frame[seg], oc = kl_octave[seg];
+            const float e0 = lines[4 * (size_t)seg], e1 = lines[4 * (size_t)seg + 1], e2 = lines[4 * (size_t)seg + 2], e3 = lines[4 * (size_t)seg + 3];
+            Hc = planes.H[oc]; W = planes.W[oc];
+            pdxy = planes.base[oc] + (size_t)f * Hc * W;
+            lengthOfLSP = (int)(short)kl_npx[seg];
+            const float direction = kl_angle[seg];
+            const int halfWidth = (lengthOfLSP - 1) / 2;
+            const int halfHeight = (LSP_H - 1) / 2;
+            const float midX = (float)(0.5 * (e0 + e2));
+            const float midY = (float)(0.5 * (e1 + e3));
+            double sn_, cs_;
+            dm::dsincos((double)direction, sn_, cs_);
+            dL0 = (float)cs_; dL1 = (float)sn_;
+            sCorX0 = -dL0 * halfWidth + dL1 * halfHeight + midX;
+            sCorY0 = -dL1 * halfWidth - dL0 * halfHeight + midY;
+        }
+    } else if (sample) {
+        const uint4* hp = reinterpret_cast<const uint4*>(hdr + seg);
+        const uint4 h0 = hp[0], h1 = hp[1];
+        lengthOfLSP = (int)h0.x;
+        pdxy = dxyi + (size_t)(int)h0.y * Hc * W;
+        dL0 = __uint_as_float(h0.z); dL1 = __uint_as_float(h0.w);
+        sCorX0 = __uint_as_float(h1.x); sCorY0 = __uint_as_float(h1.y);
+    }
+    if (sample) {
     const int imageWidth = W - 1, imageHeight = Hc - 1;
-    const float midX = (float)(0.5 * (e0 + e2));
-    const float midY = (float)(0.5 * (e1 + e3));
-    double sn_, cs_;
-    dm::dsincos((double)direction, sn_, cs_);
-    const float dL0 = (float)cs_, dL1 = (float)sn_;
     const float dO0 = -dL1, dO1 = dL0;
-    float sCorX0 = -dL0 * halfWidth + dL1 * halfHeight + midX;
-    float sCorY0 = -dL1 * halfWidth - dL0 * halfHeight + midY;
     int row_done = 0;
     for (int row = lane; row < LSP_H; row += 64) {
         for (; row_done < row; ++row_done) { sCorX0 -= dL1; sCorY0 += dL0; }
@@ -274,88 +273,118 @@
         rows[wave][row][3] = cg * ngdO;
         if (!ANYW) break;
     }
-    __builtin_amdgcn_wave_barrier();
-    __builtin_amdgcn_fence(__ATOMIC_ACQ_REL, "wavefront");
-    float* D = dsc[wave];
-    for (int e = lane; e < 72; e += 64) {
-        const int b = e >> 3, q = e & 7;
-        const bool sq = q >= 4;
-        const int src = q & 3;
-        const int h0 = (b - 1) * WBAND;
-        const float* rp = &rows[wave][0][src] + 4 * h0;
-        float acc = 0;
-#pragma unroll
-        for (int i = 0; i < (ANYW ? 3 * LBD_MAXW : 3 * lf::WBAND); ++i) {
-            if (ANYW && i >= 3 * WBAND) break;
-            const int hID = h0 + i;
-            if (hID >= 0 && hID < LSP_H) {
-                const float coef = gauss_l[i];
-                const float v = rp[4 * i];
-                if (!sq) acc += coef * v;
-                else acc += coef * coef * (v * v);
-            }
-        }
-        D[e] = acc;
-    }
-    __builtin_amdgcn_wave_barrier();
-    __builtin_amdgcn_fence(__ATOMIC_ACQ_REL, "wavefront");
-    float mean[4] = {0, 0, 0, 0}, sd[4] = {0, 0, 0, 0};
-    if (lane < NBANDS) {
-        const float invN = (lane == 0 || lane == NBANDS - 1) ? (float)(1.0 / (WBAND * 2.0)) : (float)(1.0 / (WBAND * 3.0));
-#pragma unroll
-        for (int q = 0; q < 4; ++q) {
-            float temp = D[lane * 8 + q] * invN;
-            mean[q] = temp;
-            sd[q] = (float)dm::dsqrt((double)(D[lane * 8 + 4 + q] * invN - temp * temp));
-        }
-    }
-    __builtin_amdgcn_wave_barrier();
-    __builtin_amdgcn_fence(__ATOMIC_ACQ_REL, "wavefront");
-    if (lane < NBANDS) {
-#pragma unroll
-        for (int q = 0; q < 4; ++q) { D[lane * 8 + q] = mean[q]; D[lane * 8 + 4 + q] = sd[q]; }
-    }
-    __builtin_amdgcn_wave_barrier();
-    __builtin_amdgcn_fence(__ATOMIC_ACQ_REL, "wavefront");
-    float tempM = 0, tempS = 0;
-    for (int b = 0; b < NBANDS; ++b) {
-        const float* v = D + 8 * b;
-        tempM += v[0] * v[0]; tempM += v[1] * v[1]; tempM += v[2] * v[2]; tempM += v[3] * v[3];
-        tempS += v[4] * v[4]; tempS += v[5] * v[5]; tempS += v[6] * v[6]; tempS += v[7] * v[7];
-    }
-    tempM = dm::fdiv(1.f, dm::fsqrt(tempM));
-    tempS = dm::fdiv(1.f, dm::fsqrt(tempS));
-    __builtin_amdgcn_wave_barrier();
-    for (int e = lane; e < 72; e += 64) {
-        float v = D[e] * (((e & 7) < 4) ? tempM : tempS);
-        if ((double)v > 0.4) v = (float)0.4;
-        D[e] = v;
-    }
-    __builtin_amdgcn_wave_barrier();
-    __builtin_amdgcn_fence(__ATOMIC_ACQ_REL, "wavefront");
-    float temp = 0;
-    for (int i = 0; i < 72; ++i) temp += D[i] * D[i];
-    temp = dm::fdiv(1.f, dm::fsqrt(temp));
-    __builtin_amdgcn_wave_barrier();
-    for (int e = lane; e < 72; e += 64) {
-        float v = D[e] * temp;
-        D[e] = v;
-        if (desc) desc[(size_t)seg * 72 + e] = v;
-    }
-    __builtin_amdgcn_wave_barrier();
-    __builtin_amdgcn_fence(__ATOMIC_ACQ_REL, "wavefront");
-    if (code && lane < 32) {
-        const float* f1 = D + 8 * c_comb[lane][0];
-        const float* f2 = D + 8 * c_comb[lane][1];
-        unsigned r = 0;
-#pragma unroll
-        for (int i = 0; i < 8; ++i) if (f1[i] > f2[i]) r += 1u << i;
-        code[(size_t)seg * 32 + lane] = (uint8_t)r;
-    }
+    }
+    __syncthreads();
+    if (wave == 0) {
+        bool have[4];
+#pragma unroll
+        for (int j = 0; j < 4; ++j) have[j] = base + j < n_seg && described(base + j);
+        auto have_of = [&](int j) { return j == 0 ? have[0] : (j == 1 ? have[1] : (j == 2 ? have[2] : have[3])); };
+        for (int it = lane; it < 4 * 72; it += 64) {
+            const int j = it / 72, e = it - 72 * j;
+            if (!have_of(j)) continue;
+            const int b = e >> 3, q = e & 7;
+            const bool sq = q >= 4;
+            const int src = q & 3;
+            const int h0 = (b - 1) * WBAND;
+            const float* rp = &rows[j][0][src] + 4 * h0;
+            float acc = 0;
+#pragma unroll
+            for (int i = 0; i < (ANYW ? 3 * LBD_MAXW : 3 * lf::WBAND); ++i) {
+                if (ANYW && i >= 3 * WBAND) break;
+                const int hID = h0 + i;
+                if (hID >= 0 && hID < LSP_H) {
+                    const float coef = gauss_l[i];
+                    const float v = rp[4 * i];
+                    if (!sq) acc += coef * v;
+                    else acc += coef * coef * (v * v);
+                }
+            }
+            dsc[j][e] = acc;
+        }
+        __builtin_amdgcn_wave_barrier();
+        __builtin_amdgcn_fence(__ATOMIC_ACQ_REL, "wavefront");
+        if (lane < 4 * NBANDS) {
+            const int j = lane / NBANDS, b = lane - NBANDS * j;
+            if (have_of(j)) {
+                float* D = dsc[j];
+                const float invN = (b == 0 || b == NBANDS - 1) ? (float)(1.0 / (WBAND * 2.0)) : (float)(1.0 / (WBAND * 3.0));
+                float mean[4], sd[4];
+#pragma unroll
+                for (int q = 0; q < 4; ++q) {
+                    float temp = D[b * 8 + q] * invN;
+                    mean[q] = temp;
+                    sd[q] = (float)dm::dsqrt((double)(D[b * 8 + 4 + q] * invN - temp * temp));
+                }
+#pragma unroll
+                for (int q = 0; q < 4; ++q) { D[b * 8 + q] = mean[q]; D[b * 8 + 4 + q] = sd[q]; }
+            }
+        }
+        __builtin_amdgcn_wave_barrier();
+        __builtin_amdgcn_fence(__ATOMIC_ACQ_REL, "wavefront");
+        const int js = lane & 3;
+        const bool sums = lane < 4 && have_of(js);
+        float tempM = 0, tempS = 0;
+        if (sums) {
+            for (int b = 0; b < NBANDS; ++b) {
+                const float* v = dsc[js] + 8 * b;
+                tempM += v[0] * v[0]; tempM += v[1] * v[1]; tempM += v[2] * v[2]; tempM += v[3] * v[3];
+                tempS += v[4] * v[4]; tempS += v[5] * v[5]; tempS += v[6] * v[6]; tempS += v[7] * v[7];
+            }
+            tempM = dm::fdiv(1.f, dm::fsqrt(tempM));
+            tempS = dm::fdiv(1.f, dm::fsqrt(tempS));
+        }
+        __builtin_amdgcn_wave_barrier();
+        __builtin_amdgcn_fence(__ATOMIC_ACQ_REL, "wavefront");
+        for (int it0 = 0; it0 < 4 * 72; it0 += 64) {
+            const int it = it0 + lane;
+            const int j = it < 4 * 72 ? it / 72 : 0, e = it - 72 * j;
+            const float sM = __shfl(tempM, j, 64), sS = __shfl(tempS, j, 64);
+            if (it < 4 * 72 && have_of(j)) {
+                float v = dsc[j][e] * (((e & 7) < 4) ? sM : sS);
+                if ((double)v > 0.4) v = (float)0.4;
+                dsc[j][e] = v;
+            }
+        }
+        __builtin_amdgcn_wave_barrier();
+        __builtin_amdgcn_fence(__ATOMIC_ACQ_REL, "wavefront");
+        float temp = 0;
+        if (sums) {
+            for (int i = 0; i < 72; ++i) temp += dsc[js][i] * dsc[js][i];
+            temp = dm::fdiv(1.f, dm::fsqrt(temp));
+        }
+        __builtin_amdgcn_wave_barrier();
+        __builtin_amdgcn_fence(__ATOMIC_ACQ_REL, "wavefront");
+        for (int it0 = 0; it0 < 4 * 72; it0 += 64) {
+            const int it = it0 + lane;
+            const int j = it < 4 * 72 ? it / 72 : 0, e = it - 72 * j;
+            const float sT = __shfl(temp, j, 64);
+            if (it < 4 * 72 && have_of(j)) {
+                const float v = dsc[j][e] * sT;
+                dsc[j][e] = v;
+                if (desc) desc[(size_t)(base + j) * 72 + e] = v;
+            }
+        }
+        __builtin_amdgcn_wave_barrier();
+        __builtin_amdgcn_fence(__ATOMIC_ACQ_REL, "wavefront");
+        if (code) {
+            for (int it = lane; it < 4 * 32; it += 64) {
+                const int j = it >> 5, k = it & 31;
+                if (!have_of(j)) continue;
+                const float* f1 = dsc[j] + 8 * c_comb[k][0];
+                const float* f2 = dsc[j] + 8 * c_comb[k][1];
+                unsigned r = 0;
+#pragma unroll
+                for (int i = 0; i < 8; ++i) if (f1[i] > f2[i]) r += 1u << i;
+                code[(size_t)(base + j) * 32 + k] = (uint8_t)r;
+            }
+        }
+    }
+    __syncthreads();
   }
 }
 
-void launch_lbd(int Hc, int W, int n_seg_cap, const int* n_seg, const float* lines, const int* seg_frame,
+void launch_lbd(int Hc, int W, int n_seg_cap, const int* n_seg, const LbdSegHeader* hdr,
                 const uint32_t* dxy, const float* gauss_g, const float* gauss_l,
                 float* desc, uint8_t* code, hipStream_t s, int wband)
 {
@@ -365,10 +394,10 @@
     LbdPlanes none;
     for (int i = 0; i < LF_MAX_OCTAVES; ++i) { none.base[i] = nullptr; none.W[i] = 0; none.H[i] = 0; }
     if (wband == WBAND)
-        hipLaunchKernelGGL((k_lbd<false, false>), dim3(blocks), dim3(256), 0, s, Hc, W, n_seg, lines, seg_frame, dxy,
+        hipLaunchKernelGGL((k_lbd<false, false>), dim3(blocks), dim3(256), 0, s, Hc, W, n_seg, nullptr, nullptr, hdr, dxy,
                            gauss_g, gauss_l, desc, code, none, nullptr, nullptr, nullptr, n_seg_cap, 0, WBAND);
     else
-        hipLaunchKernelGGL((k_lbd<false, true>), dim3(blocks), dim3(256), 0, s, Hc, W, n_seg, lines, seg_frame, dxy,
+        hipLaunchKernelGGL((k_lbd<false, true>), dim3(blocks), dim3(256), 0, s, Hc, W, n_seg, nullptr, nullptr, hdr, dxy,
                            gauss_g, gauss_l, desc, code, none, nullptr, nullptr, nullptr, n_seg_cap, 0, wband);
 }
 int lbd_max_width_of_band() { return LBD_MAXW; }
@@ -381,10 +410,10 @@
     int blocks = (n_cap + 3) / 4;
     if (blocks > 4096) blocks = 4096;
     if (wband == WBAND)
-        hipLaunchKernelGGL((k_lbd<true, false>), dim3(blocks), dim3(256), 0, s, 0, 0, n_lines, in_octave4, frame, nullptr, gauss_g, gauss_l, desc, code,
+        hipLaunchKernelGGL((k_lbd<true, false>), dim3(blocks), dim3(256), 0, s, 0, 0, n_lines, in_octave4, frame, nullptr, nullptr, gauss_g, gauss_l, desc, code,
                            planes, angle, npx, octave, n_cap, n_frames, WBAND);
     else
-        hipLaunchKernelGGL((k_lbd<true, true>), dim3(blocks), dim3(256), 0, s, 0, 0, n_lines, in_octave4, frame, nullptr, gauss_g, gauss_l, desc, code,
+        hipLaunchKernelGGL((k_lbd<true, true>), dim3(blocks), dim3(256), 0, s, 0, 0, n_lines, in_octave4, frame, nullptr, nullptr, gauss_g, gauss_l, desc, code,
                            planes, angle, npx, octave, n_cap, n_frames, wband);
 }
 
diff --git a/lane_slam_amd/csrc/k_segments.hip b/lane_slam_amd/csrc/k_segments.hip
--- a/lane_slam_amd/csrc/k_segments.hip
+++ b/lane_slam_amd/csrc/k_segments.hip
@@ -89,7 +89,8 @@
 __global__ void k_segments(SegParams p, int n_frames, const float* __restrict__ slot_lines,
                            const int* __restrict__ counts, const int* __restrict__ seg_offset,
                            const uint32_t* __restrict__ maskbits, int Ww, lf_segments out, int* __restrict__ seg_frame,
-                           double* __restrict__ normals64, float* __restrict__ centers)
+                           double* __restrict__ normals64, float* __restrict__ centers,
+                           LbdSegHeader* __restrict__ lbd_hdr, uint32_t* __restrict__ lbd_mask, int lbd_rows)
 {
     const int slot = blockIdx.x * blockDim.x + threadIdx.x;
     const int pc = slot / p.cap_lines, i = slot - pc * p.cap_lines;
@@ -157,6 +158,16 @@
     if (centers) { centers[2 * (size_t)idx] = cx; centers[2 * (size_t)idx + 1] = cy; }
     }
     if (seg_frame) seg_frame[idx] = f;
+    if (lbd_hdr) {
+        const LbdSegHeader hd = lbd_seg_header(x1, y1, x2, y2, f, p.W, p.Hc, lbd_rows);
+        uint4* hp = reinterpret_cast<uint4*>(lbd_hdr + idx);
+        hp[0] = make_uint4((uint32_t)hd.lengthOfLSP, (uint32_t)hd.frame, __float_as_uint(hd.dL0), __float_as_uint(hd.dL1));
+        hp[1] = make_uint4(__float_as_uint(hd.sCorX0), __float_as_uint(hd.sCorY0), 0u, 0u);
+        if (lbd_mask) {
+            uint32_t* words = lbd_mask + (size_t)f * lbd_mask_words(p.W, p.Hc);
+            lbd_mark_tiles(hd, p.W, p.Hc, lbd_rows, [&](int w, uint32_t bits) { atomicOr(words + w, bits); });
+        }
+    }
     const float pn0 = (float)(((double)x1 + 0.0) * p.rx);
     const float pn1 = (float)(((double)y1 + p.cut) * p.ry);
     const float pn2 = (float)(((double)x2 + 0.0) * p.rx);
@@ -183,18 +194,19 @@
 
 void launch_segments(const SegParams& p, int n_frames, const float* slot_lines, const int* counts,
                      const int* seg_offset, const uint32_t* side, int Ww, lf_segments out, int* seg_frame,
-                     double* normals64, float* centers, hipStream_t s, SegMode mode)
+                     double* normals64, float* centers, hipStream_t s, SegMode mode,
+                     LbdSegHeader* lbd_hdr, uint32_t* lbd_mask, int lbd_rows)
 {
     const int total = n_frames * 3 * p.cap_lines;
     if (mode == SEG_DENSE)
         hipLaunchKernelGGL(k_segments<SEG_DENSE>, dim3((total + 255) / 256), dim3(256), 0, s, p, n_frames, slot_lines, counts,
-                           seg_offset, side, Ww, out, seg_frame, normals64, centers);
+                           seg_offset, side, Ww, out, seg_frame, normals64, centers, lbd_hdr, lbd_mask, lbd_rows);
     else if (mode == SEG_HOUGH)
         hipLaunchKernelGGL(k_segments<SEG_HOUGH>, dim3((total + 255) / 256), dim3(256), 0, s, p, n_frames, slot_lines, counts,
-                           seg_offset, side, Ww, out, seg_frame, normals64, centers);
+                           seg_offset, side, Ww, out, seg_frame, normals64, centers, lbd_hdr, lbd_mask, lbd_rows);
     else
         hipLaunchKernelGGL(k_segments<SEG_FLOAT>, dim3((total + 255) / 256), dim3(256), 0, s, p, n_frames, slot_lines, counts,
-                           seg_offset, side, Ww, out, seg_frame, normals64, centers);
-}
-
-}
+                           seg_offset, side, Ww, out, seg_frame, normals64, centers, lbd_hdr, lbd_mask, lbd_rows);
+}
+
+}
diff --git a/lane_slam_amd/csrc/lanefront_api.hip b/lane_slam_amd/csrc/lanefront_api.hip
--- a/lane_slam_amd/csrc/lanefront_api.hip
+++ b/lane_slam_amd/csrc/lanefront_api.hip
@@ -189,7 +189,7 @@
     if (dalloc(h, &h->d_frames, h->frames_bytes) || dalloc(h, &h->d_bgr, B * P) || dalloc(h, &h->d_gray, B * P) || 
         dalloc(h, &h->d_edges_u8, B * P) || dalloc(h, &h->d_strong, B * h->Hc * h->Ww) || dalloc(h, &h->d_weak, B * h->Hc * h->Ww) || dalloc(h, &h->d_maskbits, nprob * h->Hc * h->Ww) ||
         dalloc(h, &h->d_counts, nprob) || dalloc(h, &h->d_seg_offset, nprob + 1) || dalloc(h, &h->d_frame_offset, B + 1) ||
-        dalloc(h, &h->d_slot_lines, cap * 4) || dalloc(h, &h->d_seg_frame, cap) ||
+        dalloc(h, &h->d_slot_lines, cap * 4) || dalloc(h, &h->d_seg_frame, cap) || dalloc(h, &h->d_lbd_hdr, cap) ||
         dalloc(h, &h->d_dxy, B * P) || dalloc(h, &h->d_normals64, cap * 2) ||
         dalloc(h, &h->d_centers, cap * 2))
         return LF_ERR_HIP;
@@ -353,26 +353,41 @@
 }
 
 
+static bool diag_flag(const char* name)
+{
+    const char* e = getenv(name);
+    return e && *e && strcmp(e, "0") != 0;
+}
+
 int lf::run_segments(lf_handle* h, int n, lf_segments dev_out, bool describe)
 {
     hipStream_t s = h->stream;
+    const int lbd_rows = 9 * h->desc_params.width_of_band;
     {
         StageClock::Scope t(h, h->clock, ST_SEGMENTS);
-        if (!h->overflow_zeroed) LF_HIP_CHECK(h, hipMemsetAsync(h->lsd.d_overflow, 0, 4 * sizeof(int), s));
+        if (!h->overflow_zeroed) {
+            uint32_t* from = describe ? h->lsd.d_lbd_mask : reinterpret_cast<uint32_t*>(h->lsd.d_overflow);
+            LF_HIP_CHECK(h, hipMemsetAsync(from, 0, (size_t)(reinterpret_cast<uint32_t*>(h->lsd.d_overflow) - from) * 4 + 4 * sizeof(int), s));
+        }
         h->overflow_zeroed = false;
         launch_seg_offsets(n, h->cap_lines, h->d_counts, h->d_seg_offset, dev_out.frame_offset ? dev_out.frame_offset : h->d_frame_offset,
                            h->lsd.d_overflow, h->slot_mode != SEG_FLOAT ? nullptr : h->lsd.d_norder, lsd_grow_def_lds(h->lsd.params, kGrowLdsKb[0]),
                            lsd_grow_def_lds(h->lsd.params, kGrowLdsKb[1]), s);
         launch_segments(h->seg, n, h->d_slot_lines, h->d_counts, h->d_seg_offset,
                         h->slot_mode == SEG_DENSE ? reinterpret_cast<const uint32_t*>(h->d_dense_rec.p) : h->d_maskbits.p, h->Ww, dev_out,
-                        h->d_seg_frame, h->d_normals64, h->d_centers, s, h->slot_mode);
+                        h->d_seg_frame, h->d_normals64, h->d_centers, s, h->slot_mode,
+                        describe ? h->d_lbd_hdr.p : nullptr, describe ? h->lsd.d_lbd_mask : nullptr, lbd_rows);
     }
     if (describe) {
-        { StageClock::Scope t(h, h->clock, ST_LBD_GRAD); launch_lbd_grad(h->Hc, h->W, n, h->d_gray, h->d_dxy, s); }
+        {
+            StageClock::Scope t(h, h->clock, ST_LBD_GRAD);
+            if (diag_flag("LF_DIAG_LBD_POISON")) LF_HIP_CHECK(h, hipMemsetD32Async(reinterpret_cast<hipDeviceptr_t>(h->d_dxy.p), 0x7fff7fff, (size_t)n * h->P, s));
+            launch_lbd_grad(h->Hc, h->W, n, h->d_gray, h->d_dxy, s, diag_flag("LF_DIAG_LBD_ALL_TILES") ? nullptr : h->lsd.d_lbd_mask);
+        }
         {
             StageClock::Scope t(h, h->clock, ST_LBD);
             int cap = dev_out.capacity < n * 3 * h->cap_lines ? dev_out.capacity : n * 3 * h->cap_lines;
-            launch_lbd(h->Hc, h->W, cap, h->d_seg_offset + n * 3, dev_out.lines, h->d_seg_frame, h->d_dxy,
+            launch_lbd(h->Hc, h->W, cap, h->d_seg_offset + n * 3, h->d_lbd_hdr, h->d_dxy,
                        h->d_gauss_g, h->d_gauss_l, dev_out.desc, dev_out.code, s, h->desc_params.width_of_band);
         }
     }
@@ -971,6 +986,7 @@
         int rc = scratch(h, h->dbg_dx, n * h->P * sizeof(int16_t));
         if (rc == LF_OK) rc = scratch(h, h->dbg_dy, n * h->P * sizeof(int16_t));
         if (rc != LF_OK) return rc;
+        launch_lbd_grad(h->Hc, h->W, (int)n, h->d_gray, h->d_dxy, s);
         launch_lbd_split_debug(n * h->P, h->d_dxy, (int16_t*)h->dbg_dx.p, (int16_t*)h->dbg_dy.p, s);
         src = buffer_id == LF_BUF_LBD_DX ? h->dbg_dx.p : h->dbg_dy.p;
         avail = n * h->P * sizeof(int16_t);
diff --git a/lane_slam_amd/csrc/lanefront_handle.h b/lane_slam_amd/csrc/lanefront_handle.h
--- a/lane_slam_amd/csrc/lanefront_handle.h
+++ b/lane_slam_amd/csrc/lanefront_handle.h
@@ -115,6 +115,7 @@
     DevArray<uint8_t> d_zero; size_t zero_bytes = 0;
     unsigned long long* d_maxgrad = nullptr;
     int *d_nrec = nullptr, *d_nlow = nullptr, *d_tile_count = nullptr, *d_overflow = nullptr;
+    uint32_t* d_lbd_mask = nullptr; int lbd_mask_stride = 0;
     int lists_grown = 0;
     bool lists_lost = false;
     bool grow_mixed = false;
@@ -182,6 +183,7 @@
     lf::DevArray<int> d_counts, d_seg_offset, d_frame_offset;
     lf::DevArray<float> d_slot_lines;
     lf::DevArray<int> d_seg_frame;
+    lf::DevArray<lf::LbdSegHeader> d_lbd_hdr;
     lf::DevArray<uint32_t> d_dxy;
     lf::DevBuf dbg_dx, dbg_dy;
     lf::DevArray<float> d_gauss_g, d_gauss_l;
diff --git a/lane_slam_amd/csrc/lanefront_lsd.hip b/lane_slam_amd/csrc/lanefront_lsd.hip
--- a/lane_slam_amd/csrc/lanefront_lsd.hip
+++ b/lane_slam_amd/csrc/lanefront_lsd.hip
@@ -122,14 +122,17 @@
         dalloc(h, &d_comp_list, nprob * (size_t)kCompCap) || dalloc(h, &d_comp_count, nprob) || dalloc(h, &d_perm, nprob) || dalloc(h, &d_comp_key, nprob) ||
         dalloc(h, &d_tmp_lines, cap * 4) || dalloc(h, &d_tmp_tags, cap) || dalloc(h, &d_norder, nprob))
         return LF_ERR_HIP;
-    zero_bytes = nprob * 8 + nprob * 4 + nprob * 4 + 16 + 32;
+    lbd_mask_stride = lbd_mask_words(W, Hc);
+    const size_t mask_bytes = (size_t)max_frames * lbd_mask_stride * 4;
+    zero_bytes = nprob * 8 + nprob * 4 + nprob * 4 + 16 + mask_bytes + 32;
     if (dalloc(h, &d_zero, zero_bytes)) return LF_ERR_HIP;
     d_maxgrad = reinterpret_cast<unsigned long long*>(d_zero.p);
     d_nrec = reinterpret_cast<int*>(d_zero + nprob * 8);
     int* nlow = d_nrec + nprob;
     if (seed_order == LF_LSD_SEED_OPENCV32) d_nlow = nlow;
     d_tile_count = nlow + nprob;
-    d_overflow = d_tile_count + 4;
+    d_lbd_mask = reinterpret_cast<uint32_t*>(d_tile_count + 4);
+    d_overflow = reinterpret_cast<int*>(d_lbd_mask + (size_t)max_frames * lbd_mask_stride);
     LF_HIP_CHECK(h, hipMemset(d_zero, 0, zero_bytes));
     if (const char* ev = getenv("LF_GROW_LDS_LEVEL")) { const int v = atoi(ev); env_lds_level = v < 0 ? 0 : (v > 2 ? 2 : v); }
     if (const char* ev = getenv("LF_GROW_MIXED")) env_mixed = atoi(ev) != 0 ? 1 : 0;
diff --git a/lane_slam_amd/csrc/lbd_setup.h b/lane_slam_amd/csrc/lbd_setup.h
--- /dev/null
+++ b/lane_slam_amd/csrc/lbd_setup.h
@@ -0,0 +1,97 @@
+#pragma once
+#include "detmath.h"
+
+#ifndef LF_LBD_TILE_H
+#define LF_LBD_TILE_H 64
+#endif
+
+namespace lf {
+
+constexpr int LBD_TILE_W = 64, LBD_TILE_H = LF_LBD_TILE_H;
+
+struct LbdSegHeader {
+    int lengthOfLSP;
+    int frame;
+    float dL0, dL1;
+    float sCorX0, sCorY0;
+    int pad[2];
+};
+static_assert(sizeof(LbdSegHeader) == 32, "k_lbd reads a header as two uint4");
+
+LF_HD int lbd_tiles_x(int W) { return (W + LBD_TILE_W - 1) / LBD_TILE_W; }
+LF_HD int lbd_tiles_y(int Hc) { return (Hc + LBD_TILE_H - 1) / LBD_TILE_H; }
+LF_HD int lbd_mask_words(int W, int Hc) { return (lbd_tiles_x(W) * lbd_tiles_y(Hc) + 31) / 32; }
+
+LF_HD LbdSegHeader lbd_seg_header(float e0, float e1, float e2, float e3, int frame, int W, int Hc, int lsp_h)
+{
+    if (e0 < 0) e0 = 0;
+    if (e0 >= W) e0 = (float)W - 1.0f;
+    if (e2 < 0) e2 = 0;
+    if (e2 >= W) e2 = (float)W - 1.0f;
+    if (e1 < 0) e1 = 0;
+    if (e1 >= Hc) e1 = (float)Hc - 1.0f;
+    if (e3 < 0) e3 = 0;
+    if (e3 >= Hc) e3 = (float)Hc - 1.0f;
+    const int ix0 = dm::round_half_even((double)e0), iy0 = dm::round_half_even((double)e1);
+    const int ix1 = dm::round_half_even((double)e2), iy1 = dm::round_half_even((double)e3);
+    const int adx = ix1 - ix0 < 0 ? ix0 - ix1 : ix1 - ix0, ady = iy1 - iy0 < 0 ? iy0 - iy1 : iy1 - iy0;
+    const int lengthOfLSP = (adx > ady ? adx : ady) + 1;
+    const float ddy = e3 - e1, ddx = e2 - e0;
+    const float direction = (float)dm::datan2((double)ddy, (double)ddx);
+    const int halfWidth = (lengthOfLSP - 1) / 2;
+    const int halfHeight = (lsp_h - 1) / 2;
+    const float midX = (float)(0.5 * (e0 + e2));
+    const float midY = (float)(0.5 * (e1 + e3));
+    double sn_, cs_;
+    dm::dsincos((double)direction, sn_, cs_);
+    const float dL0 = (float)cs_, dL1 = (float)sn_;
+    LbdSegHeader h;
+    h.lengthOfLSP = lengthOfLSP;
+    h.frame = frame;
+    h.dL0 = dL0; h.dL1 = dL1;
+    h.sCorX0 = -dL0 * halfWidth + dL1 * halfHeight + midX;
+    h.sCorY0 = -dL1 * halfWidth - dL0 * halfHeight + midY;
+    h.pad[0] = 0; h.pad[1] = 0;
+    return h;
+}
+
+constexpr float LBD_TILE_MARGIN = 1.5f;
+
+LF_HD int lbd_clamp_px(float v, float vmax)
+{
+    return !(v > 0.f) ? 0 : (int)(v > vmax ? vmax : v);
+}
+
+template <class Mark>
+LF_HD void lbd_mark_tiles(const LbdSegHeader& h, int W, int Hc, int lsp_h, Mark&& mark)
+{
+    if (h.lengthOfLSP < 1) return;
+    const int TX = lbd_tiles_x(W);
+    const float xmax = (float)(W - 1), ymax = (float)(Hc - 1);
+    const float span = (float)(h.lengthOfLSP - 1);
+    const float sx = span * h.dL0, sy = span * h.dL1;
+    float ox = h.sCorX0, oy = h.sCorY0;
+    int wa = -1, wb = -1;
+    uint32_t ba = 0, bb = 0;
+    for (int row = 0; row < lsp_h; ++row) {
+        const float ex = ox + sx, ey = oy + sy;
+        const int x0 = lbd_clamp_px((ox < ex ? ox : ex) - LBD_TILE_MARGIN, xmax), x1 = lbd_clamp_px((ox < ex ? ex : ox) + LBD_TILE_MARGIN, xmax);
+        const int y0 = lbd_clamp_px((oy < ey ? oy : ey) - LBD_TILE_MARGIN, ymax), y1 = lbd_clamp_px((oy < ey ? ey : oy) + LBD_TILE_MARGIN, ymax);
+        for (int ty = y0 / LBD_TILE_H; ty <= y1 / LBD_TILE_H; ++ty)
+            for (int tx = x0 / LBD_TILE_W; tx <= x1 / LBD_TILE_W; ++tx) {
+                const int t = ty * TX + tx, w = t >> 5;
+                const uint32_t bit = 1u << (t & 31);
+                if (w == wa) ba |= bit;
+                else if (w == wb) bb |= bit;
+                else {
+                    if (ba) mark(wa, ba);
+                    wa = wb; ba = bb; wb = w; bb = bit;
+                }
+            }
+        ox -= h.dL1; oy += h.dL0;
+    }
+    if (ba) mark(wa, ba);
+    if (bb) mark(wb, bb);
+}
+
+}
```

New measurement: 110,200. 0.963x the previous value.
